# ru-wang/slam-plus-plus

Measured on AMD Instinct MI355X. Metric: Λ-solve block-nnz/sec + batch GN iters/sec, Venice BA, 1→8 MI355X, higher is better.
Workload: dtype f64; 1 GPU; venice871-shaped synthetic BA (871 cams, 530304 points, 2838740 observations, LM-damped); nnzb=3369915, n=1596138, mode=schur+dense, n_reduced=5226, schur_pairs=12875640, parallelism=single GPU

## Files before the change

include/spp_hip.h:

```cpp
#ifndef SPP_HIP_H
#define SPP_HIP_H

#include <stddef.h>
#include <stdint.h>

#ifdef __cplusplus
extern "C" {
#endif

#define SPP_OK            0
#define SPP_NOT_POSDEF    1
#define SPP_E_BADARG     -1
#define SPP_E_NOMEM      -2
#define SPP_E_HIP        -3
#define SPP_E_NO_DEVICE  -4
#define SPP_E_STATE      -5
#define SPP_E_UNSUPPORTED -6

#define SPP_MODE_AUTO     0
#define SPP_MODE_SPARSE   1
#define SPP_MODE_SCHUR    2
#define SPP_MODE_SCHUR_SPARSE 3

#define SPP_FLAG_PROFILE  1
// ... 31 lines not shown
#define SPP_INFO_N_SUPERNODES   12
#define SPP_INFO_N_LEVELS       13
#define SPP_INFO_S_LD           14
#define SPP_INFO_S_NNZB         15
#define SPP_INFO_DENSE_STREAMED 16
#define SPP_INFO_LM_STREAM      17
#define SPP_INFO_BS_GROUPS      18
#define SPP_INFO_SCHUR_SIDE     19
#define SPP_INFO_S_CLEAR        20
#define SPP_INFO_S_DEVICE_PTR   21
#define SPP_INFO_ASM_HUB_CHUNK   22
#define SPP_INFO_SOLVE_ASYNC    23
int spp_get_info(const spp_ctx *ctx, int what, int64_t *out);
int spp_get_ordering(const spp_ctx *ctx, int64_t *h_order);
int64_t spp_sparse_fronts(const spp_ctx *ctx, int64_t capacity, int32_t *h, int32_t *w, int32_t *pad, int32_t *cls, int32_t *level,
	int32_t *parent, int32_t *team);

#define SPP_ORDER_AMD 0
#define SPP_ORDER_ND  1
int spp_block_ordering(int64_t nb, const int64_t *col_ptr, const int64_t *row_idx, int method, int64_t *h_order);

int spp_schur_plan_host(int64_t nb, const int32_t *dim, const int64_t *col_ptr, const int64_t *row_idx, int shard_rank,
	int shard_world, int sparse_S, int64_t *out, double *seconds);

int spp_factor_solve(spp_ctx *ctx, const double *h_vals, double *h_rhs_inout);

int spp_factor_solve_device(spp_ctx *ctx, const double *d_vals, double *d_rhs_inout);

int spp_schur_buffer_size(const spp_ctx *ctx, int64_t *n_doubles);
int spp_schur_form(spp_ctx *ctx, const double *d_vals, const double *d_rhs, double *d_S_rhs);
int spp_schur_finish(spp_ctx *ctx, const double *d_vals, double *d_S_rhs, double *d_rhs_inout);
int spp_schur_packed_size(const spp_ctx *ctx, int64_t *n_doubles);
int spp_schur_pack(spp_ctx *ctx, const double *d_S_rhs, double *d_packed);
int spp_schur_unpack(spp_ctx *ctx, const double *d_packed, double *d_S_rhs);

int spp_assemble_analyze(spp_ctx *ctx, int64_t nv, const int32_t *h_dim,
	int64_t ne, const int64_t *h_v0, const int64_t *h_v1, int d0, int d1, int rd,
	int64_t unary_vertex);
int spp_assemble_get_structure(const spp_ctx *ctx, int64_t *h_col_ptr, int64_t *h_row_idx,
	int64_t *h_blk_off);
int spp_assemble_device(spp_ctx *ctx, const double *d_J0, const double *d_J1,
	const double *d_Omega, const double *d_r, double damping, double *d_vals_out, double *d_eta_out);
int spp_assemble_set_edge_weights(spp_ctx *ctx, const double *d_w);
#define SPP_MAX_EDGE_GROUPS 4
int spp_assemble_analyze_groups(spp_ctx *ctx, int64_t nv, const int32_t *h_dim, int n_groups,
	const int64_t *h_ne, const int64_t *const *h_v0, const int64_t *const *h_v1, const int64_t *const *h_seq,
	const int32_t *h_d0, const int32_t *h_d1, const int32_t *h_rd, int64_t unary_vertex);
int spp_assemble_groups_device(spp_ctx *ctx, const double *const *d_J0, const double *const *d_J1,
	const double *const *d_Omega, const double *const *d_r, double damping, double *d_vals_out, double *d_eta_out);
int spp_assemble_set_group_edge_weights(spp_ctx *ctx, int group, const double *d_w);
int spp_assemble_analyze_ternary(spp_ctx *ctx, int64_t nv, const int32_t *h_dim, int64_t ne, const int64_t *h_v0,
	const int64_t *h_v1, const int64_t *h_v2, int d0, int d1, int d2, int live2, int rd, int64_t unary_vertex);
int spp_assemble_ternary_device(spp_ctx *ctx, const double *d_J0, const double *d_J1, const double *d_J2,
	const double *d_Omega, const double *d_r, double damping, double *d_vals_out, double *d_eta_out);
int spp_edge_robust_weights_device(spp_ctx *ctx, int64_t n_edges, int rd, int kind, double scale, double param,
	const double *d_r, double *d_w_out);

int spp_se2_linearize_device(spp_ctx *ctx, int64_t n_edges, const int32_t *d_v0, const int32_t *d_v1,
	const double *d_poses, const double *d_measurements, double *d_J0, double *d_J1, double *d_r);
int spp_se2_update_device(spp_ctx *ctx, int64_t n_vertices, double *d_poses, const double *d_dx, int apply,
	double *h_dx_norm2);

int spp_se2_linearize_at_device(spp_ctx *ctx, int64_t n_edges, const int64_t *d_off0, const int64_t *d_off1,
	const double *d_state, const double *d_measurements, double *d_J0, double *d_J1, double *d_r);
int spp_se2_rb_linearize_device(spp_ctx *ctx, int64_t n_edges, const int64_t *d_pose_off, const int64_t *d_lm_off,
	const double *d_state, const double *d_measurements, double *d_J0, double *d_J1, double *d_r);
int spp_slam2d_update_device(spp_ctx *ctx, int64_t n, double *d_state, const double *d_dx, int64_t n_pose_angles,
	const int64_t *d_angle_off, int apply, double *h_dx_norm2);

int spp_se3_linearize_device(spp_ctx *ctx, int64_t n_edges, const int32_t *d_v0, const int32_t *d_v1,
	const double *d_poses, const double *d_measurements, double *d_J0, double *d_J1, double *d_r);
int spp_se3_update_device(spp_ctx *ctx, int64_t n_vertices, double *d_poses, const double *d_dx, int apply,
	double *h_dx_norm2);

int spp_se3_linearize_at_device(spp_ctx *ctx, int64_t n_edges, const int64_t *d_off0, const int64_t *d_off1,
	const double *d_state, const double *d_measurements, double *d_J0, double *d_J1, double *d_r);
int spp_se3_xyz_linearize_device(spp_ctx *ctx, int64_t n_edges, const int64_t *d_pose_off, const int64_t *d_lm_off,
	const double *d_state, const double *d_measurements, double *d_J0, double *d_J1, double *d_r);
int spp_slam3d_update_device(spp_ctx *ctx, int64_t n, double *d_state, const double *d_dx, int64_t n_poses,
	const int64_t *d_pose_off, int apply, double *h_dx_norm2);

int spp_rocv_range_linearize_device(spp_ctx *ctx, int64_t n_edges, const int64_t *d_recv_off, const int64_t *d_lm_off,
	const double *d_state, const double *d_measurements, double *d_J0, double *d_J1, double *d_r);
int spp_rocv_cv_linearize_device(spp_ctx *ctx, int64_t n_edges, const int64_t *d_off0, const int64_t *d_off1,
	const double *d_state, const double *d_dt, double *d_J0, double *d_J1, double *d_r);

int spp_ba_linearize_device(spp_ctx *ctx, int64_t n_obs, const int32_t *d_cam_of, const int32_t *d_pt_of,
	const double *d_cams, const double *d_intrinsics, const double *d_points, const double *d_measurements,
	double *d_J0, double *d_J1, double *d_r);
int spp_ba_update_device(spp_ctx *ctx, int64_t n_cams, double *d_cams, const int64_t *d_cam_dxoff,
	int64_t n_points, double *d_points, const int64_t *d_pt_dxoff, const double *d_dx, int64_t n_dx, int apply,
	double *h_dx_norm2);

int spp_sim3_ba_linearize_device(spp_ctx *ctx, int64_t n_obs, const int32_t *d_cam_of, const int32_t *d_pt_of,
	const double *d_cams, const double *d_intrinsics, const double *d_points, const double *d_measurements,
	double *d_J0, double *d_J1, double *d_r);
int spp_sim3_update_device(spp_ctx *ctx, int64_t n_cams, double *d_cams, const int64_t *d_cam_dxoff,
	int64_t n_points, double *d_points, const int64_t *d_pt_dxoff, const double *d_dx, int64_t n_dx, int apply,
	double *h_dx_norm2);

int spp_ba_stereo_linearize_device(spp_ctx *ctx, int64_t n_obs, const int32_t *d_cam_of, const int32_t *d_pt_of,
	const double *d_cams, const double *d_intrinsics, const double *d_points, const double *d_measurements,
	double *d_J0, double *d_J1, double *d_r);

int spp_ba_intrinsics_linearize_device(spp_ctx *ctx, int64_t n_obs, const int32_t *d_cam_of, const int32_t *d_pt_of,
	const int32_t *d_intr_of, const double *d_cams, const double *d_intrinsics, const double *d_points,
	const double *d_measurements, double *d_J0, double *d_J1, double *d_J2, double *d_r);
int spp_ba_intrinsics_update_device(spp_ctx *ctx, int64_t n_intrinsics, double *d_intrinsics, const int64_t *d_intr_dxoff,
	const double *d_dx, int apply, double *h_dx_norm2);

int spp_edge_chi2_device(spp_ctx *ctx, int64_t n_edges, int rd, const double *d_r, const double *d_Omega, double *h_chi2);
int spp_edge_hessian_maxdiag_device(spp_ctx *ctx, int64_t n_edges, int rd, int d0, int d1, const double *d_J0,
	const double *d_J1, const double *d_Omega, double *h_max);
int spp_lm_gain_denominator_device(spp_ctx *ctx, int64_t n, const double *d_dx, const double *d_eta, double alpha,
	double *h_out);

int spp_device_malloc(spp_ctx *ctx, size_t bytes, void **d_ptr);
int spp_device_free(spp_ctx *ctx, void *d_ptr);
int spp_memcpy_h2d(spp_ctx *ctx, void *d_dst, const void *h_src, size_t bytes);
int spp_memcpy_d2h(spp_ctx *ctx, void *h_dst, const void *d_src, size_t bytes);
int spp_memcpy_d2d(spp_ctx *ctx, void *d_dst, const void *d_src, size_t bytes);

int spp_set_profiling(spp_ctx *ctx, int on);

#define SPP_PHASE_PERMUTE   0
#define SPP_PHASE_SCHUR_INV 1
#define SPP_PHASE_SCHUR_GEMM 2
#define SPP_PHASE_SCHUR_RHS 3
#define SPP_PHASE_FACTOR    4
#define SPP_PHASE_TRISOLVE  5
#define SPP_PHASE_BACKSUBST 6
#define SPP_PHASE_ASSEMBLE  7
#define SPP_PHASE_TOTAL     8
#define SPP_N_PHASES        9
int spp_get_phase_ms(spp_ctx *ctx, double *ms_out );
int spp_get_dominant_kernel(spp_ctx *ctx, double *ms_total, int64_t *n_launches, double *flops);

int spp_microbench_copy(spp_ctx *ctx, size_t bytes, int iters, double *gb_per_s);
int spp_microbench_mfma_f64(spp_ctx *ctx, int iters, double *tflops);
int spp_microbench_ctile(spp_ctx *ctx, int n, int iters, double *gb_per_s);
int spp_microbench_update(spp_ctx *ctx, int64_t m, int iters, double *ms_per_launch);

int spp_dense_potrf_upper(spp_ctx *ctx, double *d_A, int64_t n, int64_t ld);
int spp_dense_posv(spp_ctx *ctx, double *d_A, int64_t n, int64_t ld, double *d_b);
int spp_dense_posv_masked(spp_ctx *ctx, double *d_A, int64_t n, int64_t ld, double *d_b, const uint64_t *words, int64_t nwords);
int spp_tile_mask_host(int64_t n, int bs, int64_t nblk, const int32_t *i1, const int32_t *i2, int has_rhs, int fill,
	uint64_t *words, int64_t *n_updates);
int spp_schur_tile_mask_host(int64_t nb, const int32_t *dim, const int64_t *col_ptr, const int64_t *row_idx, int shard_rank,
	int shard_world, uint64_t *words);
int spp_schur_cam_order_host(int64_t nb, const int32_t *dim, const int64_t *col_ptr, const int64_t *row_idx, int shard_rank,
	int shard_world, int flags, const int64_t *order_in, int64_t *cam_order, double *figures);
int spp_tail_order_host(int64_t n, int has_rhs, const uint64_t *words, int64_t nwords, int resident, int early, double beta,
	int32_t *table, int32_t *info);
int spp_dense_gemm_tn_sub(spp_ctx *ctx, int64_t m, int64_t n, int64_t k,
	const double *d_A, int64_t lda, const double *d_B, int64_t ldb, double *d_C, int64_t ldc);
int spp_dense_gemm_tn_sub_upper(spp_ctx *ctx, int64_t m, int64_t n, int64_t k,
	const double *d_A, int64_t lda, const double *d_B, int64_t ldb, double *d_C, int64_t ldc);
int spp_dense_front_factor(spp_ctx *ctx, double *d_F, int64_t ld, int64_t w, int64_t h, double *d_image);

const char *spp_version(void);

#ifdef __cplusplus
}
#endif
#endif
```

slam_plus_plus_amd/api.py:

```python
import ctypes
import os

import numpy as np

_HERE = os.path.dirname(os.path.abspath(__file__))
LIB_PATH = os.environ.get("SPP_LIB") or os.path.join(_HERE, "libspp_hip.so")

SPP_OK, SPP_NOT_POSDEF = 0, 1
MODE_AUTO, MODE_SPARSE, MODE_SCHUR, MODE_SCHUR_SPARSE, MODE_SCHUR_MIS = 0, 1, 2, 3, 4
FLAG_PROFILE = 1
INFO = dict(MODE=0, N=1, NNZB=2, NVALS=3, FACTOR_NNZ=4, FACTOR_FLOPS=5, N_REDUCED=6, N_POSES=7,
            N_LANDMARKS=8, SCHUR_PAIRS=9, N_OBS=10, SOLVE_BYTES=11, N_SUPERNODES=12, N_LEVELS=13, S_LD=14, S_NNZB=15, DENSE_STREAMED=16,
            LM_STREAM=17, BS_GROUPS=18, SCHUR_SIDE=19, S_CLEAR=20, S_DEVICE_PTR=21, ASM_HUB_CHUNK=22, SOLVE_ASYNC=23)
PHASES = ["permute", "schur_inv", "schur_gemm", "schur_rhs", "factor", "trisolve", "backsubst", "assemble", "total"]

EXPORTS = [
    "spp_create", "spp_destroy", "spp_free_memory", "spp_last_error", "spp_host_staging", "spp_set_stream", "spp_synchronize",
    "spp_analyze", "spp_set_shard", "spp_get_info", "spp_get_ordering", "spp_sparse_fronts", "spp_factor_solve",
    "spp_factor_solve_device", "spp_schur_buffer_size", "spp_schur_form", "spp_schur_finish",
    "spp_schur_packed_size", "spp_schur_pack", "spp_schur_unpack",
    "spp_assemble_analyze", "spp_assemble_get_structure", "spp_assemble_device", "spp_assemble_set_edge_weights",
    "spp_assemble_analyze_groups", "spp_assemble_groups_device", "spp_assemble_set_group_edge_weights",
    "spp_assemble_analyze_ternary", "spp_assemble_ternary_device", "spp_ba_intrinsics_linearize_device",
    "spp_ba_intrinsics_update_device",
    "spp_se2_linearize_at_device", "spp_se2_rb_linearize_device", "spp_slam2d_update_device",
    "spp_se3_linearize_at_device", "spp_se3_xyz_linearize_device", "spp_slam3d_update_device", "spp_rocv_range_linearize_device",
    "spp_rocv_cv_linearize_device", "spp_device_malloc",
    "spp_device_free", "spp_memcpy_h2d", "spp_memcpy_d2h", "spp_memcpy_d2d", "spp_get_phase_ms", "spp_get_dominant_kernel",
    "spp_microbench_copy", "spp_microbench_mfma_f64", "spp_microbench_ctile", "spp_microbench_update", "spp_block_ordering", "spp_schur_plan_host", "spp_set_profiling", "spp_se2_linearize_device", "spp_se2_update_device", "spp_ba_linearize_device", "spp_ba_stereo_linearize_device", "spp_ba_update_device", "spp_sim3_ba_linearize_device", "spp_sim3_update_device", "spp_se3_linearize_device", "spp_se3_update_device", "spp_edge_chi2_device", "spp_edge_robust_weights_device", "spp_edge_hessian_maxdiag_device",
    "spp_lm_gain_denominator_device", "spp_dense_potrf_upper", "spp_dense_posv",
    "spp_dense_posv_masked", "spp_tile_mask_host", "spp_schur_tile_mask_host", "spp_tail_order_host", "spp_schur_cam_order_host",
    "spp_dense_gemm_tn_sub", "spp_dense_gemm_tn_sub_upper", "spp_dense_front_factor", "spp_version",
]

_lib = None
_c_i64p = ctypes.POINTER(ctypes.c_int64)
_c_i32p = ctypes.POINTER(ctypes.c_int32)
_c_f64p = ctypes.POINTER(ctypes.c_double)


class SppError(RuntimeError):
    """std::runtime_error of the C++ adapter (reference LinearSolver_Schur_GPU.cpp:734-797)."""


def load_library():
    global _lib
    if _lib is not None:
        return _lib
    if not os.path.exists(LIB_PATH):
        raise SppError("libspp_hip.so is not built: run `python -m slam_plus_plus_amd.build` "
                       "(hipcc --offload-arch=gfx950); there is no CPU fallback")
    lib = ctypes.CDLL(LIB_PATH)
    vp, i64, i32, dbl, cint = ctypes.c_void_p, ctypes.c_int64, ctypes.c_int32, ctypes.c_double, ctypes.c_int
    sig = {
        "spp_create": (vp, [cint, cint]),
        "spp_destroy": (None, [vp]),
        "spp_free_memory": (cint, [vp]),
        "spp_last_error": (cint, [vp, ctypes.c_char_p, ctypes.c_size_t]),
        "spp_host_staging": (vp, [vp, i64]),
        "spp_set_stream": (cint, [vp, vp]),
        "spp_synchronize": (cint, [vp]),
        "spp_analyze": (cint, [vp, i64, vp, vp, vp, vp, cint]),
        "spp_set_shard": (cint, [vp, cint, cint]),
        "spp_get_info": (cint, [vp, cint, _c_i64p]),
        "spp_get_ordering": (cint, [vp, vp]),
        "spp_sparse_fronts": (i64, [vp, i64, vp, vp, vp, vp, vp, vp, vp]),
        "spp_factor_solve": (cint, [vp, vp, vp]),
        "spp_factor_solve_device": (cint, [vp, vp, vp]),
        "spp_schur_buffer_size": (cint, [vp, _c_i64p]),
        "spp_schur_form": (cint, [vp, vp, vp, vp]),
        "spp_schur_finish": (cint, [vp, vp, vp, vp]),
        "spp_schur_packed_size": (cint, [vp, _c_i64p]),
        "spp_schur_pack": (cint, [vp, vp, vp]),
        "spp_schur_unpack": (cint, [vp, vp, vp]),
        "spp_assemble_analyze": (cint, [vp, i64, vp, i64, vp, vp, cint, cint, cint, i64]),
        "spp_assemble_get_structure": (cint, [vp, vp, vp, vp]),
        "spp_assemble_device": (cint, [vp, vp, vp, vp, vp, dbl, vp, vp]),
        "spp_assemble_set_edge_weights": (cint, [vp, vp]),
        "spp_assemble_analyze_groups": (cint, [vp, i64, vp, cint, vp, vp, vp, vp, vp, vp, vp, i64]),
        "spp_assemble_groups_device": (cint, [vp, vp, vp, vp, vp, dbl, vp, vp]),
        "spp_assemble_set_group_edge_weights": (cint, [vp, cint, vp]),
        "spp_assemble_analyze_ternary": (cint, [vp, i64, vp, i64, vp, vp, vp, cint, cint, cint, cint, cint, i64]),
        "spp_assemble_ternary_device": (cint, [vp, vp, vp, vp, vp, vp, dbl, vp, vp]),
        "spp_ba_intrinsics_linearize_device": (cint, [vp, i64, vp, vp, vp, vp, vp, vp, vp, vp, vp, vp, vp]),
        "spp_ba_intrinsics_update_device": (cint, [vp, i64, vp, vp, vp, cint, _c_f64p]),
        "spp_se2_linearize_at_device": (cint, [vp, i64, vp, vp, vp, vp, vp, vp, vp]),
        "spp_se2_rb_linearize_device": (cint, [vp, i64, vp, vp, vp, vp, vp, vp, vp]),
        "spp_slam2d_update_device": (cint, [vp, i64, vp, vp, i64, vp, cint, _c_f64p]),
        "spp_se3_linearize_at_device": (cint, [vp, i64, vp, vp, vp, vp, vp, vp, vp]),
        "spp_se3_xyz_linearize_device": (cint, [vp, i64, vp, vp, vp, vp, vp, vp, vp]),
        "spp_slam3d_update_device": (cint, [vp, i64, vp, vp, i64, vp, cint, _c_f64p]),
        "spp_rocv_range_linearize_device": (cint, [vp, i64, vp, vp, vp, vp, vp, vp, vp]),
        "spp_rocv_cv_linearize_device": (cint, [vp, i64, vp, vp, vp, vp, vp, vp, vp]),
        "spp_device_malloc": (cint, [vp, ctypes.c_size_t, ctypes.POINTER(vp)]),
        "spp_device_free": (cint, [vp, vp]),
        "spp_memcpy_h2d": (cint, [vp, vp, vp, ctypes.c_size_t]),
        "spp_memcpy_d2h": (cint, [vp, vp, vp, ctypes.c_size_t]),
        "spp_memcpy_d2d": (cint, [vp, vp, vp, ctypes.c_size_t]),
        "spp_get_phase_ms": (cint, [vp, _c_f64p]),
        "spp_get_dominant_kernel": (cint, [vp, _c_f64p, _c_i64p, _c_f64p]),
        "spp_microbench_copy": (cint, [vp, ctypes.c_size_t, cint, _c_f64p]),
        "spp_microbench_mfma_f64": (cint, [vp, cint, _c_f64p]),
        "spp_microbench_ctile": (cint, [vp, cint, cint, _c_f64p]),
        "spp_microbench_update": (cint, [vp, ctypes.c_int64, cint, _c_f64p]),
        "spp_block_ordering": (cint, [ctypes.c_int64, vp, vp, cint, vp]),
        "spp_schur_plan_host": (cint, [ctypes.c_int64, vp, vp, vp, cint, cint, cint, vp, vp]),
        "spp_set_profiling": (cint, [vp, cint]),
        "spp_se2_linearize_device": (cint, [vp, ctypes.c_int64, vp, vp, vp, vp, vp, vp, vp]),
        "spp_se2_update_device": (cint, [vp, ctypes.c_int64, vp, vp, cint, _c_f64p]),
        "spp_se3_linearize_device": (cint, [vp, ctypes.c_int64, vp, vp, vp, vp, vp, vp, vp]),
        "spp_se3_update_device": (cint, [vp, ctypes.c_int64, vp, vp, cint, _c_f64p]),
        "spp_edge_chi2_device": (cint, [vp, ctypes.c_int64, cint, vp, vp, _c_f64p]),
        "spp_edge_robust_weights_device": (cint, [vp, ctypes.c_int64, cint, cint, dbl, dbl, vp, vp]),
        "spp_edge_hessian_maxdiag_device": (cint, [vp, ctypes.c_int64, cint, cint, cint, vp, vp, vp, _c_f64p]),
        "spp_lm_gain_denominator_device": (cint, [vp, ctypes.c_int64, vp, vp, ctypes.c_double, _c_f64p]),
        "spp_ba_linearize_device": (cint, [vp, ctypes.c_int64, vp, vp, vp, vp, vp, vp, vp, vp, vp]),
        "spp_ba_stereo_linearize_device": (cint, [vp, ctypes.c_int64, vp, vp, vp, vp, vp, vp, vp, vp, vp]),
        "spp_ba_update_device": (cint, [vp, ctypes.c_int64, vp, vp, ctypes.c_int64, vp, vp, vp, ctypes.c_int64, cint, _c_f64p]),
        "spp_sim3_ba_linearize_device": (cint, [vp, ctypes.c_int64, vp, vp, vp, vp, vp, vp, vp, vp, vp]),
        "spp_sim3_update_device": (cint, [vp, ctypes.c_int64, vp, vp, ctypes.c_int64, vp, vp, vp, ctypes.c_int64, cint, _c_f64p]),
        "spp_dense_potrf_upper": (cint, [vp, vp, i64, i64]),
        "spp_dense_posv": (cint, [vp, vp, i64, i64, vp]),
        "spp_dense_posv_masked": (cint, [vp, vp, i64, i64, vp, vp, i64]),
        "spp_tile_mask_host": (cint, [i64, cint, i64, vp, vp, cint, cint, vp, vp]),
        "spp_schur_tile_mask_host": (cint, [i64, vp, vp, vp, cint, cint, vp]),
        "spp_tail_order_host": (cint, [i64, cint, vp, i64, cint, cint, dbl, vp, vp]),
        "spp_schur_cam_order_host": (cint, [i64, vp, vp, vp, cint, cint, cint, vp, vp, vp]),
        "spp_dense_gemm_tn_sub": (cint, [vp, i64, i64, i64, vp, i64, vp, i64, vp, i64]),
        "spp_dense_gemm_tn_sub_upper": (cint, [vp, i64, i64, i64, vp, i64, vp, i64, vp, i64]),
        "spp_dense_front_factor": (cint, [vp, vp, i64, i64, i64, vp]),
        "spp_version": (ctypes.c_char_p, []),
    }
    for name, (res, args) in sig.items():
        fn = getattr(lib, name)
        fn.restype = res
        fn.argtypes = args
    _lib = lib
    return lib


def _ptr(a):
    return a.ctypes.data_as(ctypes.c_void_p)


ORDER_AMD, ORDER_ND = 0, 1


def block_ordering(lam, method=ORDER_AMD):
    lib = load_library()
    col_ptr = np.ascontiguousarray(lam.col_ptr, dtype=np.int64)
    row_idx = np.ascontiguousarray(lam.row_idx, dtype=np.int64)
    out = np.empty(lam.nb, dtype=np.int64)
    code = lib.spp_block_ordering(lam.nb, _ptr(col_ptr), _ptr(row_idx), method, _ptr(out))
    if code != 0:
        raise SppError("spp_block_ordering failed: %d" % code)
    return out


def schur_plan_host(lam, shard_rank=0, shard_world=1, sparse_S=False, mis=False):
    lib = load_library()
    col_ptr = np.ascontiguousarray(lam.col_ptr, dtype=np.int64)
    row_idx = np.ascontiguousarray(lam.row_idx, dtype=np.int64)
    dim = np.ascontiguousarray(lam.dim, dtype=np.int32)
    out = np.zeros(9, dtype=np.int64)
    sec = ctypes.c_double(0.0)
    code = lib.spp_schur_plan_host(lam.nb, _ptr(dim), _ptr(col_ptr), _ptr(row_idx), shard_rank, shard_world,
                                   (1 if sparse_S else 0) | (2 if mis else 0), _ptr(out), ctypes.byref(sec))
    if code != 0:
        raise SppError("spp_schur_plan_host failed: %d" % code)
    keys = ("nc", "nl", "no", "n_pairs", "n_sblk", "n_items", "n_multi", "checksum", "checksum_all")
    d = dict(zip(keys, (int(v) for v in out)))
    d["seconds"] = sec.value
    return d


def tile_mask_host(n, bs, i1, i2, has_rhs=True, fill=True):
    lib = load_library()
    i1 = np.ascontiguousarray(i1, dtype=np.int32)
    i2 = np.ascontiguousarray(i2, dtype=np.int32)
    words = np.zeros(64, dtype=np.uint64)
    upd = ctypes.c_int64(0)
    code = lib.spp_tile_mask_host(n, bs, i1.size, _ptr(i1), _ptr(i2), 1 if has_rhs else 0, 1 if fill else 0, _ptr(words),
                                  ctypes.byref(upd))
    if code < 0:
        raise SppError("spp_tile_mask_host failed: %d" % code)
    return words[:code].copy(), upd.value


def schur_tile_mask_host(lam, shard_rank=0, shard_world=1):
    lib = load_library()
    col_ptr = np.ascontiguousarray(lam.col_ptr, dtype=np.int64)
    row_idx = np.ascontiguousarray(lam.row_idx, dtype=np.int64)
    dim = np.ascontiguousarray(lam.dim, dtype=np.int32)
    words = np.zeros(64, dtype=np.uint64)
    code = lib.spp_schur_tile_mask_host(lam.nb, _ptr(dim), _ptr(col_ptr), _ptr(row_idx), shard_rank, shard_world, _ptr(words))
    if code < 0:
        raise SppError("spp_schur_tile_mask_host failed: %d" % code)
    return words[:code].copy()


def schur_cam_order_host(lam, order=None, sparse_S=False, mis=False, shard_rank=0, shard_world=1):
    lib = load_library()
    col_ptr = np.ascontiguousarray(lam.col_ptr, dtype=np.int64)
    row_idx = np.ascontiguousarray(lam.row_idx, dtype=np.int64)
    dim = np.ascontiguousarray(lam.dim, dtype=np.int32)
    nc = int((dim == dim.max()).sum()) if not mis else int(dim.size)
    out = np.full(max(nc, 1), -1, dtype=np.int64)
    fig = np.zeros(8, dtype=np.float64)
    oin = None if order is None else np.ascontiguousarray(order, dtype=np.int64)
    if oin is not None and oin.size != nc:
        raise SppError("schur_cam_order_host: order must list every camera once")
    code = lib.spp_schur_cam_order_host(lam.nb, _ptr(dim), _ptr(col_ptr), _ptr(row_idx), shard_rank, shard_world,
                                        (1 if sparse_S else 0) | (2 if mis else 0),
                                        _ptr(oin) if oin is not None else None, _ptr(out), _ptr(fig))
    if code < 0:
        raise SppError("spp_schur_cam_order_host failed: %d" % code)
    keys = ("tiles", "updates", "path", "cost_us")
    natural = dict(zip(keys, (int(fig[0]), int(fig[1]), int(fig[2]), float(fig[3]))))
    chosen = dict(zip(keys, (int(fig[4]), int(fig[5]), int(fig[6]), float(fig[7]))))
    return out[out >= 0], bool(code), natural, chosen


def tail_order_host(n, words, has_rhs=True, resident=256, early=True, beta=0.0):
    lib = load_library()
    words = np.ascontiguousarray(words if words is not None else [], dtype=np.uint64)
    table = np.zeros(64 * 65 // 2 + 64, dtype=np.int32)
    info = np.zeros(5, dtype=np.int32)
    code = lib.spp_tail_order_host(int(n), 1 if has_rhs else 0, _ptr(words) if words.size else None, words.size, int(resident),
                                   1 if early else 0, float(beta), _ptr(table), _ptr(info))
    if code < 0:
        raise SppError("spp_tail_order_host failed: %d" % code)
    tiles = [(int(t) >> 16, int(t) & 0xffff) for t in table[:code]]
    return tiles, dict(zip(("n_early", "r_star", "rows_resident", "live_demand", "widest"), (int(v) for v in info)))


class DeviceArray:

    def __init__(self, ctx, n, dtype=np.float64):
        self.ctx, self.n, self.dtype = ctx, int(n), np.dtype(dtype)
        p = ctypes.c_void_p()
        ctx._check(ctx.lib.spp_device_malloc(ctx.h, self.n * self.dtype.itemsize, ctypes.byref(p)))
        self.ptr = p.value

    @classmethod
    def from_host(cls, ctx, arr):
        arr = np.ascontiguousarray(arr)
        d = cls(ctx, arr.size, arr.dtype)
        d.upload(arr)
        return d

    def upload(self, arr):
        arr = np.ascontiguousarray(arr, dtype=self.dtype)
        assert arr.size == self.n
        self.ctx._check(self.ctx.lib.spp_memcpy_h2d(self.ctx.h, self.ptr, _ptr(arr), arr.nbytes))

    def download(self):
        out = np.empty(self.n, dtype=self.dtype)
        self.ctx._check(self.ctx.lib.spp_memcpy_d2h(self.ctx.h, _ptr(out), self.ptr, out.nbytes))
        return out

    def copy_from(self, other):
        assert other.n * other.dtype.itemsize <= self.n * self.dtype.itemsize
        self.ctx._check(self.ctx.lib.spp_memcpy_d2d(self.ctx.h, self.ptr, other.ptr, other.n * other.dtype.itemsize))

    def free(self):
        if self.ptr:
            self.ctx.lib.spp_device_free(self.ctx.h, self.ptr)
            self.ptr = None


class Context:

    def __init__(self, device=0, flags=0):
        self.lib = load_library()
        self.h = self.lib.spp_create(int(device), int(flags))
        if not self.h:
            raise SppError("spp_create failed: no usable HIP device %d (the solver has no CPU fallback)" % device)

    def close(self):
        if getattr(self, "h", None):
            self.lib.spp_destroy(self.h)
            self.h = None

    def __del__(self):
        try:
            self.close()
        except Exception:
            pass

    def last_error(self):
        buf = ctypes.create_string_buffer(1024)
        self.lib.spp_last_error(self.h, buf, 1024)
        return buf.value.decode(errors="replace")

    def _check(self, code):
        if code < 0:
            if code == -2:
                raise MemoryError(self.last_error())
            raise SppError("spp error %d: %s" % (code, self.last_error()))
        return code

    def analyze(self, bcsc, mode=MODE_AUTO):
        self._keep = bcsc
        return self._check(self.lib.spp_analyze(self.h, bcsc.nb, _ptr(bcsc.col_ptr), _ptr(bcsc.row_idx),
                                                 _ptr(bcsc.blk_off), _ptr(bcsc.dim), mode))

    def set_shard(self, rank, world):
        return self._check(self.lib.spp_set_shard(self.h, rank, world))

    def info(self, key):
        out = ctypes.c_int64()
        self._check(self.lib.spp_get_info(self.h, INFO[key], ctypes.byref(out)))
        return out.value

    def ordering(self, nb):
        out = np.empty(nb, dtype=np.int64)
        self._check(self.lib.spp_get_ordering(self.h, _ptr(out)))
        return out

    def sparse_fronts(self):
        keys = ("h", "w", "pad", "cls", "level", "parent", "team")
        ns = self._check(self.lib.spp_sparse_fronts(self.h, 0, None, None, None, None, None, None, None))
        out = {k: np.zeros(ns, dtype=np.int32) for k in keys}
        if ns:
            self._check(self.lib.spp_sparse_fronts(self.h, ns, *[_ptr(out[k]) for k in keys]))
        return out

    def se2_linearize_device(self, n_edges, d_v0, d_v1, d_poses, d_meas, d_J0, d_J1, d_r):
        return self._check(self.lib.spp_se2_linearize_device(self.h, n_edges, d_v0, d_v1, d_poses, d_meas, d_J0, d_J1, d_r))

    def se2_update_device(self, n_vertices, d_poses, d_dx, apply=True):
        out = ctypes.c_double()
        self._check(self.lib.spp_se2_update_device(self.h, n_vertices, d_poses, d_dx, 1 if apply else 0, ctypes.byref(out)))
        return out.value ** 0.5

    def se2_linearize_at_device(self, n_edges, d_off0, d_off1, d_state, d_meas, d_J0, d_J1, d_r):
        return self._check(self.lib.spp_se2_linearize_at_device(self.h, n_edges, d_off0, d_off1, d_state, d_meas, d_J0, d_J1, d_r))

    def se2_rb_linearize_device(self, n_edges, d_pose_off, d_lm_off, d_state, d_meas, d_J0, d_J1, d_r):
        return self._check(self.lib.spp_se2_rb_linearize_device(self.h, n_edges, d_pose_off, d_lm_off, d_state, d_meas, d_J0, d_J1, d_r))

    def slam2d_update_device(self, n, d_state, d_dx, n_pose_angles, d_angle_off, apply=True):
        out = ctypes.c_double()
        self._check(self.lib.spp_slam2d_update_device(self.h, n, d_state, d_dx, n_pose_angles, d_angle_off, 1 if apply else 0,
                                                      ctypes.byref(out)))
        return out.value ** 0.5

    def se3_linearize_at_device(self, n_edges, d_off0, d_off1, d_state, d_meas, d_J0, d_J1, d_r):
        return self._check(self.lib.spp_se3_linearize_at_device(self.h, n_edges, d_off0, d_off1, d_state, d_meas, d_J0, d_J1, d_r))

    def se3_xyz_linearize_device(self, n_edges, d_pose_off, d_lm_off, d_state, d_meas, d_J0, d_J1, d_r):
        return self._check(self.lib.spp_se3_xyz_linearize_device(self.h, n_edges, d_pose_off, d_lm_off, d_state, d_meas, d_J0, d_J1, d_r))

    def slam3d_update_device(self, n, d_state, d_dx, n_poses, d_pose_off, apply=True):
        out = ctypes.c_double()
        self._check(self.lib.spp_slam3d_update_device(self.h, n, d_state, d_dx, n_poses, d_pose_off, 1 if apply else 0,
                                                      ctypes.byref(out)))
        return out.value ** 0.5

    def rocv_range_linearize_device(self, n_edges, d_recv_off, d_lm_off, d_state, d_meas, d_J0, d_J1, d_r):
        return self._check(self.lib.spp_rocv_range_linearize_device(self.h, n_edges, d_recv_off, d_lm_off, d_state, d_meas, d_J0, d_J1, d_r))

    def rocv_cv_linearize_device(self, n_edges, d_off0, d_off1, d_state, d_dt, d_J0, d_J1, d_r):
        return self._check(self.lib.spp_rocv_cv_linearize_device(self.h, n_edges, d_off0, d_off1, d_state, d_dt, d_J0, d_J1, d_r))

    def se3_linearize_device(self, n_edges, d_v0, d_v1, d_poses, d_meas, d_J0, d_J1, d_r):
        return self._check(self.lib.spp_se3_linearize_device(self.h, n_edges, d_v0, d_v1, d_poses, d_meas, d_J0, d_J1, d_r))

    def se3_update_device(self, n_vertices, d_poses, d_dx, apply=True):
        out = ctypes.c_double()
        self._check(self.lib.spp_se3_update_device(self.h, n_vertices, d_poses, d_dx, 1 if apply else 0, ctypes.byref(out)))
        return out.value ** 0.5

    def edge_robust_weights_device(self, n_edges, rd, d_r, d_w, scale, param=1.345, kind=0):
        return self._check(self.lib.spp_edge_robust_weights_device(self.h, n_edges, rd, kind, float(scale), float(param), d_r, d_w))

    def edge_chi2_device(self, n_edges, rd, d_r, d_Om):
        out = ctypes.c_double()
        self._check(self.lib.spp_edge_chi2_device(self.h, n_edges, rd, d_r, d_Om, ctypes.byref(out)))
        return out.value

    def edge_hessian_maxdiag_device(self, n_edges, rd, d0, d1, d_J0, d_J1, d_Om):
        out = ctypes.c_double()
        self._check(self.lib.spp_edge_hessian_maxdiag_device(self.h, n_edges, rd, d0, d1, d_J0, d_J1, d_Om, ctypes.byref(out)))
        return out.value

# ... 227 lines not shown
```

slam_plus_plus_amd/csrc/spp_api.cpp:

```cpp

#include "spp_internal.h"
#include <string.h>
#include <new>

using namespace spp;

namespace spp {

void phases_reset(spp_ctx *ctx)
{
	if(!(ctx->flags & SPP_FLAG_PROFILE))
		return;
	if(!ctx->timer.created) {
		for(int i = 0; i < 2 * SPP_N_PHASES; ++ i)
			SPP_HIP_CHECK(hipEventCreate(&ctx->timer.ev[i]));
		ctx->timer.created = true;
	}
	for(int i = 0; i < SPP_N_PHASES; ++ i) {
		ctx->timer.used[i] = false;
		ctx->phase_ms[i] = 0;
	}
	ctx->dom_used = 0;
	ctx->dom_flops = 0;
}
// ... 404 lines not shown
	return SPP_OK;
}

int spp_get_ordering(const spp_ctx *ctx, int64_t *h_order)
{
	if(!ctx || !h_order)
		return SPP_E_BADARG;
	if(ctx->mode < 0)
		return SPP_E_STATE;
	for(size_t i = 0; i < ctx->order.size(); ++ i)
		h_order[i] = ctx->order[i];
	return SPP_OK;
}

int64_t spp_sparse_fronts(const spp_ctx *ctx, int64_t capacity, int32_t *h, int32_t *w, int32_t *pad, int32_t *cls, int32_t *level,
	int32_t *parent, int32_t *team)
{
	if(!ctx || capacity < 0)
		return SPP_E_BADARG;
#ifdef SPP_HAVE_SPARSE
	if(ctx->sparse)
		return sparse_fronts(ctx, capacity, h, w, pad, cls, level, parent, team);
#endif
	return 0;
}

int spp_block_ordering(int64_t nb, const int64_t *col_ptr, const int64_t *row_idx, int method, int64_t *h_order)
{
	if(nb <= 0 || !col_ptr || !row_idx || !h_order || (method != SPP_ORDER_AMD && method != SPP_ORDER_ND))
		return SPP_E_BADARG;
	try {
		for(int64_t j = 0; j < nb; ++ j)
			for(int64_t p = col_ptr[j]; p < col_ptr[j + 1]; ++ p)
				if(row_idx[p] < 0 || row_idx[p] > j)
					return SPP_E_BADARG;
		std::vector<int64_t> order;
		if(method == SPP_ORDER_AMD)
			min_degree_order(nb, col_ptr, row_idx, order);
		else
			nested_dissection_order(nb, col_ptr, row_idx, order);
		for(int64_t k = 0; k < nb; ++ k)
			h_order[k] = order[k];
		return SPP_OK;
	} catch(const std::bad_alloc &) {
		return SPP_E_NOMEM;
	} catch(...) {
		return SPP_E_HIP;
	}
}

static bool structure_of_pattern(int64_t nb, const int32_t *dim, const int64_t *col_ptr, const int64_t *row_idx, Structure &st)
{
	st.nb = nb;
	st.nnzb = col_ptr[nb];
	st.col_ptr.assign(col_ptr, col_ptr + nb + 1);
	st.row_idx.assign(row_idx, row_idx + st.nnzb);
	st.dim.assign(dim, dim + nb);
	st.base.resize(nb + 1);
	st.base[0] = 0;
	for(int64_t j = 0; j < nb; ++ j)
		st.base[j + 1] = st.base[j] + dim[j];
	st.n = st.base[nb];
	st.blk_off.resize(st.nnzb);
	int64_t off = 0;
	for(int64_t j = 0; j < nb; ++ j)
		for(int64_t p = col_ptr[j]; p < col_ptr[j + 1]; ++ p) {
			if(row_idx[p] < 0 || row_idx[p] > j)
				return false;
			st.blk_off[p] = off;
			off += (int64_t)dim[row_idx[p]] * dim[j];
		}
	st.nvals = off;
	return true;
}

extern "C++" {
template <class F>
static int schur_host_entry(int64_t nb, const int32_t *dim, const int64_t *col_ptr, const int64_t *row_idx, int shard_rank,
	int shard_world, const void *out, F fn)
{
	if(nb <= 0 || !dim || !col_ptr || !row_idx || !out || shard_world < 1 || shard_rank < 0 || shard_rank >= shard_world)
		return SPP_E_BADARG;
	try {
		Structure st;
		if(!structure_of_pattern(nb, dim, col_ptr, row_idx, st))
			return SPP_E_BADARG;
		return fn(st);
	} catch(const Error &e) {
		return e.code;
	} catch(const std::bad_alloc &) {
		return SPP_E_NOMEM;
	} catch(...) {
		return SPP_E_HIP;
	}
}
}

int spp_schur_plan_host(int64_t nb, const int32_t *dim, const int64_t *col_ptr, const int64_t *row_idx, int shard_rank,
	int shard_world, int sparse_S, int64_t *out, double *seconds)
{
	return schur_host_entry(nb, dim, col_ptr, row_idx, shard_rank, shard_world, out, [&](const Structure &st) {
		const double sec = schur_plan_host_probe(st, shard_rank, shard_world, (sparse_S & 1) != 0, (sparse_S & 2) != 0, out);
		if(seconds)
			*seconds = sec;
		return (int)SPP_OK;
	});
}

int spp_schur_tile_mask_host(int64_t nb, const int32_t *dim, const int64_t *col_ptr, const int64_t *row_idx, int shard_rank,
	int shard_world, uint64_t *words)
{
	return schur_host_entry(nb, dim, col_ptr, row_idx, shard_rank, shard_world, words, [&](const Structure &st) {
		std::vector<uint64_t> w;
		schur_tile_mask_host_probe(st, w);
		for(size_t q = 0; q < w.size(); ++ q)
			words[q] = w[q];
		return (int)w.size();
	});
}

int spp_schur_cam_order_host(int64_t nb, const int32_t *dim, const int64_t *col_ptr, const int64_t *row_idx, int shard_rank,
	int shard_world, int flags, const int64_t *order_in, int64_t *cam_order, double *figures)
{
	if(!figures)
		return SPP_E_BADARG;
	return schur_host_entry(nb, dim, col_ptr, row_idx, shard_rank, shard_world, cam_order, [&](const Structure &st) {
		if(order_in) {
			int64_t nc = 0;
			const int dmax = *std::max_element(dim, dim + nb);
			for(int64_t j = 0; j < nb; ++ j)
				nc += dim[j] == dmax;
			std::vector<char> seen((size_t)nc, 0);
			for(int64_t q = 0; q < nc; ++ q) {
				if(order_in[q] < 0 || order_in[q] >= nc || seen[order_in[q]])
					return (int)SPP_E_BADARG;
				seen[order_in[q]] = 1;
			}
		}
		std::vector<int32_t> order;
		TileDagCost cost[2];
		const bool used = schur_cam_order_host_probe(st, shard_rank, shard_world, (flags & 1) != 0, (flags & 2) != 0, order_in, order, cost);
		for(size_t q = 0; q < order.size(); ++ q)
			cam_order[q] = order[q];
		for(int side = 0; side < 2; ++ side) {
			figures[4 * side] = (double)cost[side].tiles;
			figures[4 * side + 1] = (double)cost[side].updates;
			figures[4 * side + 2] = (double)cost[side].path;
			figures[4 * side + 3] = cost[side].cost_us;
		}
		return used ? 1 : 0;
	});
}

int spp_schur_buffer_size(const spp_ctx *ctx, int64_t *n_doubles)
{
	if(!ctx || !n_doubles)
		return SPP_E_BADARG;
	if(ctx->mode != SPP_MODE_SCHUR)
		return SPP_E_STATE;
	*n_doubles = schur_buffer_doubles(ctx);
	return SPP_OK;
}

int spp_schur_form(spp_ctx *ctx, const double *d_vals, const double *d_rhs, double *d_S_rhs)
{
	if(!ctx || !d_vals || !d_rhs || !d_S_rhs)
		return SPP_E_BADARG;
	SPP_TRY(ctx)
	SPP_REQUIRE(ctx->mode == SPP_MODE_SCHUR, SPP_E_STATE, "spp_schur_form: analyze in Schur mode first");
	SPP_HIP_CHECK(hipSetDevice(ctx->device));
	phases_reset(ctx);
	phase_begin(ctx, SPP_PHASE_TOTAL);
	schur_form(ctx, d_vals, d_rhs, d_S_rhs);
	return SPP_OK;
	SPP_CATCH(ctx)
}

int spp_schur_packed_size(const spp_ctx *ctx, int64_t *n_doubles)
{
	if(!ctx || !n_doubles)
		return SPP_E_BADARG;
	if(ctx->mode != SPP_MODE_SCHUR)
		return SPP_E_STATE;
	if(ctx->schur.sparse_S) {
		*n_doubles = schur_buffer_doubles(ctx);
		return SPP_OK;
	}
	const int64_t nblk = ctx->schur.ld / DENSE_NB;
	*n_doubles = (int64_t)DENSE_NB * DENSE_NB * (nblk * (nblk + 1) / 2);
	return SPP_OK;
}

int spp_schur_pack(spp_ctx *ctx, const double *d_S_rhs, double *d_packed)
{
	if(!ctx || !d_S_rhs || !d_packed)
		return SPP_E_BADARG;
	SPP_TRY(ctx)
	SPP_REQUIRE(ctx->mode == SPP_MODE_SCHUR, SPP_E_STATE, "spp_schur_pack: analyze in Schur mode first");
	SPP_HIP_CHECK(hipSetDevice(ctx->device));
	if(ctx->schur.sparse_S)
		SPP_HIP_CHECK(hipMemcpyAsync(d_packed, d_S_rhs, (size_t)schur_buffer_doubles(ctx) * sizeof(double),
			hipMemcpyDeviceToDevice, ctx->stream));
	else
		schur_pack(ctx, const_cast<double*>(d_S_rhs), d_packed, true);
	return SPP_OK;
	SPP_CATCH(ctx)
}

int spp_schur_unpack(spp_ctx *ctx, const double *d_packed, double *d_S_rhs)
{
	if(!ctx || !d_S_rhs || !d_packed)
		return SPP_E_BADARG;
	SPP_TRY(ctx)
	SPP_REQUIRE(ctx->mode == SPP_MODE_SCHUR, SPP_E_STATE, "spp_schur_unpack: analyze in Schur mode first");
	SPP_HIP_CHECK(hipSetDevice(ctx->device));
	if(ctx->schur.sparse_S)
		SPP_HIP_CHECK(hipMemcpyAsync(d_S_rhs, d_packed, (size_t)schur_buffer_doubles(ctx) * sizeof(double),
			hipMemcpyDeviceToDevice, ctx->stream));
	else
		schur_pack(ctx, d_S_rhs, const_cast<double*>(d_packed), false);
	return SPP_OK;
	SPP_CATCH(ctx)
}

int spp_schur_finish(spp_ctx *ctx, const double *d_vals, double *d_S_rhs, double *d_rhs_inout)
{
	if(!ctx || !d_vals || !d_rhs_inout || !d_S_rhs)
		return SPP_E_BADARG;
	SPP_TRY(ctx)
	SPP_REQUIRE(ctx->mode == SPP_MODE_SCHUR, SPP_E_STATE, "spp_schur_finish: analyze in Schur mode first");
	SPP_HIP_CHECK(hipSetDevice(ctx->device));
	int ret = schur_finish(ctx, d_vals, d_S_rhs, d_rhs_inout);
	phase_end(ctx, SPP_PHASE_TOTAL);
	phases_collect(ctx);
	dense_chain_check(ctx);
	return ret;
	SPP_CATCH(ctx)
}

int spp_factor_solve_device(spp_ctx *ctx, const double *d_vals, double *d_rhs)
{
	if(!ctx || !d_vals || !d_rhs)
		return SPP_E_BADARG;
	SPP_TRY(ctx)
	SPP_REQUIRE(ctx->mode >= 0, SPP_E_STATE, "spp_factor_solve: call spp_analyze first");
	SPP_HIP_CHECK(hipSetDevice(ctx->device));
	phases_reset(ctx);
	phase_begin(ctx, SPP_PHASE_TOTAL);
	int ret;
	if(ctx->mode == SPP_MODE_SCHUR) {
		SPP_REQUIRE(ctx->shard_world == 1, SPP_E_STATE,
			"sharded ctx: use spp_schur_form / all-reduce / spp_schur_finish");
		if(!ctx->schur.S.p || ctx->schur.S.cap < (size_t)schur_buffer_doubles(ctx)) {
			ctx->schur.unlisted_dirty = true;
			ctx_drain(ctx);
		}
		ctx->schur.S.reserve((size_t)schur_buffer_doubles(ctx));
		schur_form(ctx, d_vals, d_rhs, ctx->schur.S.p, true);
		ret = schur_finish(ctx, d_vals, ctx->schur.S.p, d_rhs);
	} else
		ret = sparse_factor_solve(ctx, d_vals, d_rhs);
	phase_end(ctx, SPP_PHASE_TOTAL);
	phases_collect(ctx);
	if(!(ctx->mode == SPP_MODE_SCHUR && ctx->schur.async_last))
		SPP_HIP_CHECK(hipStreamSynchronize(ctx->stream));
	dense_chain_check(ctx);
	return ret;
	SPP_CATCH(ctx)
}

int spp_factor_solve(spp_ctx *ctx, const double *h_vals, double *h_rhs)
{
	if(!ctx || !h_vals || !h_rhs)
		return SPP_E_BADARG;
	SPP_TRY(ctx)
	SPP_REQUIRE(ctx->mode >= 0, SPP_E_STATE, "spp_factor_solve: call spp_analyze first");
	SPP_HIP_CHECK(hipSetDevice(ctx->device));
	ctx->d_vals.reserve((size_t)ctx->st.nvals);
	ctx->d_rhs.reserve((size_t)ctx->st.n);
	SPP_HIP_CHECK(hipMemcpyAsync(ctx->d_vals.p, h_vals, ctx->st.nvals * sizeof(double), hipMemcpyHostToDevice, ctx->stream));
	SPP_HIP_CHECK(hipMemcpyAsync(ctx->d_rhs.p, h_rhs, ctx->st.n * sizeof(double), hipMemcpyHostToDevice, ctx->stream));
	int ret = spp_factor_solve_device(ctx, ctx->d_vals.p, ctx->d_rhs.p);
	if(ret != SPP_OK)
		return ret;
	SPP_HIP_CHECK(hipMemcpyAsync(h_rhs, ctx->d_rhs.p, ctx->st.n * sizeof(double), hipMemcpyDeviceToHost, ctx->stream));
	SPP_HIP_CHECK(hipStreamSynchronize(ctx->stream));
	dense_chain_check(ctx);
	return SPP_OK;
	SPP_CATCH(ctx)
}

int spp_assemble_analyze(spp_ctx *ctx, int64_t nv, const int32_t *h_dim, int64_t ne, const int64_t *h_v0,
	const int64_t *h_v1, int d0, int d1, int rd, int64_t unary_vertex)
{
	if(!ctx)
		return SPP_E_BADARG;
	assemble_release(ctx);
	if(!h_dim || !h_v0 || !h_v1 || nv <= 0 || ne <= 0)
		return SPP_E_BADARG;
	SPP_TRY(ctx)
	SPP_HIP_CHECK(hipSetDevice(ctx->device));
	assemble_analyze(ctx, nv, h_dim, 1, &ne, &h_v0, &h_v1, nullptr, &d0, &d1, &rd, unary_vertex);
	return SPP_OK;
	SPP_CATCH(ctx)
}

// ... 365 lines not shown
		return SPP_E_BADARG;
	SPP_TRY(ctx)
	SPP_HIP_CHECK(hipSetDevice(ctx->device));
	SPP_HIP_CHECK(hipMemcpyAsync(h_dst, d_src, bytes, hipMemcpyDeviceToHost, ctx->stream));
	SPP_HIP_CHECK(hipStreamSynchronize(ctx->stream));
	dense_chain_check(ctx);
	return SPP_OK;
	SPP_CATCH(ctx)
}

int spp_memcpy_d2d(spp_ctx *ctx, void *d_dst, const void *d_src, size_t bytes)
{
	if(!ctx)
		return SPP_E_BADARG;
	SPP_TRY(ctx)
	SPP_HIP_CHECK(hipSetDevice(ctx->device));
	SPP_HIP_CHECK(hipMemcpyAsync(d_dst, d_src, bytes, hipMemcpyDeviceToDevice, ctx->stream));
	return SPP_OK;
	SPP_CATCH(ctx)
}

int spp_get_phase_ms(spp_ctx *ctx, double *ms_out)
{
	if(!ctx || !ms_out)
		return SPP_E_BADARG;
	for(int i = 0; i < SPP_N_PHASES; ++ i)
		ms_out[i] = ctx->phase_ms[i];
	return SPP_OK;
}

int spp_get_dominant_kernel(spp_ctx *ctx, double *ms_total, int64_t *n_launches, double *flops)
{
	if(!ctx || !ms_total || !n_launches || !flops)
		return SPP_E_BADARG;
	SPP_TRY(ctx)
	SPP_HIP_CHECK(hipStreamSynchronize(ctx->stream));
	double total = 0;
	for(size_t i = 0; i + 1 < ctx->dom_used; i += 2) {
		float ms = 0;
		SPP_HIP_CHECK(hipEventElapsedTime(&ms, ctx->dom_events[i], ctx->dom_events[i + 1]));
		total += ms;
	}
	*ms_total = total;
	*n_launches = (int64_t)(ctx->dom_used / 2);
	*flops = ctx->dom_flops;
	return SPP_OK;
	SPP_CATCH(ctx)
}

int spp_microbench_copy(spp_ctx *ctx, size_t bytes, int iters, double *gb_per_s)
{
	if(!ctx || !gb_per_s)
		return SPP_E_BADARG;
	SPP_TRY(ctx)
	SPP_HIP_CHECK(hipSetDevice(ctx->device));
	*gb_per_s = microbench_copy(ctx, bytes, iters);
	return SPP_OK;
	SPP_CATCH(ctx)
}

int spp_microbench_ctile(spp_ctx *ctx, int n, int iters, double *gb_per_s)
{
	if(!ctx || !gb_per_s)
		return SPP_E_BADARG;
	SPP_TRY(ctx)
	SPP_HIP_CHECK(hipSetDevice(ctx->device));
	*gb_per_s = microbench_ctile(ctx, n, iters);
	return SPP_OK;
	SPP_CATCH(ctx)
}

int spp_microbench_update(spp_ctx *ctx, int64_t m, int iters, double *ms_per_launch)
{
	if(!ctx || !ms_per_launch || m < 128 || iters < 1)
		return SPP_E_BADARG;
	SPP_TRY(ctx)
	SPP_HIP_CHECK(hipSetDevice(ctx->device));
	*ms_per_launch = microbench_update(ctx, m, iters);
	return SPP_OK;
	SPP_CATCH(ctx)
}

int spp_microbench_mfma_f64(spp_ctx *ctx, int iters, double *tflops)
{
	if(!ctx || !tflops)
		return SPP_E_BADARG;
	SPP_TRY(ctx)
	SPP_HIP_CHECK(hipSetDevice(ctx->device));
	*tflops = microbench_mfma_f64(ctx, iters);
	return SPP_OK;
	SPP_CATCH(ctx)
}

int spp_dense_potrf_upper(spp_ctx *ctx, double *d_A, int64_t n, int64_t ld)
{
	if(!ctx || !d_A || n <= 0 || ld < n)
		return SPP_E_BADARG;
	SPP_TRY(ctx)
	SPP_HIP_CHECK(hipSetDevice(ctx->device));
	const int64_t ldp = ((n + 1 + DENSE_NB - 1) / DENSE_NB) * DENSE_NB;
	DevBuf<double> tmp;
	tmp.reserve((size_t)ldp * ldp);
	SPP_HIP_CHECK(hipMemsetAsync(tmp.p, 0, (size_t)ldp * ldp * sizeof(double), ctx->stream));
	SPP_HIP_CHECK(hipMemcpy2DAsync(tmp.p, ldp * sizeof(double), d_A, ld * sizeof(double), n * sizeof(double), n,
		hipMemcpyDeviceToDevice, ctx->stream));
	dense_set_padding(ctx, tmp.p, ldp, n);
	int ret = dense_potrf_upper(ctx, tmp.p, n, ldp, true);
	SPP_HIP_CHECK(hipMemcpy2DAsync(d_A, ld * sizeof(double), tmp.p, ldp * sizeof(double), n * sizeof(double), n,
		hipMemcpyDeviceToDevice, ctx->stream));
	SPP_HIP_CHECK(hipStreamSynchronize(ctx->stream));
	return ret;
	SPP_CATCH(ctx)
}

int spp_dense_posv(spp_ctx *ctx, double *d_A, int64_t n, int64_t ld, double *d_b)
{
	return spp_dense_posv_masked(ctx, d_A, n, ld, d_b, nullptr, 0);
}

int spp_tile_mask_host(int64_t n, int bs, int64_t nblk, const int32_t *i1, const int32_t *i2, int has_rhs, int fill,
	uint64_t *words, int64_t *n_updates)
{
	if(n <= 0 || bs <= 0 || nblk < 0 || (nblk && (!i1 || !i2)) || !words)
		return SPP_E_BADARG;
	try {
		std::vector<uint64_t> w;
		tile_mask_mark(n, bs, nblk, i1, i2, w);
		const int64_t upd = tile_mask_close(n, has_rhs != 0, fill != 0, w);
		if(n_updates)
			*n_updates = upd;
		for(size_t q = 0; q < w.size(); ++ q)
			words[q] = w[q];
		return (int)w.size();
	} catch(...) {
		return SPP_E_NOMEM;
	}
}

int spp_tail_order_host(int64_t n, int has_rhs, const uint64_t *words, int64_t nwords, int resident, int early, double beta,
	int32_t *table, int32_t *info)
{
	const int64_t Tr = (n + DENSE_NB - 1) / DENSE_NB, Tc = has_rhs ? n / DENSE_NB + 1 : Tr;
	if(n <= 0 || Tr > 64 || Tc > 64 || nwords < 0 || (nwords && (!words || nwords != Tr)) || !table || !(beta >= 0))
		return SPP_E_BADARG;
	try {
		std::vector<uint64_t> bits((size_t)Tr + 1);
		const uint64_t all_cols = Tc == 64 ? ~0ull : (1ull << Tc) - 1;
		bits[0] = all_cols;
		for(int64_t i = 0; i < Tr; ++ i)
			bits[(size_t)i + 1] = (((nwords ? words[i] : all_cols) | (1ull << i)) & ~((1ull << i) - 1)) & all_cols;
		std::vector<int> order;
		int oinfo[5];
		const bool use = nwords && early;
		tail_order_table(bits, (int)Tr, (int)Tc, false, beta, use ? resident : 0, use, order, oinfo);
		for(size_t q = 0; q < order.size(); ++ q)
			table[q] = order[q];
		if(info)
			for(int q = 0; q < 5; ++ q)
				info[q] = oinfo[q];
		return (int)order.size();
	} catch(...) {
		return SPP_E_NOMEM;
	}
}

int spp_dense_posv_masked(spp_ctx *ctx, double *d_A, int64_t n, int64_t ld, double *d_b, const uint64_t *words, int64_t nwords)
{
	if(!ctx || !d_A || !d_b || n <= 0 || ld < n || nwords < 0 || (nwords && !words))
		return SPP_E_BADARG;
	SPP_TRY(ctx)
	SPP_HIP_CHECK(hipSetDevice(ctx->device));
	std::vector<uint64_t> mask(words, words + nwords);
	if(nwords) {
		SPP_REQUIRE(nwords == (n + DENSE_NB - 1) / DENSE_NB, SPP_E_BADARG, "posv: one mask word per tile row of 128");
		tile_mask_close(n, true, true, mask);
	}
	TileMaskGuard guard(ctx->dense, &mask);
	const int64_t ldp = ((n + 1 + DENSE_NB - 1) / DENSE_NB) * DENSE_NB;
	DevBuf<double> tmp;
	tmp.reserve((size_t)ldp * ldp);
	SPP_HIP_CHECK(hipMemsetAsync(tmp.p, 0, (size_t)ldp * ldp * sizeof(double), ctx->stream));
	SPP_HIP_CHECK(hipMemcpy2DAsync(tmp.p, ldp * sizeof(double), d_A, ld * sizeof(double), n * sizeof(double), n,
		hipMemcpyDeviceToDevice, ctx->stream));
	dense_set_padding(ctx, tmp.p, ldp, n);
	SPP_HIP_CHECK(hipMemcpyAsync(tmp.p + n * ldp, d_b, n * sizeof(double), hipMemcpyDeviceToDevice, ctx->stream));
	int ret = dense_potrf_upper(ctx, tmp.p, n, ldp, true);
	if(ret == SPP_OK) {
		dense_potrs_upper(ctx, tmp.p, n, ldp, tmp.p + n * ldp);
		SPP_HIP_CHECK(hipMemcpyAsync(d_b, tmp.p + n * ldp, n * sizeof(double), hipMemcpyDeviceToDevice, ctx->stream));
		SPP_HIP_CHECK(hipMemcpy2DAsync(d_A, ld * sizeof(double), tmp.p, ldp * sizeof(double), n * sizeof(double), n,
			hipMemcpyDeviceToDevice, ctx->stream));
	}
	SPP_HIP_CHECK(hipStreamSynchronize(ctx->stream));
	dense_chain_check(ctx);
	return ret;
	SPP_CATCH(ctx)
}

int spp_dense_gemm_tn_sub(spp_ctx *ctx, int64_t m, int64_t n, int64_t k, const double *d_A, int64_t lda,
	const double *d_B, int64_t ldb, double *d_C, int64_t ldc)
{
	if(!ctx || !d_A || !d_B || !d_C)
		return SPP_E_BADARG;
	SPP_TRY(ctx)
	SPP_REQUIRE((lda % 2) == 0 && (ldb % 2) == 0, SPP_E_BADARG, "gemm_tn_sub: lda/ldb must be even (16-byte loads)");
	SPP_HIP_CHECK(hipSetDevice(ctx->device));
	dense_gemm_tn_sub(ctx, m, n, k, d_A, lda, d_B, ldb, d_C, ldc, false);
	SPP_HIP_CHECK(hipStreamSynchronize(ctx->stream));
	return SPP_OK;
	SPP_CATCH(ctx)
}

int spp_dense_gemm_tn_sub_upper(spp_ctx *ctx, int64_t m, int64_t n, int64_t k, const double *d_A, int64_t lda,
	const double *d_B, int64_t ldb, double *d_C, int64_t ldc)
{
	if(!ctx || !d_A || !d_B || !d_C)
		return SPP_E_BADARG;
	SPP_TRY(ctx)
	SPP_REQUIRE((lda % 2) == 0 && (ldb % 2) == 0, SPP_E_BADARG, "gemm_tn_sub: lda/ldb must be even (16-byte loads)");
	SPP_HIP_CHECK(hipSetDevice(ctx->device));
	dense_gemm_tn_sub(ctx, m, n, k, d_A, lda, d_B, ldb, d_C, ldc, true);
	SPP_HIP_CHECK(hipStreamSynchronize(ctx->stream));
	return SPP_OK;
	SPP_CATCH(ctx)
}

int spp_dense_front_factor(spp_ctx *ctx, double *d_F, int64_t ld, int64_t w, int64_t h, double *d_image)
{
	if(!ctx || !d_F)
		return SPP_E_BADARG;
	SPP_TRY(ctx)
	SPP_HIP_CHECK(hipSetDevice(ctx->device));
	return dense_front_factor(ctx, d_F, ld, w, h, d_image);
	SPP_CATCH(ctx)
}

}
```

slam_plus_plus_amd/csrc/spp_dense.hip:

```cpp

#include "spp_internal.h"
#include "spp_tiles.h"
#include "spp_dense_dev.h"
#include <stdio.h>
#include <stdlib.h>
#include <string.h>
#include <algorithm>
#include <vector>
#include <mutex>

namespace spp {


constexpr int BK = 16;
constexpr int LDS_STRIDE = 18;

template <int BM, int BN, int WM, int WN, int MODE, int DEPTH, int BKT, int SC1 = 0>
__device__ __forceinline__ void gemm_tn_tile(const int64_t m0, const int64_t n0, int64_t M, int64_t N, int K,
	const double *__restrict__ A, int64_t lda, const double *B, int64_t ldb, double *C, int64_t ldc, double *gemm_lds)
{
	constexpr int NWM = BM / WM, NWN = BN / WN, NT = NWM * NWN * 64;
	constexpr int TA = WM / 16, TB = WN / 16;
	constexpr int PPC = BKT / 2, LSTR = BKT + 2;
	constexpr int PA = (BM * PPC) / NT, PB = (BN * PPC) / NT;
// ... 1144 lines not shown
		const int64_t ntr = nr - 1, ntc = nc - 1;
		const int64_t T = ntr > 0 ? ntr * (ntr + 1) / 2 + (ntc - ntr) * ntr : 0;
		const int64_t n128 = (T / slots) * slots;
		const int64_t grid = 4 * (int64_t)npri + n128 + 4 * (T - n128);
		if(grid > 0)
			hipLaunchKernelGGL(la_bulk_kernel, dim3((unsigned)grid), dim3(1024), LA_BULK_LDS_DOUBLES * sizeof(double), sb,
				a, k, nr, nc, npri, n128);
	}
	SPP_HIP_CHECK(hipEventRecord(dw.ev[1], sb));
	SPP_HIP_CHECK(hipEventRecord(dw.ev_chain, sc));
	SPP_HIP_CHECK(hipStreamWaitEvent(s, dw.ev[1], 0));
	SPP_HIP_CHECK(hipStreamWaitEvent(s, dw.ev_chain, 0));
	SPP_HIP_CHECK(hipGetLastError());
	if(tracing) {
		std::vector<long long> h((size_t)12 * nsteps + 16);
		SPP_HIP_CHECK(hipMemcpyAsync(h.data(), dw.la_trace.p, h.size() * sizeof(long long), hipMemcpyDeviceToHost, s));
		SPP_HIP_CHECK(hipStreamSynchronize(s));
		fprintf(stderr, "[spp] lookahead factorization, %d steps: potrf start / duration / gap to the next start (us)\n", a.nsteps);
		for(int k = 0; k < a.nsteps; ++ k)
			fprintf(stderr, "  k %2d  start %8.1f  potrf %5.1f  publish %4.1f | b1 seen +%4.1f  done +%4.1f | c1 seen +%4.1f  done +%4.1f | step %5.1f\n", k,
				(h[8 * k] - h[0]) * 0.01, (h[8 * k + 2] - h[8 * k]) * 0.01, (h[8 * k + 1] - h[8 * k + 2]) * 0.01,
				(h[8 * k + 3] - h[8 * k + 1]) * 0.01, (h[8 * k + 4] - h[8 * k + 1]) * 0.01, (h[8 * k + 5] - h[8 * k + 1]) * 0.01,
				(h[8 * k + 6] - h[8 * k + 1]) * 0.01, k + 1 < a.nsteps ? (h[8 * (k + 1)] - h[8 * k]) * 0.01 : 0.0);
		fprintf(stderr, "[spp] per step: panel (rest) done / bulk launch: first tile starts, priority tiles done, last tile done, busy workgroup-us (all relative to potrf(0) start)\n");
		for(int k = 0; k < a.nsteps; ++ k) {
			const long long *b = h.data() + 8 * nsteps + 8 + 4 * k;
			fprintf(stderr, "  k %2d  panel done %8.1f | bulk start %8.1f  pri done %8.1f  end %8.1f  busy %9.1f\n", k, h[8 * k + 7] ? (h[8 * k + 7] - h[0]) * 0.01 : 0.0,
				b[1] ? (b[0] - h[0]) * 0.01 : 0.0, b[3] ? (b[3] - h[0]) * 0.01 : 0.0, b[1] ? (b[1] - h[0]) * 0.01 : 0.0, b[2] * 0.01);
		}
	}
}

void dense_factor_steps(spp_ctx *ctx, double *d_A, int64_t ld, int64_t n, int64_t rows, int64_t ncols,
	int64_t nsteps, bool has_rhs)
{
	ensure_dense_work(ctx, nsteps);
	ctx->dense.tail_rows_last = 0;
	ctx->dense.tail_masked_whole = false;
	const bool captured = capturing(ctx->stream);
	if(!captured && la_usable(ctx, nsteps)) {
		dense_factor_lookahead(ctx, d_A, ld, n, rows, ncols, nsteps, has_rhs);
		ctx->dense.tinv_half = 0;
		return;
	}
	ctx->dense.tinv_half = nsteps;
	const bool flags = !captured && nsteps >= 4 && flag_schedule_usable(ctx);
	dense_factor_steps_enqueue(ctx, d_A, ld, n, rows, ncols, nsteps, has_rhs, flags, !captured);
}

static void flag_signal(hipStream_t st, int *flag, int value)
{
	hipLaunchKernelGGL(flag_signal_kernel, dim3(1), dim3(64), 0, st, flag, value);
}

static FlagWait make_flag_wait(spp_ctx *ctx, const int *flag, int value, long long timeout_ticks = WAIT_TICKS_DEFAULT)
{
	return FlagWait{flag, value, ctx->dense.info.p + 2, timeout_ticks};
}

static void flag_wait(spp_ctx *ctx, hipStream_t st, const int *flag, int value, long long timeout_ticks)
{
	hipLaunchKernelGGL(flag_wait_kernel, dim3(1), dim3(64), 0, st, make_flag_wait(ctx, flag, value, timeout_ticks));
}

static bool streams_concurrent(spp_ctx *ctx, hipStream_t a, hipStream_t b, int slot)
{
	DenseWork &dw = ctx->dense;
	hipStream_t st[2] = {a, b};
	dw.sync.reserve(16);
	SPP_HIP_CHECK(hipMemsetAsync(dw.sync.p, 0, 16 * sizeof(int), ctx->stream));
	SPP_HIP_CHECK(hipStreamSynchronize(ctx->stream));
	for(int p = 0; p < 2; ++ p) {
		flag_wait(ctx, st[p], dw.sync.p + slot + p, 1, 20 * WAIT_TICKS_PER_MS);
		flag_signal(st[1 - p], dw.sync.p + slot + p, 1);
	}
	for(int i = 0; i < 2; ++ i)
		SPP_HIP_CHECK(hipStreamSynchronize(st[i]));
	int h_abort = 0;
	SPP_HIP_CHECK(hipMemcpy(&h_abort, dw.info.p + 2, sizeof(int), hipMemcpyDeviceToHost));
	if(h_abort) {
		SPP_HIP_CHECK(hipMemset(dw.info.p + 2, 0, sizeof(int)));
		return false;
	}
	return true;
}

static bool flag_schedule_usable(spp_ctx *ctx)
{
	if(!switches().dense_sched)
		return false;
	DenseWork &dw = ctx->dense;
	if(dw.sync_state == 0 || dw.sync_stream != ctx->stream) {
		if(capturing(ctx->stream))
			return false;
		dw.sync_state = streams_concurrent(ctx, ctx->stream, dw.aux, 0) ? 1 : -1;
		dw.sync_stream = ctx->stream;
	}
	return dw.sync_state == 1;
}

static bool dense_tail_applies(spp_ctx *ctx, int64_t rows, int64_t nsteps)
{
	return !ctx->dense.tail_disabled && nsteps * NB >= rows && !(ctx->dense.ident_from >= 0 && ctx->dense.ident_from < rows);
}

static bool launch_dense_tail(spp_ctx *ctx, double *d_A, int64_t ld, int64_t rows, int64_t ncols, int64_t nsteps, int64_t k, bool has_rhs)
{
	const Switches &sw = switches();
	DenseWork &dw = ctx->dense;
	const int64_t c1 = (k + 1) * NB;
	if(!dense_tail_applies(ctx, rows, nsteps))
		return false;
	const int Tr = (int)(nsteps - (k + 1)), Tc = (int)((ncols - c1 + NB - 1) / NB);
	if(Tr < 1 || Tr > sw.tail_rows || Tc < Tr || Tc > Tr + 1 || Tc > TAIL_MAX_ROWS)
		return false;
	const std::vector<uint64_t> *mask = (sw.tail_mask && dw.tile_mask && (int64_t)dw.tile_mask->size() == nsteps) ? dw.tile_mask : nullptr;
	std::vector<uint64_t> bits((size_t)Tr + 1);
	const uint64_t all_cols = Tc == 64 ? ~0ull : (1ull << Tc) - 1;
	for(int i = -1; i < Tr; ++ i) {
		const int64_t g = k + 1 + i;
		uint64_t w = (mask && g >= 0) ? ((*mask)[(size_t)g] >> (k + 1)) : all_cols;
		if(i >= 0)
			w = (w | (1ull << i)) & ~((1ull << i) - 1);
		bits[(size_t)i + 1] = w & all_cols;
	}
	hipStream_t s = ctx->stream;
	static uint64_t attr_seen = 0;
	if(first_on_this_device(attr_seen))
		SPP_HIP_CHECK(hipFuncSetAttribute((const void*)dense_tail_kernel, hipFuncAttributeMaxDynamicSharedMemorySize,
			TAIL_LDS_DOUBLES * (int)sizeof(double)));
	if(dw.tail_pub.cap < (size_t)Tr * Tc) {
		dw.tail_pub.reserve(std::max<size_t>((size_t)Tr * Tc, 24 * 25));
		SPP_HIP_CHECK(hipMemsetAsync(dw.tail_pub.p, 0, dw.tail_pub.cap * sizeof(int), s));
		dw.tail_epoch = 0;
	}
	if(dw.tail_dinv.cap < (size_t)Tr * 8 * 256)
		dw.tail_dinv.reserve(std::max<size_t>((size_t)Tr * 8 * 256, (size_t)24 * 8 * 256));
	if(++ dw.tail_epoch >= (1 << 26)) {
		SPP_HIP_CHECK(hipMemsetAsync(dw.tail_pub.p, 0, dw.tail_pub.cap * sizeof(int), s));
		dw.tail_epoch = 1;
	}
	const bool early = mask != nullptr && sw.tail_early != 0;
	if(early && dw.tail_resident < 0) {
		int per_cu = 0;
		hipDeviceProp_t prop;
		if(hipOccupancyMaxActiveBlocksPerMultiprocessor(&per_cu, (const void*)dense_tail_kernel, POTRF_THREADS,
		   TAIL_LDS_DOUBLES * sizeof(double)) == hipSuccess && hipGetDeviceProperties(&prop, ctx->device) == hipSuccess)
			dw.tail_resident = std::max(per_cu, 0) * prop.multiProcessorCount;
		else {
			(void)hipGetLastError();
			dw.tail_resident = 0;
		}
	}
	if(dw.tail_order_tr != Tr || dw.tail_order_tc != Tc || dw.tail_order_bits != bits || dw.tail_order_pre != (k >= 0) ||
	   dw.tail_order_masked != early) {
		if(!dw.tail_order_host.empty())
			SPP_HIP_CHECK(hipStreamSynchronize(s));
		std::vector<int> &order = dw.tail_order_host;
		int oinfo[5];
		tail_order_table(bits, Tr, Tc, k >= 0, sw.tail_order_beta, early ? dw.tail_resident : 0, early, order, oinfo);
		if(sw.verbose)
			fprintf(stderr, "[spp] streamed tail: %d x %d tiles, %d listed, %d resident; %d tiles of rows %d.. seated first (whole rows resident %d, live demand %d)\n",
				Tr, Tc, (int)order.size(), early ? dw.tail_resident : 0, oinfo[0], oinfo[1], oinfo[2], oinfo[3]);
		dw.tail_order.upload(order, s);
		dw.tail_order_tr = Tr;
		dw.tail_order_tc = Tc;
		dw.tail_order_bits = bits;
		dw.tail_order_pre = k >= 0;
		dw.tail_order_masked = early;
	}
	const int ntile = (int)dw.tail_order_host.size();
	TailArgs a;
	a.order = dw.tail_order.p;
	memset(a.rowbits, 0, sizeof(a.rowbits));
	for(size_t q = 0; q < bits.size(); ++ q)
		a.rowbits[q] = bits[q];
	a.A = d_A;
	a.ld = ld;
	a.rows = rows;
	a.ncols = ncols;
	a.c0 = c1;
	a.have_pre = (k >= 0) ? 1 : 0;
	a.Tr = Tr;
	a.Tc = Tc;
	a.has_rhs = has_rhs ? 1 : 0;
	a.tinv = dw.tinv_all.p + (size_t)(k + 1) * NB * NB;
	a.dbuf = dw.tail_dinv.p;
	a.pub = dw.tail_pub.p;
	a.epoch = dw.tail_epoch;
	a.info = dw.info.p;
	a.abort = dw.info.p + 2;
	a.timeout_ticks = sw.tail_timeout_ticks;
	static int launches = 0;
	DevBuf<long long> trace;
	a.trace = nullptr;
	if(sw.tail_trace && ++ launches == sw.tail_trace) {
		trace.reserve((size_t)Tr * 8);
		SPP_HIP_CHECK(hipMemsetAsync(trace.p, 0, (size_t)Tr * 8 * sizeof(long long), s));
		a.trace = trace.p;
	}
	dom_begin(ctx);
	hipLaunchKernelGGL(dense_tail_kernel, dim3((unsigned)ntile), dim3(POTRF_THREADS), TAIL_LDS_DOUBLES * sizeof(double), s, a);
	{
		const double m = (double)(rows - c1);
		dom_end(ctx, m * m * m / 3.0 + (a.have_pre ? (double)NB * m * (m + 1.0) : 0.0) + 2.0 * m * m);
	}
	dw.tail_rows_last = Tr;
	dw.tail_masked_whole = k < 0 && mask != nullptr;
	SPP_HIP_CHECK(hipGetLastError());
	if(a.trace) {
		std::vector<long long> h((size_t)Tr * 8);
		SPP_HIP_CHECK(hipStreamSynchronize(s));
		SPP_HIP_CHECK(hipMemcpy(h.data(), trace.p, h.size() * sizeof(long long), hipMemcpyDeviceToHost));
		fprintf(stderr, "[spp] streamed tail, %d tile rows, %d of %d tiles launched (us from the launch's first stamp): diagonal tile: updates complete / factored+inverted | first panel tile: first row tile seen / last seen / last published\n", Tr, ntile, Tr * Tc - Tr * (Tr - 1) / 2);
		const long long t0 = h[0];
		for(int i = 0; i < Tr; ++ i)
			fprintf(stderr, "  row %2d  start %7.1f  updated %7.1f  done %7.1f | %7.1f %7.1f %7.1f\n", i, (h[8 * i] - t0) * 0.01, (h[8 * i + 1] - t0) * 0.01,
				(h[8 * i + 2] - t0) * 0.01, h[8 * i + 3] ? (h[8 * i + 3] - t0) * 0.01 : 0.0, h[8 * i + 4] ? (h[8 * i + 4] - t0) * 0.01 : 0.0, h[8 * i + 5] ? (h[8 * i + 5] - t0) * 0.01 : 0.0);
	}
	return true;
}

static void dense_factor_steps_enqueue(spp_ctx *ctx, double *d_A, int64_t ld, int64_t n, int64_t rows, int64_t ncols,
	int64_t nsteps, bool has_rhs, bool use_flags, bool allow_fused)
{
	hipStream_t s = ctx->stream, s2 = ctx->dense.aux;
	hipEvent_t evA = ctx->dense.ev[0], evB = ctx->dense.ev[1];
	DenseWork &dw = ctx->dense;
	const int64_t n_id = (dw.ident_from >= 0 && dw.ident_from < n) ? dw.ident_from : n;
	int ep = 0;
	int64_t step_a = -1, step_b = -1;
	int64_t need_wait_b = -1;
	if(use_flags) {
		if(dw.sync.cap < (size_t)(2 * nsteps + 16)) {
			dw.sync.reserve((size_t)(2 * nsteps + 16));
			SPP_HIP_CHECK(hipMemsetAsync(dw.sync.p, 0, dw.sync.cap * sizeof(int), s));
			dw.sync_epoch = 1;
		}
		ep = ++ dw.sync_epoch;
		SPP_HIP_CHECK(hipEventRecord(evA, s));
		SPP_HIP_CHECK(hipStreamWaitEvent(s2, evA, 0));
	}
	int64_t pend_sig = -1;
	auto record_a = [&](int64_t k) {
		step_a = k;
		if(use_flags)
			pend_sig = k;
		else
			SPP_HIP_CHECK(hipEventRecord(evA, s));
	};
	int64_t pend_sig_b = -1;
	auto wait_a_on_bulk = [&]() {
		if(use_flags && pend_sig_b >= 0) {
			hipLaunchKernelGGL(flag_signal_wait_kernel, dim3(1), dim3(64), 0, s2, dw.sync.p + 2 * pend_sig_b + 1, ep,
				make_flag_wait(ctx, dw.sync.p + 2 * step_a, ep));
			pend_sig_b = -1;
		} else if(use_flags)
			flag_wait(ctx, s2, dw.sync.p + 2 * step_a, ep);
		else
			SPP_HIP_CHECK(hipStreamWaitEvent(s2, evA, 0));
	};
	auto flush_sig_b = [&]() {
		if(pend_sig_b >= 0)
			flag_signal(s2, dw.sync.p + 2 * pend_sig_b + 1, ep);
		pend_sig_b = -1;
	};
	auto record_b = [&](int64_t k) {
		step_b = k;
		if(use_flags)
			pend_sig_b = k;
		else
			SPP_HIP_CHECK(hipEventRecord(evB, s2));
	};
	auto wait_b_now = [&]() {
		if(use_flags && pend_sig_b == step_b)
			flush_sig_b();
		if(use_flags && pend_sig >= 0) {
			flag_signal(s, dw.sync.p + 2 * pend_sig, ep);
			pend_sig = -1;
		}
		if(use_flags)
			flag_wait(ctx, s, dw.sync.p + 2 * step_b + 1, ep);
		else
			SPP_HIP_CHECK(hipStreamWaitEvent(s, evB, 0));
	};
	auto wait_b_deferred = [&]() {
		if(use_flags)
			need_wait_b = step_b;
		else
			SPP_HIP_CHECK(hipStreamWaitEvent(s, evB, 0));
	};
	auto flush_wait_b = [&]() {
		if(need_wait_b >= 0 && pend_sig_b == need_wait_b)
			flush_sig_b();
		if(need_wait_b >= 0 && pend_sig >= 0)
			hipLaunchKernelGGL(flag_signal_wait_kernel, dim3(1), dim3(64), 0, s, dw.sync.p + 2 * pend_sig, ep,
				make_flag_wait(ctx, dw.sync.p + 2 * need_wait_b + 1, ep));
		else if(need_wait_b >= 0)
			flag_wait(ctx, s, dw.sync.p + 2 * need_wait_b + 1, ep);
		else if(pend_sig >= 0)
			flag_signal(s, dw.sync.p + 2 * pend_sig, ep);
		need_wait_b = pend_sig = -1;
	};
	bool bulk_pending = false;
	const int fused = allow_fused ? switches().fused : 0;
	if(fused) {
		static uint64_t fattr_seen = 0;
		if(first_on_this_device(fattr_seen)) {
			SPP_HIP_CHECK(hipFuncSetAttribute((const void*)update_potrf_kernel, hipFuncAttributeMaxDynamicSharedMemorySize,
				POTRF_LDS_DOUBLES * (int)sizeof(double)));
		}
		if(dw.fuse_cnt.cap < (size_t)(nsteps + 2) || dw.fuse_dirty) {
			dw.fuse_cnt.reserve(std::max<size_t>((size_t)(nsteps + 2), 64));
			SPP_HIP_CHECK(hipMemsetAsync(dw.fuse_cnt.p, 0, dw.fuse_cnt.cap * sizeof(int), s));
			dw.fuse_expect.assign(dw.fuse_cnt.cap, 0);
			dw.fuse_dirty = false;
		}
	}
	static_assert(POTRF_LDS_DOUBLES >= (64 + 64) * FS_STRIDE, "the fused kernel's LDS is sized by the factorization");
	auto fused_update_potrf = [&](int64_t r0, int64_t m, int64_t kp0, int64_t kn) {
		const int64_t N = ncols - r0;
		if(m <= 0 || N <= 0)
			return false;
		const int64_t md = std::min<int64_t>(NB, m), nd = std::min<int64_t>(NB, N);
		const int ti = (int)((md + 31) / 32), tj = (int)((nd + 31) / 32);
		int nA = 0;
		for(int j = 0; j < tj; ++ j)
			nA += std::min(j, ti - 1) + 1;
		const int64_t nbi = (m + 63) / 64, nbj = (N + 63) / 64;
// ... 479 lines not shown
```

slam_plus_plus_amd/csrc/spp_dense_tail.h:

```cpp
#pragma once
#include "spp_dense_dev.h"

namespace spp {

constexpr int TAIL_MAX_ROWS = 64;

struct TailArgs {
	double *A;
	int64_t ld;
	int64_t rows;
	int64_t ncols;
	int64_t c0;
	int have_pre;
	int Tr, Tc;
	int has_rhs;
	double *tinv;
	double *dbuf;
	int *pub;
	int epoch;
	int *info, *abort;
	long long timeout_ticks;
	long long *trace;
	const int *order;
	unsigned long long rowbits[TAIL_MAX_ROWS + 1];
};

constexpr int TAIL_ABORT_TIMEOUT = 2;

constexpr int TAIL_LDS_DOUBLES = POTRF_LDS_DOUBLES_INV2 + 16;

#ifndef SPP_TAIL_PLAIN_LD
#define SPP_TAIL_PLAIN_LD 0
#endif
__device__ __forceinline__ double tail_ld(const double *p)
{
#if SPP_TAIL_PLAIN_LD
	return __hip_atomic_load(p, __ATOMIC_RELAXED, __HIP_MEMORY_SCOPE_WORKGROUP);
#else
	return __hip_atomic_load(p, __ATOMIC_RELAXED, __HIP_MEMORY_SCOPE_AGENT);
#endif
}

__device__ __noinline__ void tail_first_tile(double *sm, const v4f64 t00, const int lane, int *info, const int64_t k0)
{
	const int l15 = lane & 15, l4 = lane >> 4;
#pragma unroll
	for(int r = 0; r < 4; ++ r)
		sm[(l4 + 4 * r) + l15 * TS] = t00[r];
	if(lane == 0)
		potrf_lds2_fail(sm)[0] = 0;
	__builtin_amdgcn_fence(__ATOMIC_ACQ_REL, "wavefront");
	__builtin_amdgcn_wave_barrier();
	diag_tile_factor<TS>(sm, potrf_lds2_dv(sm), potrf_lds2_gd0(sm), potrf_lds2_dinv(sm), 0, lane, potrf_lds2_fail(sm), info, k0);
}

__global__ __launch_bounds__(POTRF_THREADS)
void dense_tail_kernel(const TailArgs a)
{
	extern __shared__ double sm[];
	const int tid = threadIdx.x, lane = tid & 63, wave = __builtin_amdgcn_readfirstlane(tid >> 6);
	const int l15 = lane & 15, l4 = lane >> 4;
	int *st = (int*)(sm + POTRF_LDS_DOUBLES_INV2);
	const int ord = a.order[blockIdx.x];
	const int ti = ord >> 16, tj = ord & 0xffff;
	const bool diag = ti == tj;
	const int64_t i0 = a.c0 + (int64_t)NB * ti, j0 = a.c0 + (int64_t)NB * tj;
	const int tag = a.epoch << 4;
	auto stamp = [&](int slot) { if(a.trace && tid == 0) a.trace[ti * 8 + slot] = wall_clock64(); };
	if(diag) stamp(0);
	auto pub_count = [&](const int v, const int w) -> int {
		const int cv = ((v >> 4) == a.epoch) ? (v & 15) : 0, cw = ((w >> 4) == a.epoch) ? (w & 15) : 0;
		return cv < cw ? cv : cw;
	};
	auto wait_pub = [&](const int *p, const int *q, const int need) -> int {
		if(tid == 0) {
			const long long t0 = wall_clock64();
			int got = -1;
			for(;;) {
				const int v = __hip_atomic_load(p, __ATOMIC_RELAXED, __HIP_MEMORY_SCOPE_AGENT);
				const int w = q ? __hip_atomic_load(q, __ATOMIC_RELAXED, __HIP_MEMORY_SCOPE_AGENT) : v;
				const int cv = ((v >> 4) == a.epoch) ? (v & 15) : 0, cw = ((w >> 4) == a.epoch) ? (w & 15) : 0;
				const int c = cv < cw ? cv : cw;
				if(c >= need) {
					got = c;
					break;
				}
				if(__hip_atomic_load(a.abort, __ATOMIC_RELAXED, __HIP_MEMORY_SCOPE_AGENT))
					break;
				if(wall_clock64() - t0 > a.timeout_ticks) {
					__hip_atomic_store(a.abort, TAIL_ABORT_TIMEOUT, __ATOMIC_RELAXED, __HIP_MEMORY_SCOPE_AGENT);
					break;
				}
				__builtin_amdgcn_s_sleep(1);
			}
			st[1] = got;
		}
		lds_barrier();
		const int got = st[1];
		lds_barrier();
		return got;
	};
	int ra[4], cb[4];
#pragma unroll
	for(int u = 0; u < 4; ++ u) {
		if(!diag) {
			ra[u] = wave & 7;
			cb[u] = 4 * (wave >> 3) + u;
		} else {
			int q = (wave == 0) ? (u == 0 ? 0 : 36) : wave + 15 * u, c = 0;
			if(q >= 36)
				ra[u] = cb[u] = -1;
			else {
				while(q > c) {
					q -= c + 1;
					++ c;
				}
				ra[u] = q;
				cb[u] = c;
			}
		}
	}
	v4f64 acc[4];
	{
		double *img = sm;
#pragma unroll 4
		for(int q = 0; q < NB * NB / POTRF_THREADS; ++ q) {
			const int e = tid + q * POTRF_THREADS, r = e & (NB - 1), c = e >> 7;
			const int64_t row = i0 + r, col = j0 + c;
			img[r + c * TS] = (col < a.ncols) ? a.A[row + col * a.ld] : ((diag && row == col) ? 1.0 : 0.0);
		}
		lds_barrier();
#pragma unroll
		for(int u = 0; u < 4; ++ u)
#pragma unroll
			for(int r = 0; r < 4; ++ r)
				acc[u][r] = (ra[u] < 0) ? 0.0 : img[(16 * ra[u] + l4 + 4 * r) + (16 * cb[u] + l15) * TS];
		lds_barrier();
	}
	bool pre_first = false;
	{
		const int ek = tid & 15, ec = tid >> 4;
		constexpr int PS = 18;
		const int ekp = 4 * (ek & 3) + (ek >> 2);
		const int kfirst = a.have_pre ? -1 : 0;
		unsigned long long steps = 0;
		for(int k = kfirst; k < ti; ++ k) {
			const unsigned long long w = a.rowbits[k + 1];
			if(((w >> ti) & (w >> tj) & 1) != 0)
				steps |= 1ull << (k - kfirst);
		}
		const int nst = 8 * __builtin_popcountll(steps);
		double va[2], vb[2];
		auto fetch = [&](const int k, const int J) {
			const double *rowp = a.A + (a.c0 + (int64_t)NB * k) + 16 * J + ek;
#pragma unroll
			for(int h = 0; h < 2; ++ h) {
				const int64_t ca = i0 + ec + 64 * h, cb = j0 + ec + 64 * h;
				va[h] = (ca < (diag ? a.ncols : a.rows)) ? tail_ld(rowp + ca * a.ld) : 0.0;
				vb[h] = (!diag && cb < a.ncols) ? tail_ld(rowp + cb * a.ld) : 0.0;
			}
		};
		int avail = a.have_pre ? 8 : 0;
		pre_first = diag && nst > 0 && (nst & 1) == 0 && a.rows - i0 >= 16;
		bool inflight = false;
		int k = kfirst;
		for(int sidx = 0; sidx < nst; ++ sidx) {
			const int J = sidx & 7;
			if(J == 0) {
				k = kfirst + __builtin_ctzll(steps);
				steps &= steps - 1;
			}
			if(J == 0 && k >= 0)
				avail = 0;
			if(!inflight) {
				if(J >= avail) {
					avail = wait_pub(a.pub + k * a.Tc + ti, a.pub + k * a.Tc + tj, J + 1);
					if(avail < 0)
						return;
				}
				fetch(k, J);
			}
			int pk = -1;
			if(tid == 0 && k >= 0 && J + 1 < 8 && J + 1 >= avail)
				pk = pub_count(__hip_atomic_load(a.pub + k * a.Tc + ti, __ATOMIC_RELAXED, __HIP_MEMORY_SCOPE_AGENT),
					__hip_atomic_load(a.pub + k * a.Tc + tj, __ATOMIC_RELAXED, __HIP_MEMORY_SCOPE_AGENT));
			double *sa = sm + (sidx & 1) * 2 * NB * PS, *sb = diag ? sa : sa + NB * PS;
#pragma unroll
			for(int h = 0; h < 2; ++ h) {
				sa[ekp + (ec + 64 * h) * PS] = va[h];
				if(!diag)
					sb[ekp + (ec + 64 * h) * PS] = vb[h];
			}
			if(tid == 0)
				st[2 + (sidx & 1)] = pk;
			lds_barrier();
			{
				const int seen = st[2 + (sidx & 1)];
				if(seen > avail)
					avail = seen;
			}
			inflight = (sidx + 1 < nst) && (J + 1 < 8) && (J + 1 < avail);
			if(inflight)
				fetch(k, J + 1);
			double fa[4];
#pragma unroll
			for(int u = 0; u < 4; ++ u) {
				if(ra[u] < 0)
					continue;
				double fb[4];
				if(u == 0 || diag) {
					const bool row_live = i0 + 16 * ra[u] + l15 < a.rows;
					const double2 a01 = *(const double2*)(sa + 4 * l4 + (16 * ra[u] + l15) * PS), a23 = *(const double2*)(sa + 4 * l4 + 2 + (16 * ra[u] + l15) * PS);
					fa[0] = row_live ? -a01.x : 0.0;
					fa[1] = row_live ? -a01.y : 0.0;
					fa[2] = row_live ? -a23.x : 0.0;
					fa[3] = row_live ? -a23.y : 0.0;
				}
				{
					const double2 b01 = *(const double2*)(sb + 4 * l4 + (16 * cb[u] + l15) * PS), b23 = *(const double2*)(sb + 4 * l4 + 2 + (16 * cb[u] + l15) * PS);
					fb[0] = b01.x;
					fb[1] = b01.y;
					fb[2] = b23.x;
					fb[3] = b23.y;
				}
#pragma unroll
				for(int kk = 0; kk < 4; ++ kk)
					acc[u] = __builtin_amdgcn_mfma_f64_16x16x4f64(fa[kk], fb[kk], acc[u], 0, 0, 0);
				if(u == 0 && pre_first && sidx == nst - 1 && wave == 0) {
					tail_first_tile(sm, acc[0], lane, a.info, i0);
				}
			}
		}
		lds_barrier();
	}
	if(diag) stamp(1);
	double *T = sm;
#pragma unroll
	for(int u = 0; u < 4; ++ u)
#pragma unroll
		for(int r = 0; r < 4; ++ r)
			if(ra[u] >= 0 && !(pre_first && wave == 0 && u == 0))
				T[(16 * ra[u] + l4 + 4 * r) + (16 * cb[u] + l15) * TS] = acc[u][r];
	lds_barrier();
	if(diag) {
		const int64_t nv = a.rows - i0;
		const int n_valid = (int)(nv < 0 ? 0 : (nv > NB ? NB : nv));
		PotrfPub pb;
		pb.flag = a.pub + ti * a.Tc + ti;
		pb.base = tag;
		pb.dbuf = a.dbuf + (size_t)ti * 8 * 256;
		pb.abort = a.abort;
		potrf_diag_body<false, 1, 2, true>(a.A + i0 + i0 * a.ld, a.ld, n_valid, (a.has_rhs && n_valid < NB) ? 1 : 0,
			a.tinv + (size_t)ti * NB * NB, a.info, i0, sm, pb, pre_first ? 1 : 0);
		stamp(2);
		return;
	}
	double *Dv = T + NB * TS;
	double *Rr = Dv + 16 * PT;
	const double *Rii = a.A + i0 + i0 * a.ld;
	int avail = 0;
	bool inflight = false;
	double dvr = 0, rr[2] = {0, 0};
	auto fetch_panel = [&](const int J) {
		if(tid < 256)
			dvr = tail_ld(a.dbuf + ((size_t)ti * 8 + J) * 256 + tid);
#pragma unroll
		for(int h = 0; h < 2; ++ h) {
			const int e = tid + POTRF_THREADS * h, k = e & 15, c = e >> 4;
			if(e < 16 * (NB - 16 * (J + 1)))
				rr[h] = tail_ld(Rii + (16 * J + k) + (int64_t)(16 * (J + 1) + c) * a.ld);
		}
	};
	for(int J = 0; J < 8; ++ J) {
		if(!inflight) {
			if(J >= avail) {
				avail = wait_pub(a.pub + ti * a.Tc + ti, nullptr, J + 1);
				if(avail < 0)
					return;
			}
			fetch_panel(J);
		}
		if(tj == ti + 1 && J == 0) stamp(3);
		if(tj == ti + 1 && J == 7) stamp(4);
		int pk = -1;
		if(tid == 0 && J + 1 < 8 && J + 1 >= avail) {
			const int v = __hip_atomic_load(a.pub + ti * a.Tc + ti, __ATOMIC_RELAXED, __HIP_MEMORY_SCOPE_AGENT);
			pk = pub_count(v, v);
		}
		if(tid < 256)
			Dv[(tid & 15) + (tid >> 4) * PT] = dvr;
#pragma unroll
		for(int h = 0; h < 2; ++ h) {
			const int e = tid + POTRF_THREADS * h;
			if(e < 16 * (NB - 16 * (J + 1)))
				Rr[(e & 15) + (e >> 4) * PT] = rr[h];
		}
		if(tid == 0)
			st[2 + (J & 1)] = pk;
		lds_barrier();
		{
			const int seen = st[2 + (J & 1)];
			if(seen > avail)
				avail = seen;
		}
		inflight = (J + 1 < 8) && (J + 1 < avail);
		if(inflight)
			fetch_panel(J + 1);
		if(wave < 8) {
			double *Y = T + 16 * J + (16 * wave) * TS;
			const v4f64 x = tile_atb(Dv, 1, PT, Y, 1, TS, lane);
			__builtin_amdgcn_fence(__ATOMIC_ACQ_REL, "wavefront");
			__builtin_amdgcn_wave_barrier();
			const int64_t col = j0 + 16 * wave + l15;
#pragma unroll
			for(int r = 0; r < 4; ++ r) {
				Y[(l4 + 4 * r) + l15 * TS] = x[r];
				if(col < a.ncols)
					__hip_atomic_store(&a.A[(i0 + 16 * J + l4 + 4 * r) + col * a.ld], x[r], __ATOMIC_RELAXED, __HIP_MEMORY_SCOPE_AGENT);
			}
		}
		lds_barrier();
		{
			const int b = wave & 7;
// ... 35 lines not shown
```

slam_plus_plus_amd/csrc/spp_internal.h:

```cpp
#pragma once

#include <hip/hip_runtime.h>
#include <stdint.h>
#include <string>
#include <vector>
#include <sys/mman.h>
#include <utility>
#include <new>
#include <exception>
#include <thread>
#include <stdexcept>
#include <algorithm>
#include <string.h>
#include <chrono>
#include <stdio.h>
#include <stdlib.h>
#include "../../include/spp_hip.h"
#include "spp_switches.h"

namespace spp {

struct Error : std::runtime_error {
	int code;
	Error(int c, const std::string &what) : std::runtime_error(what), code(c) {}
// ... 29 lines not shown
	}
};

template <class T>
struct HugeAlloc {
	typedef T value_type;
	HugeAlloc() {}
	template <class U> HugeAlloc(const HugeAlloc<U>&) {}
	T *allocate(size_t n)
	{
		const size_t bytes = n * sizeof(T), huge = (size_t)2 << 20;
		void *q = nullptr;
		if(bytes >= ((size_t)4 << 20)) {
			if(posix_memalign(&q, huge, (bytes + huge - 1) & ~(huge - 1)) != 0)
				q = nullptr;
#ifdef MADV_HUGEPAGE
			if(q)
				madvise(q, bytes, MADV_HUGEPAGE);
#endif
		}
		if(!q)
			q = malloc(bytes ? bytes : 1);
		if(!q)
			throw std::bad_alloc();
		return (T*)q;
	}
	void deallocate(T *p, size_t) { free(p); }
	template <class U> void construct(U *p) { ::new((void*)p) U; }
	template <class U, class A0, class... A> void construct(U *p, A0 &&a0, A &&... a) { ::new((void*)p) U(std::forward<A0>(a0), std::forward<A>(a)...); }
	template <class U> bool operator==(const HugeAlloc<U>&) const { return true; }
	template <class U> bool operator!=(const HugeAlloc<U>&) const { return false; }
};
template <class T> using HVec = std::vector<T, HugeAlloc<T> >;

template <class T>
struct DevBuf {
	T *p = nullptr;
	size_t cap = 0;
	bool owned = true;
	DevBuf() {}
	DevBuf(const DevBuf&) = delete;
	DevBuf &operator=(const DevBuf&) = delete;
	~DevBuf() { release(); }
	void release()
	{
		if(p && owned)
			(void)hipFree(p);
		p = nullptr;
		cap = 0;
		owned = true;
	}
	void view(T *ptr, size_t n)
	{
		release();
		p = ptr;
		cap = n;
		owned = false;
	}
	void reserve(size_t n)
	{
		if(n <= cap && owned)
			return;
		release();
		size_t want = n;
		hipError_t e = hipMalloc((void**)&p, want * sizeof(T));
		if(e != hipSuccess) {
			p = nullptr;
			throw Error(SPP_E_NOMEM, "hipMalloc of " + std::to_string(want * sizeof(T)) + " bytes failed");
		}
		cap = want;
	}
	template <class A>
	void upload(const std::vector<T, A> &h, hipStream_t s)
	{
		reserve(h.size() ? h.size() : 1);
		if(!h.empty())
			SPP_HIP_CHECK(hipMemcpyAsync(p, h.data(), h.size() * sizeof(T), hipMemcpyHostToDevice, s));
	}
};

struct UploadArena {
	hipStream_t stream;
	std::vector<unsigned char> host;
	struct Item { void **pp; size_t *pcap; bool *powned; size_t off, n; };
	std::vector<Item> items;
	explicit UploadArena(hipStream_t s) : stream(s) { host.reserve(size_t(1) << 20); }
	template <class T, class A>
	void add(DevBuf<T> &b, const std::vector<T, A> &v)
	{
		if(v.size() * sizeof(T) > (size_t(256) << 10)) {
			b.upload(v, stream);
			return;
		}
		b.release();
		const size_t off = (host.size() + 255) & ~(size_t)255, bytes = std::max<size_t>(v.size(), 1) * sizeof(T);
		host.resize(off + bytes);
		if(!v.empty())
			memcpy(host.data() + off, v.data(), v.size() * sizeof(T));
		Item it = {(void**)&b.p, &b.cap, &b.owned, off, std::max<size_t>(v.size(), 1)};
		items.push_back(it);
	}
	void commit(DevBuf<unsigned char> &store)
	{
		store.release();
		store.reserve(std::max<size_t>(host.size(), 256));
		if(!host.empty())
			SPP_HIP_CHECK(hipMemcpyAsync(store.p, host.data(), host.size(), hipMemcpyHostToDevice, stream));
		for(size_t i = 0; i < items.size(); ++ i) {
			*items[i].pp = store.p + items[i].off;
			*items[i].pcap = items[i].n;
			*items[i].powned = false;
		}
	}
};

struct Structure {
	int64_t nb = 0, n = 0, nnzb = 0, nvals = 0;
	HVec<int64_t> col_ptr, row_idx, blk_off, base;
	HVec<int32_t> dim;
};

struct SaccItem {
	int32_t beg, end;
	int32_t kind;
	int32_t a_tr;
	int64_t dst;
	int64_t aoff;
};

struct SchurDims {
	int dp = 0, dl = 0;
	int64_t nc = 0, nl = 0;
	int64_t nl_total = 0;
	int64_t no = 0;
	int64_t n_red = 0, ld = 0;
	int64_t n_sblk = 0;
	int64_t n_pairs = 0;
	int64_t n_items = 0, n_multi = 0;
	int32_t xcd_max_items = 0;
	bool u_landmark_major = true;
	bool factored = true;
};

struct SchurPlan : SchurDims {
	bool add_A = true;
	bool sparse_S = false;
	bool mis = false;
	Structure s_st;
	DevBuf<int64_t> sblk_voff;
	std::vector<int64_t> pose_block;
	std::vector<int64_t> lm_block;
	std::vector<uint8_t> is_lm;
	std::vector<uint64_t> tile_mask;
	DevBuf<int32_t> lm_ptr;
	DevBuf<int32_t> bs_ptr;
	int64_t n_bs = 0;
	int lm_stream_last = 0;
	DevBuf<int64_t> lm_coff;
	DevBuf<int64_t> lm_rbase;
	DevBuf<int32_t> obs_pose;
	DevBuf<int32_t> obs_lm;
	DevBuf<int64_t> obs_off;
	DevBuf<int64_t> pose_rbase;
	DevBuf<int32_t> cam_ptr;
	DevBuf<int32_t> cam_obs;
	DevBuf<int32_t> obs_wpos;
	DevBuf<SaccItem> items;
	DevBuf<int32_t> xcd_beg;
	DevBuf<int32_t> sblk_i1, sblk_i2;
	DevBuf<int64_t> sblk_aoff;
	DevBuf<int32_t> pair_a, pair_b;
	DevBuf<int32_t> multi_blk;
	DevBuf<int32_t> multi_ptr;
	DevBuf<double> cinv;
	DevBuf<double> lfac;
	DevBuf<double> W;
	DevBuf<double> Up;
	DevBuf<double> xw;
	DevBuf<double> partial;
	DevBuf<double> S;
	bool unlisted_dirty = true;
	bool side_pending = false, side_padded = false;
	int side_last = 0, clear_last = 0;
	int async_last = 0;
	void release_all();
};

struct DenseWork {
	DevBuf<double> tinv;
	DevBuf<int> info;
	DevBuf<double> tinv_all;
	int64_t tinv_half = 0;
	DevBuf<double> xtmp;
	DevBuf<int> flags;
	DevBuf<int> tail_pub;
	DevBuf<double> tail_dinv;
	int tail_epoch = 0;
	DevBuf<int> tail_order;
	std::vector<int> tail_order_host;
	int tail_order_tr = 0, tail_order_tc = 0;
	std::vector<uint64_t> tail_order_bits;
	bool tail_order_pre = false, tail_order_masked = false;
	int tail_resident = -1;
	const std::vector<uint64_t> *tile_mask = nullptr;
	bool tail_masked_whole = false;
	int tail_rows_last = 0;
	bool tail_disabled = false;
	DevBuf<double> trsv_m;
	DevBuf<double> trsv_pay;
	uint64_t epoch = 0;
	int *h_chain_err = nullptr;
	int *d_chain_err = nullptr;
	hipStream_t aux = nullptr;
	hipEvent_t ev[2] = {nullptr, nullptr};
	DevBuf<int> sync;
	DevBuf<int> fuse_cnt;
	std::vector<int> fuse_expect;
	bool fuse_dirty = false;
	int64_t ident_from = -1;
	hipStream_t chain = nullptr;
	hipEvent_t ev_chain = nullptr;
	DevBuf<int> la_cnt;
	DevBuf<long long> la_trace;
	int la_state = 0;
	int la_reserve = 0;
	int la_ncu = 0;
	int sync_epoch = 0;
	int sync_state = 0;
	hipStream_t sync_stream = nullptr;
};

struct SparsePlan;

struct AssemblePlan;

struct PhaseTimer {
	hipEvent_t ev[2 * SPP_N_PHASES];
	bool used[SPP_N_PHASES];
	bool created = false;
};

}

struct spp_ctx {
	int device = 0;
	int flags = 0;
	hipStream_t stream = nullptr;
	bool own_stream = false;
	hipStream_t side_stream = nullptr;
	hipEvent_t side_ev[2] = {nullptr, nullptr};
	hipEvent_t status_ev[2] = {nullptr, nullptr};
	int *h_status = nullptr;
	bool status_pending = false;
	std::string last_error;
	int mode = -1;
	int shard_rank = 0, shard_world = 1;
	spp::Structure st;
	std::vector<int64_t> order;
	std::thread plan_trash;
	spp::SchurPlan schur;
	spp::DenseWork dense;
	spp::SparsePlan *sparse = nullptr;
	spp::AssemblePlan *assemble = nullptr;
	spp::DevBuf<double> d_vals, d_rhs;
	double *h_staging = nullptr;
	size_t h_staging_cap = 0;
	spp::DevBuf<double> geom_partial;
	spp::PhaseTimer timer;
	double phase_ms[SPP_N_PHASES] = {0};
	std::vector<hipEvent_t> dom_events;
	size_t dom_used = 0;
	double dom_flops = 0;
	int64_t factor_flops = 0, solve_bytes = 0, factor_nnz = 0;
};

namespace spp {

void se2_linearize(spp_ctx *ctx, int64_t ne, const int32_t *d_v0, const int32_t *d_v1, const double *d_poses,
	const double *d_meas, double *d_J0, double *d_J1, double *d_r);
double se2_update(spp_ctx *ctx, int64_t nv, double *d_poses, const double *d_dx, bool apply);
void se2_linearize_at(spp_ctx *ctx, int64_t ne, const int64_t *d_off0, const int64_t *d_off1, const double *d_state,
	const double *d_meas, double *d_J0, double *d_J1, double *d_r);
void se2_rb_linearize(spp_ctx *ctx, int64_t ne, const int64_t *d_off0, const int64_t *d_off1, const double *d_state,
	const double *d_meas, double *d_J0, double *d_J1, double *d_r);
double slam2d_update(spp_ctx *ctx, int64_t n, double *d_state, const double *d_dx, int64_t n_angles,
	const int64_t *d_angle_off, bool apply);
void se3_linearize_at(spp_ctx *ctx, int64_t ne, const int64_t *d_off0, const int64_t *d_off1, const double *d_state,
	const double *d_meas, double *d_J0, double *d_J1, double *d_r);
void se3_xyz_linearize(spp_ctx *ctx, int64_t ne, const int64_t *d_pose_off, const int64_t *d_lm_off, const double *d_state,
	const double *d_meas, double *d_J0, double *d_J1, double *d_r);
double slam3d_update(spp_ctx *ctx, int64_t n, double *d_state, const double *d_dx, int64_t n_poses,
	const int64_t *d_pose_off, bool apply);
void rocv_range_linearize(spp_ctx *ctx, int64_t ne, const int64_t *d_recv_off, const int64_t *d_lm_off, const double *d_state,
	const double *d_meas, double *d_J0, double *d_J1, double *d_r);
void rocv_cv_linearize(spp_ctx *ctx, int64_t ne, const int64_t *d_off0, const int64_t *d_off1, const double *d_state,
	const double *d_dt, double *d_J0, double *d_J1, double *d_r);
double edge_chi2(spp_ctx *ctx, int64_t ne, int rd, const double *d_r, const double *d_Om);
void edge_robust_weights(spp_ctx *ctx, int64_t ne, int rd, int kind, double scale, double param, const double *d_r, double *d_w);
double edge_hessian_maxdiag(spp_ctx *ctx, int64_t ne, int rd, int d0, int d1, const double *d_J0, const double *d_J1,
	const double *d_Om);
double lm_gain_denominator(spp_ctx *ctx, int64_t n, const double *d_dx, const double *d_rhs, double alpha);
void se3_linearize(spp_ctx *ctx, int64_t ne, const int32_t *d_v0, const int32_t *d_v1, const double *d_poses,
	const double *d_meas, double *d_J0, double *d_J1, double *d_r);
double se3_update(spp_ctx *ctx, int64_t nv, double *d_poses, const double *d_dx, bool apply);
void ba_linearize(spp_ctx *ctx, int64_t no, const int32_t *d_cam_of, const int32_t *d_pt_of, const double *d_cams,
	const double *d_intr, const double *d_pts, const double *d_meas, double *d_J0, double *d_J1, double *d_r);
void ba_stereo_linearize(spp_ctx *ctx, int64_t no, const int32_t *d_cam_of, const int32_t *d_pt_of, const double *d_cams,
	const double *d_intr, const double *d_pts, const double *d_meas, double *d_J0, double *d_J1, double *d_r);
void ba_intrinsics_linearize(spp_ctx *ctx, int64_t no, const int32_t *d_cam_of, const int32_t *d_pt_of, const int32_t *d_intr_of,
	const double *d_cams, const double *d_intr, const double *d_pts, const double *d_meas, double *d_J0, double *d_J1, double *d_J2,
	double *d_r);
double ba_intrinsics_update(spp_ctx *ctx, int64_t ni, double *d_intr, const int64_t *d_intr_dxoff, const double *d_dx, bool apply);
double ba_update(spp_ctx *ctx, int64_t nc, double *d_cams, const int64_t *d_cam_dxoff, int64_t np, double *d_pts,
	const int64_t *d_pt_dxoff, const double *d_dx, int64_t n_dx, bool apply);
void sim3_ba_linearize(spp_ctx *ctx, int64_t no, const int32_t *d_cam_of, const int32_t *d_pt_of, const double *d_cams,
	const double *d_intr, const double *d_pts, const double *d_meas, double *d_J0, double *d_J1, double *d_r);
double sim3_update(spp_ctx *ctx, int64_t nc, double *d_cams, const int64_t *d_cam_dxoff, int64_t np, double *d_pts,
	const int64_t *d_pt_dxoff, const double *d_dx, int64_t n_dx, bool apply);

void min_degree_order(int64_t nb, const int64_t *col_ptr, const int64_t *row_idx, std::vector<int64_t> &order);
void nested_dissection_order(int64_t nb, const int64_t *col_ptr, const int64_t *row_idx, std::vector<int64_t> &order);

void tile_mask_mark(int64_t n, int bs, int64_t nblk, const int32_t *i1, const int32_t *i2, std::vector<uint64_t> &words);
int64_t tile_mask_close(int64_t n, bool has_rhs, bool fill, std::vector<uint64_t> &words);
constexpr double TAIL_MODEL_STEP_US = 36.5, TAIL_MODEL_UPDATE_US = 2.0, TAIL_MODEL_START_US = 45.0;
constexpr int TAIL_MODEL_RESIDENT = 256;
struct TileDagCost {
	int64_t tiles = 0, updates = 0, path = 0;
	double cost_us = 0;
};
TileDagCost tile_dag_cost(int64_t n, const std::vector<uint64_t> &filled, int resident);
void tail_order_table(const std::vector<uint64_t> &bits, int Tr, int Tc, bool have_pre, double beta, int resident, bool early,
	std::vector<int> &order, int *info);

void build_schur_plan(spp_ctx *ctx, bool sparse_S, bool mis = false);
int64_t schur_buffer_doubles(const spp_ctx *ctx);
bool schur_applicable(const Structure &st, int *dp, int *dl);
double schur_plan_host_probe(const Structure &st, int shard_rank, int shard_world, bool sparse_S, bool mis, int64_t *out);
void schur_tile_mask_host_probe(const Structure &st, std::vector<uint64_t> &words);
bool schur_cam_order_host_probe(const Structure &st, int shard_rank, int shard_world, bool sparse_S, bool mis, const int64_t *order_in,
	std::vector<int32_t> &cam_order, TileDagCost cost[2]);

void sparse_analyze(spp_ctx *ctx, const Structure &st);
int sparse_factor_solve(spp_ctx *ctx, const double *d_vals, double *d_rhs);
void sparse_release(spp_ctx *ctx);
void sparse_dag_disable(spp_ctx *ctx);
int64_t sparse_info(const spp_ctx *ctx, int what);
int64_t sparse_fronts(const spp_ctx *ctx, int64_t capacity, int32_t *h, int32_t *w, int32_t *pad, int32_t *cls, int32_t *level,
	int32_t *parent, int32_t *team);

constexpr int64_t SCHUR_SIDE_MIN_OBS = 500000;
void schur_form(spp_ctx *ctx, const double *d_vals, const double *d_rhs, double *d_S_rhs, bool one_call = false);
int schur_finish(spp_ctx *ctx, const double *d_vals, double *d_S_rhs, double *d_rhs);
void schur_pack(spp_ctx *ctx, double *S, double *packed, bool pack);

constexpr int DENSE_NB = 128;
int dense_potrf_upper(spp_ctx *ctx, double *d_A, int64_t n, int64_t ld, bool keep_inverses);
bool dense_potrf_upper_enqueue(spp_ctx *ctx, double *d_A, int64_t n, int64_t ld, bool info_reset = true);
int dense_info_fetch(spp_ctx *ctx, bool *dag_aborted = nullptr);
void dense_info_copy_on(spp_ctx *ctx, hipStream_t st, int *h_status4);
int dense_info_eval(spp_ctx *ctx, const int *h_status4, bool *dag_aborted = nullptr, bool drain_first = false);
void dense_potrs_upper(spp_ctx *ctx, const double *d_R, int64_t n, int64_t ld, double *d_b);
void dense_aux_park(int device, hipStream_t s);
void dense_factor_steps(spp_ctx *ctx, double *d_A, int64_t ld, int64_t n, int64_t rows, int64_t ncols,
	int64_t nsteps, bool has_rhs);
void dense_info_reset(spp_ctx *ctx);
void dense_info_ensure(spp_ctx *ctx);
void dense_info_reset_on(spp_ctx *ctx, hipStream_t st);
void dense_reserve(spp_ctx *ctx, int64_t nblk);

void dense_chain_check(spp_ctx *ctx);
void dense_set_padding(spp_ctx *ctx, double *d_A, int64_t ld, int64_t n);
void dense_set_padding_on(hipStream_t st, double *d_A, int64_t ld, int64_t n);
struct TileMaskGuard {
	DenseWork &d;
	TileMaskGuard(DenseWork &dw, const std::vector<uint64_t> *m) : d(dw) { d.tile_mask = (m && !m->empty()) ? m : nullptr; }
	~TileMaskGuard() { d.tile_mask = nullptr; }
};
int dense_front_factor(spp_ctx *ctx, double *d_F, int64_t ld, int64_t w, int64_t h, double *d_image);
bool dense_gemm_tn_sub(spp_ctx *ctx, int64_t m, int64_t n, int64_t k, const double *A, int64_t lda,
	const double *B, int64_t ldb, double *C, int64_t ldc, bool upper_only);
double microbench_copy(spp_ctx *ctx, size_t bytes, int iters);
double microbench_mfma_f64(spp_ctx *ctx, int iters);
double microbench_ctile(spp_ctx *ctx, int n, int iters);
double microbench_update(spp_ctx *ctx, int64_t m, int iters);

void assemble_analyze(spp_ctx *ctx, int64_t nv, const int32_t *dim, int n_groups, const int64_t *g_ne,
	const int64_t *const *g_v0, const int64_t *const *g_v1, const int64_t *const *g_seq, const int *g_d0, const int *g_d1,
	const int *g_rd, int64_t unary_vertex, const uint8_t *skip_vertex = nullptr);
int assemble_n_groups(const spp_ctx *ctx);
int64_t assemble_group_edges(const spp_ctx *ctx, int group);
bool assemble_group_is_unary(const spp_ctx *ctx, int group);
void assemble_run(spp_ctx *ctx, const double *J0, const double *J1, const double *Om, const double *r,
	double damping, double *vals, double *eta);
void assemble_groups_run(spp_ctx *ctx, const double *const *J0, const double *const *J1, const double *const *Om,
	const double *const *r, double damping, double *vals, double *eta);
void assemble_set_edge_weights(spp_ctx *ctx, int group, const double *d_w);
void assemble_release(spp_ctx *ctx);
bool assemble_is_ternary(const spp_ctx *ctx);
constexpr int ASM_HUB_CHUNK = 4096;
void assemble_analyze_ternary(spp_ctx *ctx, int64_t nv, const int32_t *dim, int64_t ne, const int64_t *v0, const int64_t *v1,
	const int64_t *v2, int64_t unary_vertex);
void assemble_ternary_run(spp_ctx *ctx, const double *J0, const double *J1, const double *J2, const double *Om, const double *r,
	double damping, double *vals, double *eta);
void assemble_get_structure(const spp_ctx *ctx, int64_t *col_ptr, int64_t *row_idx, int64_t *blk_off);

void phase_begin(spp_ctx *ctx, int phase);
void phase_end(spp_ctx *ctx, int phase);
void phases_reset(spp_ctx *ctx);
void phases_collect(spp_ctx *ctx);
void dom_begin(spp_ctx *ctx);
void dom_end(spp_ctx *ctx, double flops);

template <class F>
inline void run_threads(int nt, F fn)
{
	if(nt <= 1) {
		fn(0);
		return;
	}
	std::vector<std::thread> th;
	std::exception_ptr err[64];
	for(int t = 1; t < nt; ++ t)
		th.emplace_back([&, t]() { try { fn(t); } catch(...) { err[t] = std::current_exception(); } });
	try { fn(0); } catch(...) { err[0] = std::current_exception(); }
	for(size_t t = 0; t < th.size(); ++ t)
		th[t].join();
	for(int t = 0; t < nt; ++ t)
		if(err[t])
			std::rethrow_exception(err[t]);
}

inline int plan_threads(int64_t work)
{
	const int env = switches().plan_threads;
	int nt = env ? env : (int)std::min<unsigned>(16u, std::max(1u, std::thread::hardware_concurrency()));
	if(work < switches().plan_min_work)
		nt = 1;
	return std::min(nt, 64);
}

template <class V>
inline void balanced_cuts(const V &w_prefix, int nt, std::vector<int64_t> &cut)
{
	const int64_t n = (int64_t)w_prefix.size() - 1, total = w_prefix[n];
	cut.assign(nt + 1, n);
	cut[0] = 0;
	for(int t = 1; t < nt; ++ t)
		cut[t] = std::lower_bound(w_prefix.begin(), w_prefix.end(), total * t / nt) - w_prefix.begin();
	for(int t = 1; t <= nt; ++ t)
		cut[t] = std::max(cut[t], cut[t - 1]);
	cut[nt] = n;
}


}
```

slam_plus_plus_amd/csrc/spp_schur.hip:

```cpp

#include "spp_internal.h"

namespace spp {

template <int DL>
__device__ __forceinline__ void cinv_block(const double *__restrict__ m, double *o)
{
	if(DL == 3) {
#define M_(i, j) m[(i) + 3 * (j)]
#define COF_(i, j) (M_(((i) + 1) % 3, ((j) + 1) % 3) * M_(((i) + 2) % 3, ((j) + 2) % 3) - \
	M_(((i) + 1) % 3, ((j) + 2) % 3) * M_(((i) + 2) % 3, ((j) + 1) % 3))
		const double c00 = COF_(0, 0), c10 = COF_(1, 0), c20 = COF_(2, 0);
		const double det = c00 * M_(0, 0) + c10 * M_(1, 0) + c20 * M_(2, 0);
		const double id = -1.0 / det;
		o[0] = c00 * id; o[3] = c10 * id; o[6] = c20 * id;
		o[1] = COF_(0, 1) * id; o[4] = COF_(1, 1) * id; o[7] = COF_(2, 1) * id;
		o[2] = COF_(0, 2) * id; o[5] = COF_(1, 2) * id; o[8] = COF_(2, 2) * id;
#undef COF_
#undef M_
	} else if(DL == 2) {
		const double det = m[0] * m[3] - m[2] * m[1];
		const double id = -1.0 / det;
		o[0] = m[3] * id; o[2] = -m[2] * id;
		o[1] = -m[1] * id; o[3] = m[0] * id;
// ... 1083 lines not shown
		SPP_HIP_CHECK(hipEventCreateWithFlags(&ctx->status_ev[0], hipEventDisableTiming));
	if(!ctx->status_ev[1])
		SPP_HIP_CHECK(hipEventCreateWithFlags(&ctx->status_ev[1], hipEventDisableTiming));
	SPP_HIP_CHECK(hipHostMalloc((void**)&ctx->h_status, 4 * sizeof(int), hipHostMallocDefault));
}

static void side_stream_join(spp_ctx *ctx)
{
	if(!ctx->schur.side_pending)
		return;
	SPP_HIP_CHECK(hipStreamWaitEvent(ctx->stream, ctx->side_ev[1], 0));
	ctx->schur.side_pending = false;
}

static bool stream_capturing(hipStream_t s)
{
	hipStreamCaptureStatus cs = hipStreamCaptureStatusNone;
	return hipStreamIsCapturing(s, &cs) != hipSuccess || cs != hipStreamCaptureStatusNone;
}

template <int DP, int DL>
static void schur_form_t(spp_ctx *ctx, const double *d_vals, const double *d_rhs, double *S, bool one_call)
{
	SchurPlan &sp = ctx->schur;
	hipStream_t s = ctx->stream;
	const int64_t ld = sp.ld;
	const int64_t *voff = sp.sparse_S ? sp.sblk_voff.p : nullptr;
	double *xcol = sp.sparse_S ? S + sp.s_st.nvals : S + sp.n_red * ld;
	side_stream_join(ctx);
	sp.side_padded = false;
	phase_begin(ctx, SPP_PHASE_SCHUR_INV);
	const bool own_dense = S == sp.S.p && !sp.sparse_S && ctx->shard_world == 1;
	const int64_t n_trows = ld / 128;
	if(own_dense && sp.n_sblk == sp.nc * (sp.nc + 1) / 2 && sp.n_red == sp.nc * DP) {
		SPP_HIP_CHECK(hipMemsetAsync(S + sp.n_red * ld, 0, (size_t)(schur_buffer_doubles(ctx) - sp.n_red * ld) * sizeof(double), s));
		sp.clear_last = 2;
	} else if(own_dense && !sp.unlisted_dirty && !sp.tile_mask.empty() && (int64_t)sp.tile_mask.size() <= n_trows && n_trows <= 64) {
		ClearArgs ca;
		memset(ca.rowbits, 0, sizeof(ca.rowbits));
		for(size_t q = 0; q < sp.tile_mask.size(); ++ q)
			ca.rowbits[q] = sp.tile_mask[q];
		ca.n_rows = (int)sp.tile_mask.size();
		hipLaunchKernelGGL(s_clear_tiles_kernel, dim3((unsigned)n_trows, (unsigned)n_trows), dim3(256), 0, s, S, ld, ca);
		sp.clear_last = 1;
	} else {
		SPP_HIP_CHECK(hipMemsetAsync(S, 0, (size_t)schur_buffer_doubles(ctx) * sizeof(double), s));
		sp.clear_last = 0;
		if(own_dense)
			sp.unlisted_dirty = false;
	}
	constexpr int VIL = VSplit<DP * DL>::IL;
	double *Vm = sp.W.p, *Vs = sp.W.p + sp.no * VIL;
	const bool onfly = sp.factored && DL <= 3;
	if(sp.nl && !onfly)
		hipLaunchKernelGGL((cinv_kernel<DL>), dim3((unsigned)((sp.nl + 255) / 256)), dim3(256), 0, s,
			sp.nl, sp.lm_coff.p, d_vals, sp.cinv.p, sp.factored ? sp.lfac.p : nullptr);
	const int lm_stream = lm_stream_form<DP, DL>(sp);
	sp.lm_stream_last = lm_stream;
	const double *lfac_arg = onfly ? (const double*)nullptr : (const double*)sp.lfac.p;
	const dim3 obs_grid((unsigned)((sp.no + 255) / 256));
	if(sp.no && lm_stream)
		launch_obs_fact_stream<DP, DL>(lm_stream == 1, obs_grid, s, sp.no, sp.obs_lm.p, sp.obs_off.p, sp.lm_rbase.p, d_vals, d_rhs, lfac_arg,
			sp.lm_coff.p, sp.obs_wpos.p, Vm, Vs, sp.xw.p);
	else if(sp.no && sp.factored)
		hipLaunchKernelGGL((obs_fact_kernel<DP, DL>), obs_grid, dim3(256), 0, s,
			sp.no, sp.obs_lm.p, sp.obs_off.p, sp.lm_rbase.p, d_vals, d_rhs, lfac_arg, sp.lm_coff.p,
			sp.obs_wpos.p, Vm, Vs, sp.xw.p);
	else if(sp.no)
		hipLaunchKernelGGL((obs_kernel<DP, DL>), obs_grid, dim3(256), 0, s,
			sp.no, sp.obs_lm.p, sp.obs_off.p, sp.lm_rbase.p, d_vals, d_rhs, sp.cinv.p, sp.obs_wpos.p, sp.W.p, sp.Up.p, sp.xw.p, sp.u_landmark_major ? 1 : 0);
	phase_end(ctx, SPP_PHASE_SCHUR_INV);
	const int side_sw = switches().schur_side;
	const bool side = side_sw != 0 && sp.nc > 0 && (side_sw == 2 || sp.no >= SCHUR_SIDE_MIN_OBS) &&
		!(ctx->flags & SPP_FLAG_PROFILE) && !stream_capturing(s);
	sp.side_last = side ? 1 : 0;
	auto launch_rhs = [&](hipStream_t st) {
		if(sp.nc && lm_stream == 1)
			hipLaunchKernelGGL((rhs_kernel<DP, true>), dim3((unsigned)((sp.nc + 3) / 4)), dim3(256), 0, st,
				sp.nc, sp.cam_ptr.p, sp.cam_obs.p, sp.pose_rbase.p, sp.xw.p, d_rhs, sp.add_A ? 1 : 0, xcol);
		else if(sp.nc)
			hipLaunchKernelGGL((rhs_kernel<DP, false>), dim3((unsigned)((sp.nc + 3) / 4)), dim3(256), 0, st,
				sp.nc, sp.cam_ptr.p, sp.cam_obs.p, sp.pose_rbase.p, sp.xw.p, d_rhs, sp.add_A ? 1 : 0, xcol);
	};
	if(side) {
		side_stream_ensure(ctx);
		const bool pad_here = one_call && own_dense;
		if(pad_here)
			dense_info_ensure(ctx);
		SPP_HIP_CHECK(hipEventRecord(ctx->side_ev[0], s));
		SPP_HIP_CHECK(hipStreamWaitEvent(ctx->side_stream, ctx->side_ev[0], 0));
		launch_rhs(ctx->side_stream);
		if(pad_here) {
			dense_set_padding_on(ctx->side_stream, S, ld, sp.n_red);
			dense_info_reset_on(ctx, ctx->side_stream);
			sp.side_padded = true;
		}
		SPP_HIP_CHECK(hipEventRecord(ctx->side_ev[1], ctx->side_stream));
		sp.side_pending = true;
	}
	phase_begin(ctx, SPP_PHASE_SCHUR_GEMM);
	if(sp.n_items) {
		int chunk = switches().sacc_chunk;
		if(chunk <= 0)
			chunk = (int)((sp.xcd_max_items + SACC_WAVES * 64 - 1) / (SACC_WAVES * 64));
		const int64_t per = (int64_t)SACC_WAVES * chunk;
		if(sp.factored)
			hipLaunchKernelGGL((s_accum_kernel<DP, DL, true>), dim3((unsigned)(8 * ((sp.xcd_max_items + per - 1) / per))), dim3(SACC_WAVES * 64), 0, s,
				sp.items.p, sp.xcd_beg.p, chunk, sp.pair_a.p, sp.pair_b.p, Vm, Vs, d_vals, S, ld, sp.partial.p);
		else
			hipLaunchKernelGGL((s_accum_kernel<DP, DL, false>), dim3((unsigned)(8 * ((sp.xcd_max_items + per - 1) / per))), dim3(SACC_WAVES * 64), 0, s,
				sp.items.p, sp.xcd_beg.p, chunk, sp.pair_a.p, sp.pair_b.p, sp.W.p, sp.Up.p, d_vals, S, ld, sp.partial.p);
	}
	if(sp.n_multi)
		hipLaunchKernelGGL((s_multi_kernel<DP>), dim3((unsigned)((sp.n_multi + 3) / 4)), dim3(256), 0, s,
			sp.n_multi, sp.multi_blk.p, sp.multi_ptr.p, sp.sblk_i1.p, sp.sblk_i2.p, sp.sblk_aoff.p,
			sp.partial.p, d_vals, sp.add_A ? 1 : 0, S, ld, voff);
	phase_end(ctx, SPP_PHASE_SCHUR_GEMM);
	phase_begin(ctx, SPP_PHASE_SCHUR_RHS);
	if(!side)
		launch_rhs(s);
	else if(!one_call)
		side_stream_join(ctx);
	phase_end(ctx, SPP_PHASE_SCHUR_RHS);
	SPP_HIP_CHECK(hipGetLastError());
}

template <int DP, int DL>
static int schur_finish_t(spp_ctx *ctx, const double *d_vals, double *S, double *d_rhs)
{
	SchurPlan &sp = ctx->schur;
	hipStream_t s = ctx->stream;
	const int64_t ld = sp.ld;
	double *xcol;
	side_stream_join(ctx);
	const bool early = !sp.sparse_S && switches().solve_async != 0 && !(ctx->flags & SPP_FLAG_PROFILE) && !stream_capturing(s);
	sp.async_last = early ? 1 : 0;
	if(early) {
		status_ensure(ctx);
		if(ctx->status_pending) {
			SPP_HIP_CHECK(hipStreamSynchronize(ctx->side_stream));
			ctx->status_pending = false;
		}
	}
	if(sp.sparse_S) {
		xcol = S + sp.s_st.nvals;
		const int ret = sparse_factor_solve(ctx, S, xcol);
		if(ret != SPP_OK)
			return ret;
	} else {
		phase_begin(ctx, SPP_PHASE_FACTOR);
		if(!sp.side_padded)
			dense_set_padding(ctx, S, ld, sp.n_red);
		{
			TileMaskGuard guard(ctx->dense, &sp.tile_mask);
			const bool own = S == sp.S.p;
			if(own)
				sp.unlisted_dirty = true;
			const bool masked_whole = dense_potrf_upper_enqueue(ctx, S, sp.n_red, ld, !sp.side_padded);
			if(own && masked_whole)
				sp.unlisted_dirty = false;
		}
		sp.side_padded = false;
		if(early) {
			SPP_HIP_CHECK(hipEventRecord(ctx->status_ev[0], s));
			SPP_HIP_CHECK(hipStreamWaitEvent(ctx->side_stream, ctx->status_ev[0], 0));
			dense_info_copy_on(ctx, ctx->side_stream, ctx->h_status);
			SPP_HIP_CHECK(hipEventRecord(ctx->status_ev[1], ctx->side_stream));
			ctx->status_pending = true;
		}
		phase_end(ctx, SPP_PHASE_FACTOR);
		xcol = S + sp.n_red * ld;
		phase_begin(ctx, SPP_PHASE_TRISOLVE);
		dense_potrs_upper(ctx, S, sp.n_red, ld, xcol);
		phase_end(ctx, SPP_PHASE_TRISOLVE);
	}
	phase_begin(ctx, SPP_PHASE_BACKSUBST);
	static_assert(DL <= DP, "the products U^T dx reuse the W l buffer (DP doubles per observation)");
	const int bs_fused = switches().backsubst_fused;
	const double *cinv_arg = (sp.factored && DL <= 3) ? (const double*)nullptr : (const double*)sp.cinv.p;
	const int32_t bs_per = (sp.n_bs >= 1024) ? 4 : 1;
	const bool bs_stream = bs_fused && sp.n_bs > 0 && lm_stream_form<DP, DL>(sp);
	const int32_t bs_scatter = bs_stream ? (int32_t)((sp.nc * DP + BS_SCATTER_PER - 1) / BS_SCATTER_PER) : 0;
	if(bs_stream)
		launch_backsubst_stream<DP, DL>(dim3((unsigned)((sp.n_bs + bs_per - 1) / bs_per + bs_scatter)), s,
			(int32_t)sp.n_bs, bs_per, (const int32_t*)sp.bs_ptr.p, (const int32_t*)sp.lm_ptr.p, (const int32_t*)sp.obs_pose.p, (const int64_t*)sp.obs_off.p,
			(const int64_t*)sp.lm_rbase.p, cinv_arg, (const int64_t*)sp.lm_coff.p, d_vals, (const double*)xcol, d_rhs,
			bs_scatter, (int64_t)sp.nc, (const int64_t*)sp.pose_rbase.p);
	else if(bs_fused && sp.n_bs > 0)
		hipLaunchKernelGGL((backsubst_fused_kernel<DP, DL>), dim3((unsigned)sp.n_bs), dim3(256), 0, s,
			sp.bs_ptr.p, sp.lm_ptr.p, sp.obs_pose.p, sp.obs_off.p, sp.lm_rbase.p, cinv_arg, sp.lm_coff.p, d_vals, xcol, d_rhs);
	else {
		if(sp.no)
			hipLaunchKernelGGL((backsubst_obs_kernel<DP, DL>), dim3((unsigned)((sp.no + 255) / 256)), dim3(256), 0, s,
				sp.no, sp.obs_pose.p, sp.obs_off.p, d_vals, xcol, sp.xw.p);
		if(sp.nl)
			hipLaunchKernelGGL((backsubst_lm_kernel<DL>), dim3((unsigned)((sp.nl + 255) / 256)), dim3(256), 0, s,
				sp.nl, sp.lm_ptr.p, sp.lm_rbase.p, sp.xw.p, cinv_arg, sp.lm_coff.p, d_vals, d_rhs);
	}
	if(sp.nc && !bs_stream)
		hipLaunchKernelGGL((scatter_dx_kernel<DP>), dim3((unsigned)((sp.nc * DP + 255) / 256)), dim3(256), 0, s,
			sp.nc, sp.pose_rbase.p, xcol, d_rhs);
	phase_end(ctx, SPP_PHASE_BACKSUBST);
	SPP_HIP_CHECK(hipGetLastError());
	if(early) {
		SPP_HIP_CHECK(hipEventSynchronize(ctx->status_ev[1]));
		ctx->status_pending = false;
		return dense_info_eval(ctx, ctx->h_status, nullptr, true) ? SPP_NOT_POSDEF : SPP_OK;
	}
	if(!sp.sparse_S && dense_info_fetch(ctx))
		return SPP_NOT_POSDEF;
	return SPP_OK;
}

template <bool PACK>
__global__ __launch_bounds__(256)
void schur_pack_kernel(double *__restrict__ S, int64_t ld, double *__restrict__ packed)
{
	const int64_t k = blockIdx.y;
	const int64_t rows = 128 * (k + 1);
	const int64_t e = (int64_t)blockIdx.x * 256 + threadIdx.x;
	if(e >= rows * 128)
		return;
	const int64_t r = e % rows, c = e / rows;
	double *ps = S + r + (128 * k + c) * ld;
	double *pp = packed + 128 * 128 * (k * (k + 1) / 2) + e;
	if(PACK)
		*pp = *ps;
	else
		*ps = *pp;
}

void schur_pack(spp_ctx *ctx, double *S, double *packed, bool pack)
{
	const int64_t ld = ctx->schur.ld, nblk = ld / 128;
	dim3 grid((unsigned)((ld * 128 + 255) / 256), (unsigned)nblk);
	if(pack)
		hipLaunchKernelGGL((schur_pack_kernel<true>), grid, dim3(256), 0, ctx->stream, S, ld, packed);
	else
		hipLaunchKernelGGL((schur_pack_kernel<false>), grid, dim3(256), 0, ctx->stream, S, ld, packed);
	SPP_HIP_CHECK(hipGetLastError());
}

void schur_form(spp_ctx *ctx, const double *d_vals, const double *d_rhs, double *d_S_rhs, bool one_call)
{
	const int dp = ctx->schur.dp, dl = ctx->schur.dl;
	if(dp == 6 && dl == 3) schur_form_t<6, 3>(ctx, d_vals, d_rhs, d_S_rhs, one_call);
	else if(dp == 3 && dl == 2) schur_form_t<3, 2>(ctx, d_vals, d_rhs, d_S_rhs, one_call);
	else if(dp == 3 && dl == 3) schur_form_t<3, 3>(ctx, d_vals, d_rhs, d_S_rhs, one_call);
	else if(dp == 6 && dl == 6) schur_form_t<6, 6>(ctx, d_vals, d_rhs, d_S_rhs, one_call);
	else if(dp == 7 && dl == 3) schur_form_t<7, 3>(ctx, d_vals, d_rhs, d_S_rhs, one_call);
	else throw Error(SPP_E_UNSUPPORTED, "Schur kernels: block widths not instantiated");
}

int schur_finish(spp_ctx *ctx, const double *d_vals, double *d_S_rhs, double *d_rhs)
{
	const int dp = ctx->schur.dp, dl = ctx->schur.dl;
	if(dp == 6 && dl == 3) return schur_finish_t<6, 3>(ctx, d_vals, d_S_rhs, d_rhs);
	if(dp == 3 && dl == 2) return schur_finish_t<3, 2>(ctx, d_vals, d_S_rhs, d_rhs);
	if(dp == 3 && dl == 3) return schur_finish_t<3, 3>(ctx, d_vals, d_S_rhs, d_rhs);
	if(dp == 6 && dl == 6) return schur_finish_t<6, 6>(ctx, d_vals, d_S_rhs, d_rhs);
	if(dp == 7 && dl == 3) return schur_finish_t<7, 3>(ctx, d_vals, d_S_rhs, d_rhs);
	throw Error(SPP_E_UNSUPPORTED, "Schur kernels: block widths not instantiated");
}

}
```

slam_plus_plus_amd/csrc/spp_schur_plan.cpp:

```cpp

#include "spp_internal.h"
#include <sys/mman.h>
#include <stdlib.h>
#include <algorithm>
#include <numeric>
#include <string.h>
#include <stdio.h>
#include <thread>
#include <memory>
#include <chrono>
#include <exception>

namespace spp {

void SchurPlan::release_all()
{
	lm_ptr.release(); bs_ptr.release(); n_bs = 0; lm_coff.release(); lm_rbase.release(); obs_pose.release(); obs_lm.release();
	obs_off.release(); pose_rbase.release(); cam_ptr.release(); cam_obs.release(); items.release();
	obs_wpos.release(); xcd_beg.release(); sblk_i1.release(); sblk_i2.release(); sblk_aoff.release();
	sblk_voff.release(); s_st = Structure(); sparse_S = false; mis = false;
	pair_a.release(); pair_b.release(); multi_blk.release(); multi_ptr.release(); cinv.release(); lfac.release();
	W.release(); Up.release(); xw.release(); partial.release(); S.release();
	pose_block.clear(); lm_block.clear(); is_lm.clear(); tile_mask.clear();
}

bool schur_applicable(const Structure &st, int *dp_out, int *dl_out)
{
	int d_a = -1, d_b = -1;
	for(int64_t j = 0; j < st.nb; ++ j) {
		int d = st.dim[j];
		if(d_a < 0 || d == d_a) d_a = d;
		else if(d_b < 0 || d == d_b) d_b = d;
		else return false;
	}
	if(d_a < 0 || d_b < 0)
		return false;
	int dp = std::max(d_a, d_b), dl = std::min(d_a, d_b);
	if(!((dp == 6 && dl == 3) || (dp == 3 && dl == 2) || (dp == 7 && dl == 3)))
		return false;
	int64_t n_lm = 0;
	for(int64_t j = 0; j < st.nb; ++ j) {
		if(st.dim[j] == dl)
			++ n_lm;
		for(int64_t p = st.col_ptr[j]; p < st.col_ptr[j + 1]; ++ p) {
			int64_t i = st.row_idx[p];
			if(i != j && st.dim[i] == dl && st.dim[j] == dl)
				return false;
		}
	}
	if(n_lm == 0)
		return false;
	*dp_out = dp;
	*dl_out = dl;
	return true;
}

static const int PAIR_CHUNK = 2048;

int64_t schur_buffer_doubles(const spp_ctx *ctx)
{
	const SchurPlan &sp = ctx->schur;
	return sp.sparse_S ? sp.s_st.nvals + sp.n_red : sp.ld * sp.ld;
}

static bool mis_partition(const Structure &st, std::vector<uint8_t> &is_lm, int *d_out)
{
	const int d = st.dim[0];
	for(int64_t j = 0; j < st.nb; ++ j)
		if(st.dim[j] != d)
			return false;
	if(d != 3 && d != 6)
		return false;
	std::vector<std::vector<int32_t> > adj(st.nb);
	for(int64_t j = 0; j < st.nb; ++ j)
		for(int64_t p = st.col_ptr[j]; p < st.col_ptr[j + 1]; ++ p) {
			const int64_t i = st.row_idx[p];
			if(i != j) {
				adj[i].push_back((int32_t)j);
				adj[j].push_back((int32_t)i);
			}
		}
	std::vector<int32_t> order(st.nb);
	for(int64_t j = 0; j < st.nb; ++ j)
		order[j] = (int32_t)j;
	std::stable_sort(order.begin(), order.end(), [&](int32_t a, int32_t b) { return adj[a].size() < adj[b].size(); });
	is_lm.assign(st.nb, 0);
	std::vector<uint8_t> blocked(st.nb, 0);
	int64_t n_lm = 0;
	for(int64_t q = 0; q < st.nb; ++ q) {
		const int32_t v = order[q];
		if(blocked[v])
			continue;
		is_lm[v] = 1;
		++ n_lm;
		for(size_t e = 0; e < adj[v].size(); ++ e)
			blocked[adj[v][e]] = 1;
	}
	*d_out = d;
	return n_lm > 0 && n_lm < st.nb;
}

template <class T>
struct RawBuf {
	T *p = nullptr;
	size_t n = 0;
	RawBuf() {}
	RawBuf(const RawBuf&) = delete;
	RawBuf &operator=(const RawBuf&) = delete;
	~RawBuf() { free(p); }
	void resize(size_t m)
	{
		free(p);
		p = nullptr;
		if(m) {
			const size_t bytes = m * sizeof(T);
			if(bytes >= ((size_t)8 << 20)) {
				void *q = nullptr;
				if(posix_memalign(&q, (size_t)2 << 20, (bytes + (((size_t)2 << 20) - 1)) & ~(((size_t)2 << 20) - 1)) == 0) {
					p = (T*)q;
#ifdef MADV_HUGEPAGE
					madvise(q, bytes, MADV_HUGEPAGE);
#endif
				}
			}
			if(!p)
				p = (T*)malloc(bytes);
			if(!p)
				throw std::bad_alloc();
		}
		n = m;
	}
	size_t size() const { return n; }
	T &operator[](size_t i) { return p[i]; }
	const T &operator[](size_t i) const { return p[i]; }
};

static void schur_tile_mask(const Structure &st, const std::vector<uint8_t> &is_lm, const std::vector<int32_t> &pose_of,
	int dp, int64_t n_red, std::vector<uint64_t> &words)
{
	tile_mask_mark(n_red, dp, 0, nullptr, nullptr, words);
	if(words.empty())
		return;
	const int64_t Tr = (int64_t)words.size();
	auto tiles_of = [&](int32_t pose) -> uint64_t {
		return (1ull << ((int64_t)pose * dp / DENSE_NB)) | (1ull << (((int64_t)pose * dp + dp - 1) / DENSE_NB));
	};
	auto mark = [&](uint64_t rows, const uint64_t cols) {
		for(; rows; rows &= rows - 1) {
			const int a = __builtin_ctzll(rows);
			if(a < Tr)
				words[a] |= cols;
		}
	};
	std::vector<uint64_t> seen(st.nb, 0);
	for(int64_t j = 0; j < st.nb; ++ j)
		for(int64_t p = st.col_ptr[j]; p < st.col_ptr[j + 1]; ++ p) {
			const int64_t i = st.row_idx[p];
			if(!is_lm[i] && !is_lm[j])
				mark(tiles_of(pose_of[i]), tiles_of(pose_of[j])), mark(tiles_of(pose_of[j]), tiles_of(pose_of[i]));
			else if(!is_lm[i])
				seen[j] |= tiles_of(pose_of[i]);
			else if(!is_lm[j])
				seen[i] |= tiles_of(pose_of[j]);
		}
	for(int64_t j = 0; j < st.nb; ++ j)
		if(seen[j])
			mark(seen[j], seen[j]);
	tile_mask_close(n_red, true, true, words);
}

struct CamGraph {
	int64_t nc = 0, nw = 0;
	std::vector<uint64_t> bits;
	uint64_t *row(int64_t c) { return bits.data() + c * nw; }
	const uint64_t *row(int64_t c) const { return bits.data() + c * nw; }
};
// ... 132 lines not shown
	auto flood = [&](const Set &within, Set &comp) {
		Set front(comp), nb;
		for(;;) {
			nbrs(front, nb);
			bool grew = false;
			for(int64_t w = 0; w < nw; ++ w) {
				front[w] = nb[w] & within[w] & ~comp[w];
				comp[w] |= front[w];
				grew = grew || front[w];
			}
			if(!grew)
				return;
		}
	};
	auto first_bit = [&](const Set &x, Set &seed) {
		seed.assign((size_t)nw, 0);
		for(int64_t w = 0; w < nw; ++ w)
			if(x[w]) {
				seed[w] = x[w] & (~x[w] + 1);
				return true;
			}
		return false;
	};
	Set all((size_t)nw, 0);
	for(int64_t c = 0; c < nc; ++ c)
		all[c >> 6] |= 1ull << (c & 63);
	if(!((g.row(0)[(nc - 1) >> 6] >> ((nc - 1) & 63)) & 1))
		return false;
	struct Cand { int64_t shorter = 0, sep = 0, runs = 0, a = 0, m = 0; } best;
	Set A((size_t)nw), S, B((size_t)nw), bestA, bestB, comp;
	const int64_t stride = std::max<int64_t>(1, al / 8);
	for(int64_t m = al; 2 * m <= nc; m += al)
		for(int64_t a = 0; a + m <= nc; a += stride) {
			std::fill(A.begin(), A.end(), 0);
			for(int64_t c = a; c < a + m; ++ c)
				A[c >> 6] |= 1ull << (c & 63);
			nbrs(A, S);
			for(int64_t w = 0; w < nw; ++ w) {
				S[w] &= ~A[w];
				B[w] = all[w] & ~A[w] & ~S[w];
			}
			const int64_t nB = count(B), nBal = nB - nB % al;
			if(nBal == 0)
				continue;
			Cand cd;
			cd.shorter = std::min(m, nBal);
			cd.sep = nc - m - nBal;
			cd.a = a;
			cd.m = m;
			for(int64_t c = 0; c < nc; ++ c)
				cd.runs += ((B[c >> 6] >> (c & 63)) & 1) && !(c && ((B[(c - 1) >> 6] >> ((c - 1) & 63)) & 1));
			if(best.m && !(cd.shorter > best.shorter || (cd.shorter == best.shorter && (cd.sep < best.sep ||
			   (cd.sep == best.sep && cd.runs < best.runs)))))
				continue;
			first_bit(B, comp);
			flood(B, comp);
			if(comp != B)
				continue;
			best = cd;
			bestA = A;
			bestB = B;
		}
	if(switches().verbose)
		fprintf(stderr, "[spp] camera order: best arc a %lld m %lld shorter %lld sep %lld runs %lld\n", (long long)best.a,
			(long long)best.m, (long long)best.shorter, (long long)best.sep, (long long)best.runs);
	if(!best.m)
		return false;
	const int64_t nBal = count(bestB) - count(bestB) % al;
	std::vector<int32_t> cand_order;
	cand_order.reserve((size_t)nc);
	std::vector<uint8_t> placed((size_t)nc, 0);
	for(int64_t c = 0; c < nc; ++ c)
		if((bestA[c >> 6] >> (c & 63)) & 1) {
			cand_order.push_back((int32_t)c);
			placed[c] = 1;
		}
	for(int64_t c = 0, k = 0; c < nc && k < nBal; ++ c)
		if((bestB[c >> 6] >> (c & 63)) & 1) {
			cand_order.push_back((int32_t)c);
			placed[c] = 1;
			++ k;
		}
	for(int64_t c = 0; c < nc; ++ c)
		if(!placed[c])
			cand_order.push_back((int32_t)c);
	for(int64_t q = 0; q < nc; ++ q)
		pos[cand_order[q]] = (int32_t)q;
	cam_graph_mask(g, pos, dp, n_red, words);
	const TileDagCost c1 = tile_dag_cost(n_red, words, TAIL_MODEL_RESIDENT);
	const bool live_ok = cam_order_live_ok(words, n_red);
	if(switches().verbose)
		fprintf(stderr, "[spp] camera order: candidate tiles %lld updates %lld chain %lld model %.0f us (natural %.0f), live ok %d\n",
			(long long)c1.tiles, (long long)c1.updates, (long long)c1.path, c1.cost_us, cost[0].cost_us, (int)live_ok);
	if(!(c1.cost_us <= 0.9 * cost[0].cost_us) || !live_ok)
		return false;
	cost[1] = c1;
	order.swap(cand_order);
	return true;
}

static bool schur_cam_order(const Structure &st, const std::vector<uint8_t> &is_lm, const std::vector<int32_t> &cam_of, int64_t nc,
	int dp, bool sparse_S, bool mis, const int64_t *order_in, std::vector<int32_t> &cam_order, TileDagCost cost[2])
{
	cam_order.resize((size_t)nc);
	for(int64_t c = 0; c < nc; ++ c)
		cam_order[c] = (int32_t)c;
	cost[0] = cost[1] = TileDagCost();
	const int64_t n_red = nc * dp;
	if(sparse_S || mis || n_red / DENSE_NB + 1 > 64 || nc < 2 || (!order_in && !switches().schur_cam_order))
		return false;
	VClock clk("camera order");
	CamGraph g;
	cam_graph(st, is_lm, cam_of, nc, g);
	clk.lap("co-visibility graph");
	if(order_in) {
		std::vector<int32_t> pos((size_t)nc);
		for(int64_t q = 0; q < nc; ++ q) {
			cam_order[q] = (int32_t)order_in[q];
			pos[order_in[q]] = (int32_t)q;
		}
		std::vector<uint64_t> words;
		for(int side = 0; side < 2; ++ side) {
			if(!side)
				for(int64_t c = 0; c < nc; ++ c)
					pos[c] = (int32_t)c;
			else
				for(int64_t q = 0; q < nc; ++ q)
					pos[order_in[q]] = (int32_t)q;
			cam_graph_mask(g, pos, dp, n_red, words);
			cost[side] = tile_dag_cost(n_red, words, TAIL_MODEL_RESIDENT);
		}
		return false;
	}
	const bool used = cam_dissect(g, dp, n_red, cam_order, cost);
	clk.lap("dissection + cost model");
	return used;
}

struct SchurPlanHost : SchurDims {
	int64_t n_ablk = 0;
	int32_t n_slots = 0;
	std::vector<int64_t> pose_block, lm_block;
	std::vector<uint8_t> is_lm;
	HVec<int32_t> lm_ptr, obs_pose, obs_lm, cam_obs, wpos;
	std::vector<int32_t> bs_ptr;
	std::vector<int32_t> cam_ptr, sblk_i1, sblk_i2, multi_blk, multi_ptr, xb;
	RawBuf<int32_t> pair_a, pair_b;
	HVec<int64_t> lm_coff, obs_off, lm_rbase;
	std::vector<int64_t> sblk_aoff, sblk_voff, pose_rbase;
	std::vector<SaccItem> recs;
	Structure s_st;
	std::vector<uint64_t> tile_mask;
	TileDagCost cam_cost[2];
};

struct Obs { int32_t lm, pose; int64_t off; };
struct ABlk { int32_t i1, i2; int64_t off; };

struct PlanScratch {
	std::vector<int32_t> pose_of, lm_of;
	std::vector<ABlk> ablk;
	bool obs_sorted = true;
	std::vector<std::vector<int32_t> > foreign_cols;
	HVec<int32_t> cam_end;
	std::vector<int64_t> sblk_beg;
	std::vector<int32_t> item_blk, item_beg, item_end, item_slot;
};

static void schur_partition(const Structure &st, int shard_rank, int shard_world, bool mis, SchurPlanHost &h, PlanScratch &w)
{
	int dp, dl;
	std::vector<uint8_t> &is_lm = h.is_lm;
	if(mis) {
		SPP_REQUIRE(mis_partition(st, is_lm, &dp), SPP_E_UNSUPPORTED,
			"MIS Schur mode needs a graph of one block width (3 or 6) with at least one edge");
		dl = dp;
	} else {
		SPP_REQUIRE(schur_applicable(st, &dp, &dl), SPP_E_UNSUPPORTED,
			"Schur mode needs exactly two block widths ({6,3} or {3,2}) and a block-diagonal landmark part");
		is_lm.assign(st.nb, 0);
		for(int64_t j = 0; j < st.nb; ++ j)
			is_lm[j] = st.dim[j] == dl;
	}
	h.dp = dp;
	h.dl = dl;

	std::vector<int32_t> &pose_of = w.pose_of, &lm_of = w.lm_of;
	pose_of.assign(st.nb, -1);
	lm_of.assign(st.nb, -1);
	int64_t nc = 0, nl_total = 0, nl = 0;
	for(int64_t j = 0; j < st.nb; ++ j) {
		if(!is_lm[j]) {
			pose_of[j] = (int32_t)nc ++;
			h.pose_block.push_back(j);
		} else {
			if(nl_total % shard_world == shard_rank) {
				lm_of[j] = (int32_t)nl ++;
				h.lm_block.push_back(j);
			}
			++ nl_total;
		}
	}
	h.nc = nc;
	h.nl = nl;
	h.nl_total = nl_total;
}

static void apply_cam_order(const Structure &st, bool sparse_S, bool mis, SchurPlanHost &h, PlanScratch &w)
{
	const int dp = h.dp;
	const int64_t nc = h.nc;
	const std::vector<uint8_t> &is_lm = h.is_lm;
	std::vector<int32_t> &pose_of = w.pose_of;
	std::vector<int32_t> cam_order;
	if(schur_cam_order(st, is_lm, pose_of, nc, dp, sparse_S, mis, nullptr, cam_order, h.cam_cost)) {
		const std::vector<int64_t> natural(h.pose_block);
		for(int64_t q = 0; q < nc; ++ q) {
			h.pose_block[q] = natural[cam_order[q]];
			pose_of[h.pose_block[q]] = (int32_t)q;
		}
		if(switches().verbose)
			fprintf(stderr, "[spp] camera order: tiles %lld -> %lld, updates %lld -> %lld, chain %lld -> %lld, model %.0f -> %.0f us\n",
				(long long)h.cam_cost[0].tiles, (long long)h.cam_cost[1].tiles, (long long)h.cam_cost[0].updates,
				(long long)h.cam_cost[1].updates, (long long)h.cam_cost[0].path, (long long)h.cam_cost[1].path,
				h.cam_cost[0].cost_us, h.cam_cost[1].cost_us);
	}
}

static void scan_columns(const Structure &st, SchurPlanHost &h, PlanScratch &w)
{
	const int64_t nl = h.nl;
	const std::vector<uint8_t> &is_lm = h.is_lm;
	const std::vector<int32_t> &pose_of = w.pose_of, &lm_of = w.lm_of;
	HVec<int64_t> &lm_coff = h.lm_coff;
	lm_coff.assign(nl, -1);
	std::vector<ABlk> &ablk = w.ablk;
	HVec<int32_t> &lm_ptr = h.lm_ptr, &obs_pose = h.obs_pose, &obs_lm = h.obs_lm;
	HVec<int64_t> &obs_off = h.obs_off;
	bool &obs_sorted = w.obs_sorted;
	const int nts = plan_threads(st.nnzb);
	std::vector<int64_t> jcut;
	balanced_cuts(st.col_ptr, nts, jcut);
	{
		std::vector<int64_t> n_obs_t(nts + 1, 0), n_ab_t(nts + 1, 0);
		auto classify = [&](int64_t j, int64_t p, Obs &o) -> int {
			const int64_t i = st.row_idx[p];
			const bool pi = !is_lm[i], pj = !is_lm[j];
			if(pi && pj)
				return 0;
			if(!pi && !pj)
				return 1;
			if(pi) {
				if(lm_of[j] < 0)
					return 3;
				o = {lm_of[j], pose_of[i], st.blk_off[p] << 1};
			} else {
				if(lm_of[i] < 0)
					return 3;
				o = {lm_of[i], pose_of[j], (st.blk_off[p] << 1) | 1};
			}
			return 2;
		};
		run_threads(nts, [&](int t) {
			int64_t n_o = 0, n_a = 0;
			Obs o;
			for(int64_t j = jcut[t]; j < jcut[t + 1]; ++ j)
				for(int64_t p = st.col_ptr[j]; p < st.col_ptr[j + 1]; ++ p) {
					const int k = classify(j, p, o);
					n_o += k == 2;
					n_a += k == 0;
				}
			n_obs_t[t + 1] = n_o;
			n_ab_t[t + 1] = n_a;
		});
		for(int t = 0; t < nts; ++ t) {
			n_obs_t[t + 1] += n_obs_t[t];
			n_ab_t[t + 1] += n_ab_t[t];
		}
		const int64_t no_all = n_obs_t[nts];
		SPP_REQUIRE(no_all < (int64_t(1) << 31), SPP_E_UNSUPPORTED, "too many observations for 32-bit obs indices");
		obs_pose.resize(no_all);
		obs_lm.resize(no_all);
		obs_off.resize(no_all);
		ablk.resize(n_ab_t[nts]);
		std::vector<char> sorted_t(nts, 1);
		run_threads(nts, [&](int t) {
			int64_t a = n_obs_t[t], q = n_ab_t[t];
			Obs o, prev = {-1, -1, 0};
			bool sorted = true;
			for(int64_t j = jcut[t]; j < jcut[t + 1]; ++ j)
				for(int64_t p = st.col_ptr[j]; p < st.col_ptr[j + 1]; ++ p) {
					const int k = classify(j, p, o);
					if(k == 0) {
						const int32_t pi = pose_of[st.row_idx[p]], pj = pose_of[j];
						ablk[q ++] = pi <= pj ? ABlk{pi, pj, st.blk_off[p]} : ABlk{pj, pi, -2 - st.blk_off[p]};
					}
					else if(k == 1) {
						if(lm_of[j] >= 0)
							lm_coff[lm_of[j]] = st.blk_off[p];
					} else if(k == 2) {
						if(o.lm < prev.lm || (o.lm == prev.lm && o.pose < prev.pose))
							sorted = false;
						prev = o;
						obs_lm[a] = o.lm;
						obs_pose[a] = o.pose;
						obs_off[a] = o.off;
						++ a;
					}
				}
			sorted_t[t] = sorted;
		});
		for(int t = 0; t < nts; ++ t)
			obs_sorted = obs_sorted && sorted_t[t];
		for(int t = 1; t < nts && obs_sorted; ++ t) {
			const int64_t a = n_obs_t[t];
			if(a > 0 && a < no_all && (obs_lm[a] < obs_lm[a - 1] || (obs_lm[a] == obs_lm[a - 1] && obs_pose[a] < obs_pose[a - 1])))
				obs_sorted = false;
		}
	}
	h.n_ablk = (int64_t)ablk.size();
	for(int64_t l = 0; l < nl; ++ l)
		SPP_REQUIRE(lm_coff[l] >= 0, SPP_E_BADARG, "landmark without a diagonal block");
}

static void foreign_columns(const Structure &st, const SchurPlanHost &h, PlanScratch &w)
{
	const int64_t nc = h.nc;
	const std::vector<uint8_t> &is_lm = h.is_lm;
	const std::vector<int32_t> &pose_of = w.pose_of, &lm_of = w.lm_of;
	std::vector<std::vector<int32_t> > &foreign_cols = w.foreign_cols;
	std::vector<int64_t> lm_gidx(st.nb, -1);
	int64_t g = 0;
	for(int64_t j = 0; j < st.nb; ++ j)
		if(is_lm[j])
			lm_gidx[j] = g ++;
	std::vector<std::vector<int32_t> > poses_of(g);
	for(int64_t j = 0; j < st.nb; ++ j)
		for(int64_t p = st.col_ptr[j]; p < st.col_ptr[j + 1]; ++ p) {
			const int64_t i = st.row_idx[p];
			const bool pi = !is_lm[i], pj = !is_lm[j];
			if(pi && !pj && lm_of[j] < 0)
				poses_of[lm_gidx[j]].push_back(pose_of[i]);
			else if(!pi && pj && lm_of[i] < 0)
				poses_of[lm_gidx[i]].push_back(pose_of[j]);
		}
	foreign_cols.resize(nc);
	for(int64_t l = 0; l < g; ++ l) {
		std::vector<int32_t> &ps = poses_of[l];
		std::sort(ps.begin(), ps.end());
		for(size_t a = 0; a < ps.size(); ++ a)
			for(size_t b = a + 1; b < ps.size(); ++ b)
				foreign_cols[ps[a]].push_back(ps[b]);
	}
	for(int64_t c = 0; c < nc; ++ c) {
		std::sort(foreign_cols[c].begin(), foreign_cols[c].end());
		foreign_cols[c].erase(std::unique(foreign_cols[c].begin(), foreign_cols[c].end()), foreign_cols[c].end());
	}
}

static void order_observations(SchurPlanHost &h, const PlanScratch &w)
{
	const int64_t nl = h.nl;
	const bool obs_sorted = w.obs_sorted;
	HVec<int32_t> &lm_ptr = h.lm_ptr, &obs_pose = h.obs_pose, &obs_lm = h.obs_lm;
	HVec<int64_t> &obs_off = h.obs_off;
	const int64_t no = (int64_t)obs_pose.size();
	h.no = no;
	bool lm_sorted = true;
// ... 310 lines not shown
		}
		for(int64_t c = 0; c < nchunk; ++ c) {
			item_blk.push_back((int32_t)b);
			item_beg.push_back((int32_t)(beg + c * PAIR_CHUNK));
			item_end.push_back((int32_t)std::min<int64_t>(end, beg + (c + 1) * PAIR_CHUNK));
			item_slot.push_back(nchunk > 1 ? n_slots ++ : -1);
		}
	}
	multi_ptr.push_back(n_slots);
	h.n_slots = n_slots;
	bool interleave = false;
	std::vector<int32_t> xb_il;
	{
		const int64_t tb_env = switches().sacc_tile, tbc_env = switches().sacc_tile_cols;
		const int64_t TB = tb_env, TBC = (tbc_env == -2) ? TB : (tbc_env <= 0 ? nc : tbc_env), ntile = (nc + TBC - 1) / TBC;
		std::vector<int32_t> perm(item_blk.size());
		for(size_t q = 0; q < perm.size(); ++ q)
			perm[q] = (int32_t)q;
		interleave = switches().sacc_xcd != 0;
		std::vector<int64_t> tile_of_item(item_blk.size());
		for(size_t q = 0; q < tile_of_item.size(); ++ q)
			tile_of_item[q] = (sblk_i1[item_blk[q]] / TB) * ntile + sblk_i2[item_blk[q]] / TBC;
		auto tile_of = [&](int32_t q) { return tile_of_item[q]; };
		auto stable_by_key = [&](std::vector<int32_t> &pm, int64_t n_keys, auto key_of) {
			if(n_keys > 8 * (int64_t)pm.size() + 1024) {
				std::stable_sort(pm.begin(), pm.end(), [&](int32_t x, int32_t y) { return key_of(x) < key_of(y); });
				return;
			}
			std::vector<int32_t> start((size_t)n_keys + 1, 0), out(pm.size());
			for(size_t q = 0; q < pm.size(); ++ q)
				++ start[key_of(pm[q]) + 1];
			for(int64_t k = 0; k < n_keys; ++ k)
				start[k + 1] += start[k];
			for(size_t q = 0; q < pm.size(); ++ q)
				out[start[key_of(pm[q])] ++] = pm[q];
			pm.swap(out);
		};
		stable_by_key(perm, ((nc + TB - 1) / TB) * ntile, tile_of);
		if(interleave) {
			std::vector<int32_t> xcd_of(perm.size());
			int64_t load[8] = {0, 0, 0, 0, 0, 0, 0, 0};
			for(size_t q = 0; q < perm.size();) {
				const int64_t t = tile_of(perm[q]);
				size_t e = q;
				int64_t cost = 0;
				for(; e < perm.size() && tile_of(perm[e]) == t; ++ e)
					cost += 2 + (item_end[perm[e]] - item_beg[perm[e]] + 63) / 64;
				int x = 0;
				for(int y = 1; y < 8; ++ y)
					if(load[y] < load[x])
						x = y;
				load[x] += cost;
				for(size_t i = q; i < e; ++ i)
					xcd_of[perm[i]] = x;
				q = e;
			}
			stable_by_key(perm, 8, [&](int32_t x) { return (int64_t)xcd_of[x]; });
			xb_il.assign(9, 0);
			for(size_t q = 0; q < perm.size(); ++ q)
				++ xb_il[xcd_of[q] + 1];
			for(int x = 0; x < 8; ++ x)
				xb_il[x + 1] += xb_il[x];
		}
		std::vector<int32_t> t_blk(perm.size()), t_beg(perm.size()), t_end(perm.size()), t_slot(perm.size());
		for(size_t q = 0; q < perm.size(); ++ q) {
			t_blk[q] = item_blk[perm[q]];
			t_beg[q] = item_beg[perm[q]];
			t_end[q] = item_end[perm[q]];
			t_slot[q] = item_slot[perm[q]];
		}
		item_blk.swap(t_blk); item_beg.swap(t_beg); item_end.swap(t_end); item_slot.swap(t_slot);
	}
	h.n_items = (int64_t)item_blk.size();
	{
		std::vector<int32_t> &xb = h.xb;
		xb.assign(9, 0);
		if(interleave)
			xb = xb_il;
		else {
			std::vector<int64_t> cost(h.n_items + 1, 0);
			for(int64_t q = 0; q < h.n_items; ++ q)
				cost[q + 1] = cost[q] + 2 + (item_end[q] - item_beg[q] + 63) / 64;
			for(int x = 1; x < 8; ++ x)
				xb[x] = (int32_t)(std::lower_bound(cost.begin(), cost.end(), cost[h.n_items] * x / 8) - cost.begin());
			xb[8] = (int32_t)h.n_items;
		}
		h.xcd_max_items = 0;
		for(int x = 0; x < 8; ++ x) {
			xb[x + 1] = std::max(xb[x + 1], xb[x]);
			h.xcd_max_items = std::max(h.xcd_max_items, xb[x + 1] - xb[x]);
		}
	}
	h.n_multi = (int64_t)multi_blk.size();
}

static void rhs_offsets(const Structure &st, SchurPlanHost &h)
{
	const int64_t nc = h.nc, nl = h.nl;
	h.pose_rbase.resize(nc);
	h.lm_rbase.resize(nl);
	for(int64_t c = 0; c < nc; ++ c)
		h.pose_rbase[c] = st.base[h.pose_block[c]];
	for(int64_t l = 0; l < nl; ++ l)
		h.lm_rbase[l] = st.base[h.lm_block[l]];
}

static void item_records(bool add_A, bool sparse_S, SchurPlanHost &h, const PlanScratch &w)
{
	const int dp = h.dp;
	const std::vector<int32_t> &sblk_i1 = h.sblk_i1, &sblk_i2 = h.sblk_i2;
	const std::vector<int64_t> &sblk_aoff = h.sblk_aoff;
	const std::vector<int32_t> &item_blk = w.item_blk, &item_beg = w.item_beg, &item_end = w.item_end, &item_slot = w.item_slot;
	h.recs.resize(item_blk.size());
	for(size_t q = 0; q < h.recs.size(); ++ q) {
		const int32_t b = item_blk[q];
		SaccItem &r = h.recs[q];
		r.beg = item_beg[q];
		r.end = item_end[q];
		r.a_tr = 0;
		r.aoff = -1;
		if(item_slot[q] >= 0) {
			r.kind = 2;
			r.dst = (int64_t)item_slot[q] * dp * dp;
		} else {
			r.aoff = add_A ? sblk_aoff[b] : -1;
			if(r.aoff < -1) {
				r.aoff = -2 - r.aoff;
				r.a_tr = 1;
			}
			if(sparse_S) {
				r.kind = 1;
				r.dst = h.sblk_voff[b];
			} else {
				r.kind = 0;
				r.dst = (int64_t)sblk_i1[b] * dp + (int64_t)sblk_i2[b] * dp * h.ld;
			}
		}
	}
}

static void schur_plan_host(const Structure &st, int shard_rank, int shard_world, bool sparse_S, bool mis, SchurPlanHost &h)
{
	VClock clk("schur plan");
	PlanScratch w;
	schur_partition(st, shard_rank, shard_world, mis, h, w);
	apply_cam_order(st, sparse_S, mis, h, w);
	clk.lap("camera order");
	h.n_red = h.nc * h.dp;
	h.ld = ((h.n_red + 1 + DENSE_NB - 1) / DENSE_NB) * DENSE_NB;
	SPP_REQUIRE(sparse_S || h.ld <= 65536, SPP_E_UNSUPPORTED,
		"reduced camera system too large for the dense path (use SPP_MODE_SCHUR_SPARSE)");
	if(!sparse_S)
		schur_tile_mask(st, h.is_lm, w.pose_of, h.dp, h.n_red, h.tile_mask);
	scan_columns(st, h, w);
	clk.lap("partition + observation scan");
	if(sparse_S && shard_world > 1)
		foreign_columns(st, h, w);
	order_observations(h, w);
	backsubst_groups(h);
	camera_lists(h, w);
	clk.lap("observation / camera lists");
	alloc_pair_lists(h);
	clk.lap("pair list buffers");
	s_pattern_and_pairs(h, w, clk);
	if(sparse_S)
		sparse_s_structure(h);
	clk.lap("block lists");
	work_items(h, w);
	rhs_offsets(st, h);
	clk.lap("work items");
	item_records(shard_rank == 0, sparse_S, h, w);
	clk.lap("item records");
}

void build_schur_plan(spp_ctx *ctx, bool sparse_S, bool mis)
{
	const Structure &st = ctx->st;
	SchurPlan &sp = ctx->schur;
	sp.release_all();
	sp.sparse_S = sparse_S;
	hipStream_t s = ctx->stream;
	VClock clk0("schur plan (device)");
	std::unique_ptr<SchurPlanHost> hp(new SchurPlanHost);
	SchurPlanHost &h = *hp;
	clk0.lap("old plan released");
	schur_plan_host(st, ctx->shard_rank, ctx->shard_world, sparse_S, mis, h);
	VClock clk("schur plan (device)");
	const int dp = h.dp, dl = h.dl;
	const int64_t nl = h.nl, no = h.no;
	static_cast<SchurDims &>(sp) = h;
	sp.pose_block.swap(h.pose_block);
	sp.lm_block.swap(h.lm_block);
	sp.is_lm.swap(h.is_lm);
	sp.add_A = (ctx->shard_rank == 0);
	sp.tile_mask.swap(h.tile_mask);
	if(sparse_S) {
		sp.s_st = h.s_st;
		sp.sblk_voff.upload(h.sblk_voff, s);
	}

	sp.xcd_beg.upload(h.xb, s);
	sp.lm_ptr.upload(h.lm_ptr, s);
	sp.n_bs = h.bs_ptr.empty() ? 0 : (int64_t)h.bs_ptr.size() - 1;
	sp.bs_ptr.upload(h.bs_ptr, s);
	sp.lm_coff.upload(h.lm_coff, s);
	sp.lm_rbase.upload(h.lm_rbase, s);
	sp.obs_pose.upload(h.obs_pose, s);
	sp.obs_lm.upload(h.obs_lm, s);
	sp.obs_off.upload(h.obs_off, s);
	sp.pose_rbase.upload(h.pose_rbase, s);
	sp.cam_ptr.upload(h.cam_ptr, s);
	sp.cam_obs.upload(h.cam_obs, s);
	sp.items.upload(h.recs, s);
	sp.obs_wpos.upload(h.wpos, s);
	sp.sblk_i1.upload(h.sblk_i1, s);
	sp.sblk_i2.upload(h.sblk_i2, s);
	sp.sblk_aoff.upload(h.sblk_aoff, s);
	sp.pair_a.reserve(std::max<size_t>(1, h.pair_a.size()));
	sp.pair_b.reserve(std::max<size_t>(1, h.pair_b.size()));
	if(h.pair_a.size()) {
		SPP_HIP_CHECK(hipMemcpyAsync(sp.pair_a.p, h.pair_a.p, h.pair_a.size() * sizeof(int32_t), hipMemcpyHostToDevice, s));
		SPP_HIP_CHECK(hipMemcpyAsync(sp.pair_b.p, h.pair_b.p, h.pair_b.size() * sizeof(int32_t), hipMemcpyHostToDevice, s));
	}
	sp.multi_blk.upload(h.multi_blk, s);
	sp.multi_ptr.upload(h.multi_ptr, s);
	clk.lap("uploads enqueued");
	sp.cinv.reserve((size_t)std::max<int64_t>(1, nl) * dl * dl);
	sp.W.reserve((size_t)std::max<int64_t>(1, no) * dp * dl);
	if(sp.factored)
		sp.lfac.reserve((size_t)std::max<int64_t>(1, nl) * dl * dl);
	else
		sp.Up.reserve((size_t)std::max<int64_t>(1, no) * dp * dl);
	sp.xw.reserve((size_t)std::max<int64_t>(1, no) * dp);
	sp.partial.reserve((size_t)std::max<int32_t>(1, h.n_slots) * dp * dp);
	clk.lap("workspaces allocated");
	SPP_HIP_CHECK(hipStreamSynchronize(s));
	clk.lap("uploads done");

	if(!sparse_S)
		dense_reserve(ctx, (sp.n_red + DENSE_NB - 1) / DENSE_NB);
	clk.lap("dense workspaces");

	const double n = (double)sp.n_red;
	ctx->factor_flops = (int64_t)(n * n * n / 3.0 + 2.0 * n * n);
	ctx->factor_nnz = sp.ld * sp.ld;
	const int64_t blk_pl = 8 * dp * dl, blk_pp = 8 * dp * dp, blk_ll = 8 * dl * dl;
	ctx->solve_bytes = blk_pl * no + blk_ll * nl + blk_pp * h.n_ablk + 8 * st.n
		+ blk_pp * sp.n_sblk + 8 * st.n
		+ 8 * sp.n_red * sp.n_red ;
	if(ctx->plan_trash.joinable())
		ctx->plan_trash.join();
	{
		SchurPlanHost *raw = hp.release();
		try {
			ctx->plan_trash = std::thread([raw]() { delete raw; });
		} catch(...) {
			delete raw;
		}
	}
	clk.lap("host plan handed to the releasing thread");
}

double schur_plan_host_probe(const Structure &st, int shard_rank, int shard_world, bool sparse_S, bool mis, int64_t *out)
{
	const auto t0 = std::chrono::steady_clock::now();
	SchurPlanHost h;
	schur_plan_host(st, shard_rank, shard_world, sparse_S || mis, mis, h);
	const double sec = std::chrono::duration<double>(std::chrono::steady_clock::now() - t0).count();
	uint64_t sum = 1469598103934665603ull;
	auto mix = [&](uint64_t v) { sum = (sum ^ v) * 1099511628211ull; };
	for(size_t q = 0; q < h.pair_a.size(); ++ q)
		mix(((uint64_t)(uint32_t)h.pair_a[q] << 32) | (uint32_t)h.pair_b[q]);
	for(size_t q = 0; q < h.sblk_i1.size(); ++ q) {
		mix(((uint64_t)(uint32_t)h.sblk_i1[q] << 32) | (uint32_t)h.sblk_i2[q]);
		mix((uint64_t)h.sblk_aoff[q]);
	}
	for(size_t q = 0; q < h.recs.size(); ++ q) {
		mix(((uint64_t)(uint32_t)h.recs[q].beg << 32) | (uint32_t)h.recs[q].end);
		mix((uint64_t)h.recs[q].dst);
		mix((uint64_t)h.recs[q].aoff + (uint64_t)h.recs[q].kind + ((uint64_t)h.recs[q].a_tr << 8));
	}
	for(size_t q = 0; q < h.xb.size(); ++ q)
		mix((uint64_t)h.xb[q]);
	uint64_t all = 1469598103934665603ull;
	auto mix_all = [&](uint64_t v) { all = (all ^ v) * 1099511628211ull; };
	auto mix_list = [&](const auto &v) {
		mix_all((uint64_t)v.size());
		for(size_t q = 0; q < v.size(); ++ q)
			mix_all((uint64_t)(int64_t)v[q]);
	};
	mix_all(sum);
	for(int64_t v : {(int64_t)h.dp, (int64_t)h.dl, h.nc, h.nl, h.nl_total, h.no, h.n_red, h.ld, h.n_sblk, h.n_pairs, h.n_items, h.n_multi,
		h.n_ablk, (int64_t)h.n_slots, (int64_t)h.xcd_max_items, (int64_t)h.u_landmark_major, (int64_t)h.factored})
		mix_all((uint64_t)v);
	mix_list(h.pose_block); mix_list(h.lm_block); mix_list(h.is_lm); mix_list(h.tile_mask);
	mix_list(h.lm_ptr); mix_list(h.bs_ptr); mix_list(h.lm_coff); mix_list(h.lm_rbase);
	mix_list(h.obs_pose); mix_list(h.obs_lm); mix_list(h.obs_off); mix_list(h.pose_rbase);
	mix_list(h.cam_ptr); mix_list(h.cam_obs); mix_list(h.wpos);
	mix_list(h.multi_blk); mix_list(h.multi_ptr); mix_list(h.sblk_voff);
	for(int64_t v : {h.s_st.nb, h.s_st.n, h.s_st.nnzb, h.s_st.nvals})
		mix_all((uint64_t)v);
	mix_list(h.s_st.col_ptr); mix_list(h.s_st.row_idx); mix_list(h.s_st.blk_off); mix_list(h.s_st.base); mix_list(h.s_st.dim);
	mix_all((uint64_t)h.recs.size());
	for(size_t q = 0; q < h.recs.size(); ++ q)
		for(int64_t v : {(int64_t)h.recs[q].kind, (int64_t)h.recs[q].a_tr, h.recs[q].dst, h.recs[q].aoff})
			mix_all((uint64_t)v);
	out[0] = h.nc; out[1] = h.nl; out[2] = h.no; out[3] = h.n_pairs; out[4] = h.n_sblk; out[5] = h.n_items; out[6] = h.n_multi;
	out[7] = (int64_t)sum;
	out[8] = (int64_t)all;
	return sec;
}

void schur_tile_mask_host_probe(const Structure &st, std::vector<uint64_t> &words)
{
	SchurPlanHost h;
	PlanScratch w;
	schur_partition(st, 0, 1, false, h, w);
	schur_tile_mask(st, h.is_lm, w.pose_of, h.dp, h.nc * h.dp, words);
}

bool schur_cam_order_host_probe(const Structure &st, int shard_rank, int shard_world, bool sparse_S, bool mis, const int64_t *order_in,
	std::vector<int32_t> &cam_order, TileDagCost cost[2])
{
	if(!order_in) {
		SchurPlanHost h;
		schur_plan_host(st, shard_rank, shard_world, sparse_S || mis, mis, h);
		std::vector<int32_t> cam_of(st.nb, -1);
		int32_t nc = 0;
		for(int64_t j = 0; j < st.nb; ++ j)
			if(!h.is_lm[j])
				cam_of[j] = nc ++;
		cam_order.resize((size_t)nc);
		bool used = false;
		for(int32_t q = 0; q < nc; ++ q) {
			cam_order[q] = cam_of[h.pose_block[q]];
			used = used || cam_order[q] != q;
		}
		cost[0] = h.cam_cost[0];
		cost[1] = h.cam_cost[1];
		return used;
	}
	SPP_REQUIRE(!sparse_S && !mis, SPP_E_UNSUPPORTED,
		"the model of a given camera order needs the dense guided Schur mode ({6,3} or {3,2} block widths)");
	SchurPlanHost h;
	PlanScratch w;
	schur_partition(st, 0, 1, false, h, w);
	return schur_cam_order(st, h.is_lm, w.pose_of, h.nc, h.dp, false, false, order_in, cam_order, cost);
}

}
```

slam_plus_plus_amd/csrc/spp_switches.h:

```cpp
#pragma once

#include <stdint.h>
#include <stdlib.h>
#include <string.h>
#include <algorithm>

namespace spp {

constexpr long long WAIT_TICKS_PER_MS = 100000;
constexpr long long WAIT_TICKS_DEFAULT = 500 * WAIT_TICKS_PER_MS;

enum Ordering { ORDERING_AUTO, ORDERING_AMD, ORDERING_ND };
constexpr int MID_FRONT_MAX = 640;

struct Switches {
	bool verbose;
	int plan_threads;
	int64_t plan_min_work;

	int dense_sched;
	int fused;
	int aux_reserve_cus;
	int tile_444;
	int dense_la;
	int la_chain_mask;
	int la_g2;
	int la_bulk_acquire;
	int64_t la_slots;
	int la_trace;
	int tail_rows;
	int tail_mask;
	double tail_order_beta;
	int tail_early;
	long long tail_timeout_ticks;
	int tail_trace;
	int trsv_chain;
	int trsv_mform;

	bool sacc_ulm;
	bool sacc_factored;
	int64_t sacc_tile;
	int64_t sacc_tile_cols;
	int sacc_xcd;
	int sacc_chunk;
	int schur_cam_order;
	int backsubst_fused;
	int schur_side;
	int solve_async;
	int lm_stream;

	int mid_front_max;
	Ordering ordering;
	int64_t amalg_small;
	double amalg_zeros;
	int64_t amalg_relax_h;
	double amalg_zeros_small;
	bool sparse_teams;
	int sparse_team_max;
	int sparse_team_cols;
	int sparse_dag;
	int dag_split;
	long long dag_timeout_ticks;
	int dag_trace;
};

inline int env_int(const char *name, int dflt)
{
	const char *e = getenv(name);
	return e ? atoi(e) : dflt;
}

inline long long env_i64(const char *name, long long dflt)
{
	const char *e = getenv(name);
	return e ? atoll(e) : dflt;
}

inline double env_double(const char *name, double dflt)
{
	const char *e = getenv(name);
	return e ? atof(e) : dflt;
}

inline Switches parse_switches()
{
	Switches w;
	w.verbose = getenv("SPP_VERBOSE") != nullptr;
	const char *threads = getenv("SPP_PLAN_THREADS");
	w.plan_threads = threads ? std::max(1, atoi(threads)) : 0;
	w.plan_min_work = std::max<int64_t>(1, env_i64("SPP_PLAN_MIN_WORK", int64_t(1) << 18));

	w.dense_sched = env_int("SPP_DENSE_SCHED", 1);
	w.fused = env_int("SPP_FUSED", 1);
	w.aux_reserve_cus = env_int("SPP_AUX_RESERVE_CUS", 32);
	w.tile_444 = env_int("SPP_TILE_444", 0);
	w.dense_la = env_int("SPP_DENSE_LA", 0);
	w.la_chain_mask = env_int("SPP_LA_CHAIN_MASK", 1);
	w.la_g2 = env_int("SPP_LA_G2", 0);
	w.la_bulk_acquire = env_int("SPP_LA_BULK_ACQUIRE", 1);
	w.la_slots = env_i64("SPP_LA_SLOTS", 0);
	w.la_trace = env_int("SPP_LA_TRACE", 0);
	w.tail_rows = env_int("SPP_DENSE_TAIL", 1) ? env_int("SPP_TAIL_ROWS", 44) : 0;
	w.tail_mask = env_int("SPP_TAIL_MASK", 1);
	w.tail_order_beta = env_double("SPP_TAIL_ORDER_BETA", 0.0);
	w.tail_early = env_int("SPP_TAIL_EARLY", 1);
	w.tail_timeout_ticks = env_i64("SPP_TAIL_TIMEOUT_TICKS", WAIT_TICKS_DEFAULT);
	w.tail_trace = env_int("SPP_TAIL_TRACE", 0);
	w.trsv_chain = env_int("SPP_TRSV_CHAIN", 2);
	w.trsv_mform = env_int("SPP_TRSV_MFORM", 1);

	w.sacc_ulm = env_int("SPP_SACC_ULM", 1) != 0;
	w.sacc_factored = env_int("SPP_SACC_FACTORED", 1) != 0;
	w.sacc_tile = std::max<int64_t>(1, env_i64("SPP_SACC_TILE", 4));
	w.sacc_tile_cols = env_i64("SPP_SACC_TILE_COLS", -2);
	w.sacc_xcd = env_int("SPP_SACC_XCD", 1);
	w.sacc_chunk = env_int("SPP_SACC_CHUNK", 1);
	w.schur_cam_order = env_int("SPP_SCHUR_CAM_ORDER", 1);
	w.backsubst_fused = env_int("SPP_BACKSUBST_FUSED", 1);
	w.schur_side = env_int("SPP_SCHUR_SIDE", 1);
	w.solve_async = env_int("SPP_SOLVE_ASYNC", 1);
	w.lm_stream = env_int("SPP_LM_STREAM", 1);

	w.mid_front_max = std::max(128, std::min(MID_FRONT_MAX, env_int("SPP_MID_FRONT_MAX", 320)));
	const char *ordering = getenv("SPP_ORDERING");
	w.ordering = !ordering ? ORDERING_AUTO : (!strcmp(ordering, "nd") ? ORDERING_ND : ORDERING_AMD);
	w.amalg_small = env_i64("SPP_AMALG_SMALL", 32);
	w.amalg_zeros = env_double("SPP_AMALG_ZEROS", 0.12);
	w.amalg_relax_h = env_i64("SPP_AMALG_RELAX_H", 96);
	w.amalg_zeros_small = env_double("SPP_AMALG_ZEROS_SMALL", 0.2);
	w.sparse_teams = env_int("SPP_SPARSE_TEAMS", 1) != 0;
	w.sparse_team_max = std::max(1, std::min(64, env_int("SPP_SPARSE_TEAM_MAX", 40)));
	w.sparse_team_cols = std::max(8, std::min(256, env_int("SPP_SPARSE_TEAM_COLS", 16)));
	w.sparse_dag = env_int("SPP_SPARSE_DAG", 1);
	w.dag_split = env_int("SPP_DAG_SPLIT", 1);
	w.dag_timeout_ticks = env_i64("SPP_DAG_TIMEOUT_TICKS", WAIT_TICKS_DEFAULT);
	w.dag_trace = env_int("SPP_DAG_TRACE", 0);
	return w;
}

inline const Switches &switches()
{
	static const Switches w = parse_switches();
	return w;
}

}
```

slam_plus_plus_amd/csrc/spp_tile_plan.cpp:

```cpp

#include "spp_internal.h"
#include <algorithm>

namespace spp {

void tile_mask_mark(int64_t n, int bs, int64_t nblk, const int32_t *i1, const int32_t *i2, std::vector<uint64_t> &words)
{
	words.clear();
	const int64_t Tr = (n + DENSE_NB - 1) / DENSE_NB, Tc = n / DENSE_NB + 1;
	if(Tr < 1 || Tc > 64)
		return;
	words.assign((size_t)Tr, 0);
	for(int64_t q = 0; q < nblk; ++ q) {
		const int64_t a = std::min(i1[q], i2[q]), b = std::max(i1[q], i2[q]);
		const int64_t r0 = a * bs / DENSE_NB, r1 = std::min<int64_t>(a * bs + bs - 1, n - 1) / DENSE_NB;
		const int64_t c0 = b * bs / DENSE_NB, c1 = std::min<int64_t>(b * bs + bs - 1, n - 1) / DENSE_NB;
		if(a < 0 || r0 >= Tr || c0 >= Tr)
			continue;
		words[r0] |= (1ull << c0) | (1ull << c1);
		words[r1] |= (1ull << c0) | (1ull << c1);
	}
}

int64_t tile_mask_close(int64_t n, bool has_rhs, bool fill, std::vector<uint64_t> &words)
{
	const int64_t Tr = (n + DENSE_NB - 1) / DENSE_NB, Tc = has_rhs ? n / DENSE_NB + 1 : Tr;
	if(Tr < 1 || Tc > 64 || (int64_t)words.size() != Tr) {
		words.clear();
		return -1;
	}
	const uint64_t cols = Tc == 64 ? ~0ull : (1ull << Tc) - 1;
	for(int64_t i = 0; i < Tr; ++ i) {
		words[i] |= 1ull << i;
		if(has_rhs)
			words[i] |= 1ull << (n / DENSE_NB);
		words[i] &= cols & ~((1ull << i) - 1);
	}
	int64_t updates = 0;
	for(int64_t k = 0; k < Tr; ++ k) {
		const uint64_t r = words[k] & ~((2ull << k) - 1);
		for(uint64_t m = r; m; m &= m - 1) {
			const int a = __builtin_ctzll(m);
			if(a >= Tr)
				break;
			const uint64_t f = r & ~((1ull << a) - 1);
			if(fill)
				words[a] |= f;
			updates += __builtin_popcountll(words[a] & f);
		}
	}
	return updates;
}

void tail_order_table(const std::vector<uint64_t> &bits, int Tr, int Tc, bool have_pre, double beta, int resident, bool early,
	std::vector<int> &order, int *info)
{
	std::vector<std::pair<double, int> > key;
	for(int i = 0; i < Tr; ++ i)
		for(int j = i; j < Tc; ++ j)
			if((bits[(size_t)i + 1] >> j) & 1)
				key.push_back(std::make_pair((double)i + beta * (double)j, (i << 16) | j));
	std::stable_sort(key.begin(), key.end(), [](const std::pair<double, int> &x, const std::pair<double, int> &y) { return x.first < y.first; });
	order.resize(key.size());
	for(size_t q = 0; q < key.size(); ++ q)
		order[q] = key[q].second;
	int widest = 1;
	for(int i = 0; i < Tr; ++ i)
		widest = std::max(widest, (int)__builtin_popcountll(bits[(size_t)i + 1]));
	const int D = std::max(resident, 0) / widest;
	if(info) {
		info[0] = 0;
		info[1] = Tr;
		info[2] = D;
		info[3] = 0;
		info[4] = widest;
	}
	if(!early || resident <= 0)
		return;
	auto first_step = [&](const int i, const int j) -> int {
		for(int k = have_pre ? -1 : 0; k < i; ++ k) {
			const uint64_t w = bits[(size_t)k + 1];
			if((w >> i) & (w >> j) & 1)
				return k;
		}
		return i;
	};
	int r_star = Tr;
	for(int i = Tr - 1; i >= 0; -- i) {
		bool all_lag = true;
		for(int j = i; j < Tc && all_lag; ++ j)
			if((bits[(size_t)i + 1] >> j) & 1)
				all_lag = i - first_step(i, j) > D;
		if(!all_lag)
			break;
		r_star = i;
	}
	int n_early = 0;
	std::vector<int> live((size_t)Tr + 1, 0);
	for(size_t q = 0; q < order.size(); ++ q) {
		const int i = order[q] >> 16, j = order[q] & 0xffff;
		if(i >= r_star)
			++ n_early;
		else {
			++ live[(size_t)std::max(first_step(i, j), 0)];
			-- live[(size_t)i + 1];
		}
	}
	int demand = 0;
	for(int r = 0, run = 0; r < Tr; ++ r) {
		run += live[(size_t)r];
		demand = std::max(demand, run);
	}
	if(info)
		info[3] = demand;
	if(n_early == 0 || n_early > resident / 2 || resident - n_early < demand)
		return;
	std::stable_partition(order.begin(), order.end(), [r_star](const int t) { return (t >> 16) >= r_star; });
	if(info) {
		info[0] = n_early;
		info[1] = r_star;
	}
}

TileDagCost tile_dag_cost(int64_t n, const std::vector<uint64_t> &filled, int resident)
{
	TileDagCost c;
	const int64_t Tr = (int64_t)filled.size();
	std::vector<uint64_t> w(filled);
	c.updates = tile_mask_close(n, true, true, w);
	std::vector<int> depth((size_t)Tr, 1);
	for(int64_t k = 0; k < Tr; ++ k) {
		c.tiles += __builtin_popcountll(w[k]);
		for(int64_t j = 0; j < k; ++ j)
			if((w[j] >> k) & 1)
				depth[k] = std::max(depth[k], depth[j] + 1);
		c.path = std::max<int64_t>(c.path, depth[k]);
	}
	c.cost_us = std::max(c.path * TAIL_MODEL_STEP_US, c.updates * TAIL_MODEL_UPDATE_US / std::max(1, resident)) + TAIL_MODEL_START_US;
	return c;
}

}
```

Before: 1.313 billion block-nnz/s.

## Apply elimination steps in DAG-depth order in streamed dense tail factor

Computes a per-tile-row step order sorted by elimination-DAG depth from the tile mask of the dissected camera ordering, and passes it into the streamed tail kernel so each tile applies its update steps in that order instead of ascending row order. It also adds a 'lead' mode in the tail tile ordering: when the early-seating budget is exceeded, tiles are sorted by row depth and a budget-limited prefix of late rows is seated first. The intent is to shorten waits on the dependency chain in the persistent tail kernel. Each tile now decodes a byte-packed order table, which adds per-tile overhead, and the new schedule could interact badly with the residency and wait logic.

```diff
diff --git a/include/spp_hip.h b/include/spp_hip.h
--- a/include/spp_hip.h
+++ b/include/spp_hip.h
@@ -207,6 +207,11 @@
 	int shard_world, int flags, const int64_t *order_in, int64_t *cam_order, double *figures);
 int spp_tail_order_host(int64_t n, int has_rhs, const uint64_t *words, int64_t nwords, int resident, int early, double beta,
 	int32_t *table, int32_t *info);
+int spp_dense_posv_ordered(spp_ctx *ctx, double *d_A, int64_t n, int64_t ld, double *d_b, const uint64_t *words, int64_t nwords,
+	const int32_t *step_order);
+int spp_tail_step_order_host(int64_t n, const uint64_t *words, int64_t nwords, int32_t *step_order);
+int spp_schur_step_order_host(int64_t nb, const int32_t *dim, const int64_t *col_ptr, const int64_t *row_idx, int shard_rank,
+	int shard_world, int flags, int32_t *step_order);
 int spp_dense_gemm_tn_sub(spp_ctx *ctx, int64_t m, int64_t n, int64_t k,
 	const double *d_A, int64_t lda, const double *d_B, int64_t ldb, double *d_C, int64_t ldc);
 int spp_dense_gemm_tn_sub_upper(spp_ctx *ctx, int64_t m, int64_t n, int64_t k,
diff --git a/slam_plus_plus_amd/api.py b/slam_plus_plus_amd/api.py
--- a/slam_plus_plus_amd/api.py
+++ b/slam_plus_plus_amd/api.py
@@ -30,6 +30,7 @@
     "spp_microbench_copy", "spp_microbench_mfma_f64", "spp_microbench_ctile", "spp_microbench_update", "spp_block_ordering", "spp_schur_plan_host", "spp_set_profiling", "spp_se2_linearize_device", "spp_se2_update_device", "spp_ba_linearize_device", "spp_ba_stereo_linearize_device", "spp_ba_update_device", "spp_sim3_ba_linearize_device", "spp_sim3_update_device", "spp_se3_linearize_device", "spp_se3_update_device", "spp_edge_chi2_device", "spp_edge_robust_weights_device", "spp_edge_hessian_maxdiag_device",
     "spp_lm_gain_denominator_device", "spp_dense_potrf_upper", "spp_dense_posv",
     "spp_dense_posv_masked", "spp_tile_mask_host", "spp_schur_tile_mask_host", "spp_tail_order_host", "spp_schur_cam_order_host",
+    "spp_dense_posv_ordered", "spp_tail_step_order_host", "spp_schur_step_order_host",
     "spp_dense_gemm_tn_sub", "spp_dense_gemm_tn_sub_upper", "spp_dense_front_factor", "spp_version",
 ]
 
@@ -126,6 +127,9 @@
         "spp_schur_tile_mask_host": (cint, [i64, vp, vp, vp, cint, cint, vp]),
         "spp_tail_order_host": (cint, [i64, cint, vp, i64, cint, cint, dbl, vp, vp]),
         "spp_schur_cam_order_host": (cint, [i64, vp, vp, vp, cint, cint, cint, vp, vp, vp]),
+        "spp_dense_posv_ordered": (cint, [vp, vp, i64, i64, vp, vp, i64, vp]),
+        "spp_tail_step_order_host": (cint, [i64, vp, i64, vp]),
+        "spp_schur_step_order_host": (cint, [i64, vp, vp, vp, cint, cint, cint, vp]),
         "spp_dense_gemm_tn_sub": (cint, [vp, i64, i64, i64, vp, i64, vp, i64, vp, i64]),
         "spp_dense_gemm_tn_sub_upper": (cint, [vp, i64, i64, i64, vp, i64, vp, i64, vp, i64]),
         "spp_dense_front_factor": (cint, [vp, vp, i64, i64, i64, vp]),
@@ -227,11 +231,34 @@
     table = np.zeros(64 * 65 // 2 + 64, dtype=np.int32)
     info = np.zeros(5, dtype=np.int32)
     code = lib.spp_tail_order_host(int(n), 1 if has_rhs else 0, _ptr(words) if words.size else None, words.size, int(resident),
-                                   1 if early else 0, float(beta), _ptr(table), _ptr(info))
+                                   int(early), float(beta), _ptr(table), _ptr(info))
     if code < 0:
         raise SppError("spp_tail_order_host failed: %d" % code)
     tiles = [(int(t) >> 16, int(t) & 0xffff) for t in table[:code]]
     return tiles, dict(zip(("n_early", "r_star", "rows_resident", "live_demand", "widest"), (int(v) for v in info)))
+
+
+def tail_step_order_host(n, words):
+    lib = load_library()
+    words = np.ascontiguousarray(words, dtype=np.uint64)
+    out = np.zeros(64, dtype=np.int32)
+    code = lib.spp_tail_step_order_host(int(n), _ptr(words), words.size, _ptr(out))
+    if code < 0:
+        raise SppError("spp_tail_step_order_host failed: %d" % code)
+    return out[:code].copy()
+
+
+def schur_step_order_host(lam, sparse_S=False, mis=False, shard_rank=0, shard_world=1):
+    lib = load_library()
+    col_ptr = np.ascontiguousarray(lam.col_ptr, dtype=np.int64)
+    row_idx = np.ascontiguousarray(lam.row_idx, dtype=np.int64)
+    dim = np.ascontiguousarray(lam.dim, dtype=np.int32)
+    out = np.zeros(64, dtype=np.int32)
+    code = lib.spp_schur_step_order_host(lam.nb, _ptr(dim), _ptr(col_ptr), _ptr(row_idx), shard_rank, shard_world,
+                                         (1 if sparse_S else 0) | (2 if mis else 0), _ptr(out))
+    if code < 0:
+        raise SppError("spp_schur_step_order_host failed: %d" % code)
+    return out[:code].copy()
 
 
 class DeviceArray:
diff --git a/slam_plus_plus_amd/csrc/spp_api.cpp b/slam_plus_plus_amd/csrc/spp_api.cpp
--- a/slam_plus_plus_amd/csrc/spp_api.cpp
+++ b/slam_plus_plus_amd/csrc/spp_api.cpp
@@ -580,6 +580,18 @@
 	});
 }
 
+int spp_schur_step_order_host(int64_t nb, const int32_t *dim, const int64_t *col_ptr, const int64_t *row_idx, int shard_rank,
+	int shard_world, int flags, int32_t *step_order)
+{
+	return schur_host_entry(nb, dim, col_ptr, row_idx, shard_rank, shard_world, step_order, [&](const Structure &st) {
+		std::vector<int32_t> order;
+		schur_step_order_host_probe(st, shard_rank, shard_world, (flags & 1) != 0, (flags & 2) != 0, order);
+		for(size_t q = 0; q < order.size(); ++ q)
+			step_order[q] = order[q];
+		return (int)order.size();
+	});
+}
+
 int spp_schur_buffer_size(const spp_ctx *ctx, int64_t *n_doubles)
 {
 	if(!ctx || !n_doubles)
@@ -1251,7 +1263,7 @@
 		std::vector<int> order;
 		int oinfo[5];
 		const bool use = nwords && early;
-		tail_order_table(bits, (int)Tr, (int)Tc, false, beta, use ? resident : 0, use, order, oinfo);
+		tail_order_table(bits, (int)Tr, (int)Tc, false, beta, use ? resident : 0, use, order, oinfo, use && (early & 2) != 0);
 		for(size_t q = 0; q < order.size(); ++ q)
 			table[q] = order[q];
 		if(info)
@@ -1263,18 +1275,47 @@
 	}
 }
 
-int spp_dense_posv_masked(spp_ctx *ctx, double *d_A, int64_t n, int64_t ld, double *d_b, const uint64_t *words, int64_t nwords)
+int spp_tail_step_order_host(int64_t n, const uint64_t *words, int64_t nwords, int32_t *step_order)
+{
+	const int64_t Tr = (n + DENSE_NB - 1) / DENSE_NB;
+	if(n <= 0 || n / DENSE_NB + 1 > 64 || !words || nwords != Tr || !step_order)
+		return SPP_E_BADARG;
+	try {
+		std::vector<uint64_t> mask(words, words + nwords);
+		tile_mask_close(n, true, true, mask);
+		std::vector<int32_t> order;
+		tail_step_order(mask, order);
+		for(size_t q = 0; q < order.size(); ++ q)
+			step_order[q] = order[q];
+		return (int)order.size();
+	} catch(...) {
+		return SPP_E_NOMEM;
+	}
+}
+
+static int dense_posv_entry(spp_ctx *ctx, double *d_A, int64_t n, int64_t ld, double *d_b, const uint64_t *words, int64_t nwords,
+	const int32_t *step_order)
 {
 	if(!ctx || !d_A || !d_b || n <= 0 || ld < n || nwords < 0 || (nwords && !words))
 		return SPP_E_BADARG;
 	SPP_TRY(ctx)
 	SPP_HIP_CHECK(hipSetDevice(ctx->device));
 	std::vector<uint64_t> mask(words, words + nwords);
+	std::vector<int32_t> order;
 	if(nwords) {
 		SPP_REQUIRE(nwords == (n + DENSE_NB - 1) / DENSE_NB, SPP_E_BADARG, "posv: one mask word per tile row of 128");
 		tile_mask_close(n, true, true, mask);
 	}
-	TileMaskGuard guard(ctx->dense, &mask);
+	if(step_order) {
+		std::vector<char> seen((size_t)nwords, 0);
+		for(int64_t q = 0; q < nwords; ++ q) {
+			SPP_REQUIRE(step_order[q] >= 0 && step_order[q] < nwords && !seen[(size_t)step_order[q]], SPP_E_BADARG,
+				"posv: the step order must be a permutation of the tile rows 0 .. nwords - 1");
+			seen[(size_t)step_order[q]] = 1;
+		}
+		order.assign(step_order, step_order + nwords);
+	}
+	TileMaskGuard guard(ctx->dense, &mask, &order);
 	const int64_t ldp = ((n + 1 + DENSE_NB - 1) / DENSE_NB) * DENSE_NB;
 	DevBuf<double> tmp;
 	tmp.reserve((size_t)ldp * ldp);
@@ -1296,6 +1337,19 @@
 	SPP_CATCH(ctx)
 }
 
+int spp_dense_posv_masked(spp_ctx *ctx, double *d_A, int64_t n, int64_t ld, double *d_b, const uint64_t *words, int64_t nwords)
+{
+	return dense_posv_entry(ctx, d_A, n, ld, d_b, words, nwords, nullptr);
+}
+
+int spp_dense_posv_ordered(spp_ctx *ctx, double *d_A, int64_t n, int64_t ld, double *d_b, const uint64_t *words, int64_t nwords,
+	const int32_t *step_order)
+{
+	if(!step_order || nwords <= 0)
+		return SPP_E_BADARG;
+	return dense_posv_entry(ctx, d_A, n, ld, d_b, words, nwords, step_order);
+}
+
 int spp_dense_gemm_tn_sub(spp_ctx *ctx, int64_t m, int64_t n, int64_t k, const double *d_A, int64_t lda,
 	const double *d_B, int64_t ldb, double *d_C, int64_t ldc)
 {
diff --git a/slam_plus_plus_amd/csrc/spp_dense.hip b/slam_plus_plus_amd/csrc/spp_dense.hip
--- a/slam_plus_plus_amd/csrc/spp_dense.hip
+++ b/slam_plus_plus_amd/csrc/spp_dense.hip
@@ -1320,13 +1320,18 @@
 			dw.tail_resident = 0;
 		}
 	}
+	const bool ordered = k < 0 && dw.step_order && (int64_t)dw.step_order->size() == nsteps;
+	bool ascending = true;
+	for(int q = 0; ordered && q < Tr; ++ q)
+		ascending = ascending && (*dw.step_order)[(size_t)q] == q;
+	const bool lead = early && ordered && !ascending && sw.tail_early_lead != 0;
 	if(dw.tail_order_tr != Tr || dw.tail_order_tc != Tc || dw.tail_order_bits != bits || dw.tail_order_pre != (k >= 0) ||
-	   dw.tail_order_masked != early) {
+	   dw.tail_order_masked != early || dw.tail_order_lead != lead) {
 		if(!dw.tail_order_host.empty())
 			SPP_HIP_CHECK(hipStreamSynchronize(s));
 		std::vector<int> &order = dw.tail_order_host;
 		int oinfo[5];
-		tail_order_table(bits, Tr, Tc, k >= 0, sw.tail_order_beta, early ? dw.tail_resident : 0, early, order, oinfo);
+		tail_order_table(bits, Tr, Tc, k >= 0, sw.tail_order_beta, early ? dw.tail_resident : 0, early, order, oinfo, lead);
 		if(sw.verbose)
 			fprintf(stderr, "[spp] streamed tail: %d x %d tiles, %d listed, %d resident; %d tiles of rows %d.. seated first (whole rows resident %d, live demand %d)\n",
 				Tr, Tc, (int)order.size(), early ? dw.tail_resident : 0, oinfo[0], oinfo[1], oinfo[2], oinfo[3]);
@@ -1336,6 +1341,7 @@
 		dw.tail_order_bits = bits;
 		dw.tail_order_pre = k >= 0;
 		dw.tail_order_masked = early;
+		dw.tail_order_lead = lead;
 	}
 	const int ntile = (int)dw.tail_order_host.size();
 	TailArgs a;
@@ -1343,6 +1349,31 @@
 	memset(a.rowbits, 0, sizeof(a.rowbits));
 	for(size_t q = 0; q < bits.size(); ++ q)
 		a.rowbits[q] = bits[q];
+	{
+		const std::vector<int32_t> *so = ordered ? dw.step_order : nullptr;
+		if(so) {
+			uint64_t seen = 0;
+			for(int q = 0; q < Tr; ++ q) {
+				const int32_t v = (*so)[(size_t)q];
+				SPP_REQUIRE(v >= 0 && v < Tr && !((seen >> v) & 1), SPP_E_BADARG, "streamed tail: the step order is not a permutation of the tile rows");
+				seen |= 1ull << v;
+			}
+		}
+		unsigned char list[sizeof(a.sorder)];
+		memset(list, TAIL_NO_STEP, sizeof(list));
+		int p = 0;
+		if(k >= 0)
+			list[p ++] = (unsigned char)(signed char)-1;
+		for(int q = 0; q < Tr; ++ q)
+			list[p ++] = (unsigned char)(so ? (*so)[(size_t)q] : q);
+		for(size_t w = 0; w < sizeof(a.sorder) / 8; ++ w) {
+			a.sorder[w] = 0;
+			for(int b = 0; b < 8; ++ b)
+				a.sorder[w] |= (unsigned long long)list[8 * w + b] << (8 * b);
+		}
+		if(sw.verbose && so)
+			fprintf(stderr, "[spp] streamed tail: %d steps in the caller's step order\n", Tr);
+	}
 	a.A = d_A;
 	a.ld = ld;
 	a.rows = rows;
diff --git a/slam_plus_plus_amd/csrc/spp_dense_tail.h b/slam_plus_plus_amd/csrc/spp_dense_tail.h
--- a/slam_plus_plus_amd/csrc/spp_dense_tail.h
+++ b/slam_plus_plus_amd/csrc/spp_dense_tail.h
@@ -23,7 +23,14 @@
 	long long *trace;
 	const int *order;
 	unsigned long long rowbits[TAIL_MAX_ROWS + 1];
+	unsigned long long sorder[TAIL_MAX_ROWS / 8 + 1];
 };
+constexpr int TAIL_NO_STEP = 127;
+
+__host__ __device__ inline int tail_sorder_at(const unsigned long long *sorder, const int p)
+{
+	return (int)(signed char)(unsigned char)(sorder[p >> 3] >> (8 * (p & 7)));
+}
 
 constexpr int TAIL_ABORT_TIMEOUT = 2;
 
@@ -142,12 +149,20 @@
 		const int ek = tid & 15, ec = tid >> 4;
 		constexpr int PS = 18;
 		const int ekp = 4 * (ek & 3) + (ek >> 2);
-		const int kfirst = a.have_pre ? -1 : 0;
+		unsigned long long ksteps = 0;
+		for(int k = a.have_pre ? -1 : 0; k < ti; ++ k) {
+			const unsigned long long w = a.rowbits[k + 1];
+			ksteps |= ((w >> ti) & (w >> tj) & 1) << (k + 1);
+		}
 		unsigned long long steps = 0;
-		for(int k = kfirst; k < ti; ++ k) {
-			const unsigned long long w = a.rowbits[k + 1];
-			if(((w >> ti) & (w >> tj) & 1) != 0)
-				steps |= 1ull << (k - kfirst);
+		for(int q = 0; 8 * q < a.Tr + a.have_pre; ++ q) {
+			const unsigned long long word = a.sorder[q];
+#pragma unroll
+			for(int b = 0; b < 8; ++ b) {
+				const int k = (int)(signed char)(unsigned char)(word >> (8 * b));
+				if(k < ti && ((ksteps >> (k + 1)) & 1) != 0)
+					steps |= 1ull << (8 * q + b);
+			}
 		}
 		const int nst = 8 * __builtin_popcountll(steps);
 		double va[2], vb[2];
@@ -163,12 +178,15 @@
 		int avail = a.have_pre ? 8 : 0;
 		pre_first = diag && nst > 0 && (nst & 1) == 0 && a.rows - i0 >= 16;
 		bool inflight = false;
-		int k = kfirst;
+		int k = a.have_pre ? -1 : 0;
+		int knext = steps ? tail_sorder_at(a.sorder, __builtin_ctzll(steps)) : k;
 		for(int sidx = 0; sidx < nst; ++ sidx) {
 			const int J = sidx & 7;
 			if(J == 0) {
-				k = kfirst + __builtin_ctzll(steps);
+				k = knext;
 				steps &= steps - 1;
+				if(steps)
+					knext = tail_sorder_at(a.sorder, __builtin_ctzll(steps));
 			}
 			if(J == 0 && k >= 0)
 				avail = 0;
diff --git a/slam_plus_plus_amd/csrc/spp_internal.h b/slam_plus_plus_amd/csrc/spp_internal.h
--- a/slam_plus_plus_amd/csrc/spp_internal.h
+++ b/slam_plus_plus_amd/csrc/spp_internal.h
@@ -205,6 +205,7 @@
 	std::vector<int64_t> lm_block;
 	std::vector<uint8_t> is_lm;
 	std::vector<uint64_t> tile_mask;
+	std::vector<int32_t> step_order;
 	DevBuf<int32_t> lm_ptr;
 	DevBuf<int32_t> bs_ptr;
 	int64_t n_bs = 0;
@@ -253,9 +254,11 @@
 	std::vector<int> tail_order_host;
 	int tail_order_tr = 0, tail_order_tc = 0;
 	std::vector<uint64_t> tail_order_bits;
+	bool tail_order_lead = false;
 	bool tail_order_pre = false, tail_order_masked = false;
 	int tail_resident = -1;
 	const std::vector<uint64_t> *tile_mask = nullptr;
+	const std::vector<int32_t> *step_order = nullptr;
 	bool tail_masked_whole = false;
 	int tail_rows_last = 0;
 	bool tail_disabled = false;
@@ -384,7 +387,8 @@
 };
 TileDagCost tile_dag_cost(int64_t n, const std::vector<uint64_t> &filled, int resident);
 void tail_order_table(const std::vector<uint64_t> &bits, int Tr, int Tc, bool have_pre, double beta, int resident, bool early,
-	std::vector<int> &order, int *info);
+	std::vector<int> &order, int *info, bool lead = false);
+void tail_step_order(const std::vector<uint64_t> &filled, std::vector<int32_t> &order);
 
 void build_schur_plan(spp_ctx *ctx, bool sparse_S, bool mis = false);
 int64_t schur_buffer_doubles(const spp_ctx *ctx);
@@ -393,6 +397,7 @@
 void schur_tile_mask_host_probe(const Structure &st, std::vector<uint64_t> &words);
 bool schur_cam_order_host_probe(const Structure &st, int shard_rank, int shard_world, bool sparse_S, bool mis, const int64_t *order_in,
 	std::vector<int32_t> &cam_order, TileDagCost cost[2]);
+bool schur_step_order_host_probe(const Structure &st, int shard_rank, int shard_world, bool sparse_S, bool mis, std::vector<int32_t> &step_order);
 
 void sparse_analyze(spp_ctx *ctx, const Structure &st);
 int sparse_factor_solve(spp_ctx *ctx, const double *d_vals, double *d_rhs);
@@ -427,8 +432,12 @@
 void dense_set_padding_on(hipStream_t st, double *d_A, int64_t ld, int64_t n);
 struct TileMaskGuard {
 	DenseWork &d;
-	TileMaskGuard(DenseWork &dw, const std::vector<uint64_t> *m) : d(dw) { d.tile_mask = (m && !m->empty()) ? m : nullptr; }
-	~TileMaskGuard() { d.tile_mask = nullptr; }
+	TileMaskGuard(DenseWork &dw, const std::vector<uint64_t> *m, const std::vector<int32_t> *so = nullptr) : d(dw)
+	{
+		d.tile_mask = (m && !m->empty()) ? m : nullptr;
+		d.step_order = (so && !so->empty()) ? so : nullptr;
+	}
+	~TileMaskGuard() { d.tile_mask = nullptr; d.step_order = nullptr; }
 };
 int dense_front_factor(spp_ctx *ctx, double *d_F, int64_t ld, int64_t w, int64_t h, double *d_image);
 bool dense_gemm_tn_sub(spp_ctx *ctx, int64_t m, int64_t n, int64_t k, const double *A, int64_t lda,
diff --git a/slam_plus_plus_amd/csrc/spp_schur.hip b/slam_plus_plus_amd/csrc/spp_schur.hip
--- a/slam_plus_plus_amd/csrc/spp_schur.hip
+++ b/slam_plus_plus_amd/csrc/spp_schur.hip
@@ -1259,7 +1259,7 @@
 		if(!sp.side_padded)
 			dense_set_padding(ctx, S, ld, sp.n_red);
 		{
-			TileMaskGuard guard(ctx->dense, &sp.tile_mask);
+			TileMaskGuard guard(ctx->dense, &sp.tile_mask, &sp.step_order);
 			const bool own = S == sp.S.p;
 			if(own)
 				sp.unlisted_dirty = true;
diff --git a/slam_plus_plus_amd/csrc/spp_schur_plan.cpp b/slam_plus_plus_amd/csrc/spp_schur_plan.cpp
--- a/slam_plus_plus_amd/csrc/spp_schur_plan.cpp
+++ b/slam_plus_plus_amd/csrc/spp_schur_plan.cpp
@@ -21,7 +21,7 @@
 	sblk_voff.release(); s_st = Structure(); sparse_S = false; mis = false;
 	pair_a.release(); pair_b.release(); multi_blk.release(); multi_ptr.release(); cinv.release(); lfac.release();
 	W.release(); Up.release(); xw.release(); partial.release(); S.release();
-	pose_block.clear(); lm_block.clear(); is_lm.clear(); tile_mask.clear();
+	pose_block.clear(); lm_block.clear(); is_lm.clear(); tile_mask.clear(); step_order.clear();
 }
 
 bool schur_applicable(const Structure &st, int *dp_out, int *dl_out)
@@ -460,6 +460,8 @@
 	Structure s_st;
 	std::vector<uint64_t> tile_mask;
 	TileDagCost cam_cost[2];
+	bool cam_dissected = false;
+	std::vector<int32_t> step_order;
 };
 
 struct Obs { int32_t lm, pose; int64_t off; };
@@ -522,6 +524,7 @@
 	std::vector<int32_t> &pose_of = w.pose_of;
 	std::vector<int32_t> cam_order;
 	if(schur_cam_order(st, is_lm, pose_of, nc, dp, sparse_S, mis, nullptr, cam_order, h.cam_cost)) {
+		h.cam_dissected = true;
 		const std::vector<int64_t> natural(h.pose_block);
 		for(int64_t q = 0; q < nc; ++ q) {
 			h.pose_block[q] = natural[cam_order[q]];
@@ -1138,6 +1141,14 @@
 		"reduced camera system too large for the dense path (use SPP_MODE_SCHUR_SPARSE)");
 	if(!sparse_S)
 		schur_tile_mask(st, h.is_lm, w.pose_of, h.dp, h.n_red, h.tile_mask);
+	if(h.cam_dissected && !h.tile_mask.empty() && switches().tail_step_order) {
+		tail_step_order(h.tile_mask, h.step_order);
+		bool identity = true;
+		for(size_t q = 0; q < h.step_order.size(); ++ q)
+			identity = identity && h.step_order[q] == (int32_t)q;
+		if(identity)
+			h.step_order.clear();
+	}
 	scan_columns(st, h, w);
 	clk.lap("partition + observation scan");
 	if(sparse_S && shard_world > 1)
@@ -1180,6 +1191,7 @@
 	sp.is_lm.swap(h.is_lm);
 	sp.add_A = (ctx->shard_rank == 0);
 	sp.tile_mask.swap(h.tile_mask);
+	sp.step_order.swap(h.step_order);
 	if(sparse_S) {
 		sp.s_st = h.s_st;
 		sp.sblk_voff.upload(h.sblk_voff, s);
@@ -1305,6 +1317,20 @@
 	schur_tile_mask(st, h.is_lm, w.pose_of, h.dp, h.nc * h.dp, words);
 }
 
+bool schur_step_order_host_probe(const Structure &st, int shard_rank, int shard_world, bool sparse_S, bool mis, std::vector<int32_t> &step_order)
+{
+	SchurPlanHost h;
+	schur_plan_host(st, shard_rank, shard_world, sparse_S || mis, mis, h);
+	const bool carried = !h.step_order.empty();
+	step_order = h.step_order;
+	if(!carried) {
+		step_order.resize(h.tile_mask.size());
+		for(size_t q = 0; q < step_order.size(); ++ q)
+			step_order[q] = (int32_t)q;
+	}
+	return carried;
+}
+
 bool schur_cam_order_host_probe(const Structure &st, int shard_rank, int shard_world, bool sparse_S, bool mis, const int64_t *order_in,
 	std::vector<int32_t> &cam_order, TileDagCost cost[2])
 {
diff --git a/slam_plus_plus_amd/csrc/spp_switches.h b/slam_plus_plus_amd/csrc/spp_switches.h
--- a/slam_plus_plus_amd/csrc/spp_switches.h
+++ b/slam_plus_plus_amd/csrc/spp_switches.h
@@ -32,6 +32,8 @@
 	int tail_mask;
 	double tail_order_beta;
 	int tail_early;
+	int tail_step_order;
+	int tail_early_lead;
 	long long tail_timeout_ticks;
 	int tail_trace;
 	int trsv_chain;
@@ -104,6 +106,8 @@
 	w.tail_mask = env_int("SPP_TAIL_MASK", 1);
 	w.tail_order_beta = env_double("SPP_TAIL_ORDER_BETA", 0.0);
 	w.tail_early = env_int("SPP_TAIL_EARLY", 1);
+	w.tail_step_order = env_int("SPP_TAIL_STEP_ORDER", 1);
+	w.tail_early_lead = env_int("SPP_TAIL_EARLY_LEAD", 1);
 	w.tail_timeout_ticks = env_i64("SPP_TAIL_TIMEOUT_TICKS", WAIT_TICKS_DEFAULT);
 	w.tail_trace = env_int("SPP_TAIL_TRACE", 0);
 	w.trsv_chain = env_int("SPP_TRSV_CHAIN", 2);
diff --git a/slam_plus_plus_amd/csrc/spp_tile_plan.cpp b/slam_plus_plus_amd/csrc/spp_tile_plan.cpp
--- a/slam_plus_plus_amd/csrc/spp_tile_plan.cpp
+++ b/slam_plus_plus_amd/csrc/spp_tile_plan.cpp
@@ -53,7 +53,7 @@
 }
 
 void tail_order_table(const std::vector<uint64_t> &bits, int Tr, int Tc, bool have_pre, double beta, int resident, bool early,
-	std::vector<int> &order, int *info)
+	std::vector<int> &order, int *info, bool lead)
 {
 	std::vector<std::pair<double, int> > key;
 	for(int i = 0; i < Tr; ++ i)
@@ -113,13 +113,54 @@
 	}
 	if(info)
 		info[3] = demand;
-	if(n_early == 0 || n_early > resident / 2 || resident - n_early < demand)
+	if(n_early == 0)
 		return;
+	if(n_early > resident / 2 || resident - n_early < demand) {
+		if(!lead)
+			return;
+		const int room = std::min(resident / 2, resident - demand);
+		int r2 = r_star - 1, n_lead = 0;
+		for(int i = r_star; i < Tr; ++ i) {
+			const int row = (int)__builtin_popcountll(bits[(size_t)i + 1] & ~((1ull << i) - 1) & (Tc == 64 ? ~0ull : (1ull << Tc) - 1));
+			if(n_lead + row > room)
+				break;
+			n_lead += row;
+			r2 = i;
+		}
+		if(n_lead == 0)
+			return;
+		std::vector<int> depth((size_t)Tr, 1);
+		for(int k = 0; k < Tr; ++ k)
+			for(int j = 0; j < k; ++ j)
+				if((bits[(size_t)j + 1] >> k) & 1)
+					depth[k] = std::max(depth[k], depth[j] + 1);
+		auto key = [&](const int t) { const int i = t >> 16; return i < r_star ? 1 + depth[i] : (i <= r2 ? 0 : 2 + Tr); };
+		std::stable_sort(order.begin(), order.end(), [&key](const int x, const int y) { return key(x) < key(y); });
+		if(info) {
+			info[0] = n_lead;
+			info[1] = r_star;
+		}
+		return;
+	}
 	std::stable_partition(order.begin(), order.end(), [r_star](const int t) { return (t >> 16) >= r_star; });
 	if(info) {
 		info[0] = n_early;
 		info[1] = r_star;
 	}
+}
+
+void tail_step_order(const std::vector<uint64_t> &filled, std::vector<int32_t> &order)
+{
+	const int Tr = (int)std::min<size_t>(filled.size(), 64);
+	std::vector<int> depth((size_t)Tr, 1);
+	for(int k = 0; k < Tr; ++ k)
+		for(int j = 0; j < k; ++ j)
+			if((filled[(size_t)j] >> k) & 1)
+				depth[k] = std::max(depth[k], depth[j] + 1);
+	order.resize((size_t)Tr);
+	for(int k = 0; k < Tr; ++ k)
+		order[k] = k;
+	std::stable_sort(order.begin(), order.end(), [&depth](const int32_t x, const int32_t y) { return depth[x] < depth[y]; });
 }
 
 TileDagCost tile_dag_cost(int64_t n, const std::vector<uint64_t> &filled, int resident)
```

Result: faster. 1.333 billion block-nnz/s (median of 6 runs) (+1.5%).
